# Bart-Weil/Dynamic-Camera-Augmented-VideoPose3D

Measured on AMD Instinct MI355X. Metric: 3D poses/sec, 243-frame RF, 17 joints, 1024ch; MPJPE vs ref, higher is better.
Workload: dtype f16x3; 1 GPU; config4 global batch sharded over ranks, TemporalModelOptimized1f 243-frame RF windows, 17 joints, 1024 ch; window batch assembled on device from resident sequences inside the step; global_batch=65536, windows_per_gpu=65536, parallelism=dp1 (contiguous shards of one global window set, no collective)

## Files before the change

dynamic-camera-augmented-videopose3d_amd/csrc/conv_gemm_a4.hip:

```cpp
#include <cstdlib>
#include <cstring>
#include <utility>

#include "gemm_common.h"

namespace vp3d {
namespace {

using namespace gemm;

typedef __attribute__((address_space(3))) void* lds_ptr_t;
typedef __attribute__((address_space(1))) void* gbl_ptr_t;

constexpr int GM = 256, GN = 256, GK = 64;
constexpr int GBUF = (GM + GN) * GK * 2;
constexpr int GW_OFF = GM * GK * 2;
constexpr int GMAXN = 1024;
constexpr int kLgkm0 = 0xC07F;
constexpr int kVm0Lgkm0 = 0x0070;
constexpr int kVm16Lgkm0 = 0x4070;
constexpr int kVm32Lgkm0 = 0x8070;

template <typename F, int... Is>
__device__ __forceinline__ void static_for_impl(F&& f, std::integer_sequence<int, Is...>) {
    (f(std::integral_constant<int, Is>{}), ...);
}
template <int N, typename F>
__device__ __forceinline__ void static_for(F&& f) {
    static_for_impl(f, std::make_integer_sequence<int, N>{});
}

__device__ __forceinline__ void pinned_barrier() {
    __builtin_amdgcn_sched_barrier(0);
    __builtin_amdgcn_s_barrier();
    __builtin_amdgcn_sched_barrier(0);
}

template <typename CT, int R, bool ZERO>
__device__ __forceinline__ void amma(const u32x4& w, const u32x4& a) {
    if constexpr (std::is_same<CT, __bf16>::value) {
        if constexpr (ZERO)
            asm volatile("v_mfma_f32_16x16x32_bf16 a[%c2:%c3], %0, %1, 0" ::"v"(w), "v"(a), "i"(R), "i"(R + 3));
        else
            asm volatile("v_mfma_f32_16x16x32_bf16 a[%c2:%c3], %0, %1, a[%c2:%c3]" ::"v"(w), "v"(a), "i"(R),
                         "i"(R + 3));
    } else {
        if constexpr (ZERO)
            asm volatile("v_mfma_f32_16x16x32_f16 a[%c2:%c3], %0, %1, 0" ::"v"(w), "v"(a), "i"(R), "i"(R + 3));
        else
            asm volatile("v_mfma_f32_16x16x32_f16 a[%c2:%c3], %0, %1, a[%c2:%c3]" ::"v"(w), "v"(a), "i"(R),
                         "i"(R + 3));
    }
}

#ifdef VP3D_ABLATION
template <typename CT, int R, bool ZERO>
__device__ __forceinline__ void amma32(const u32x4& w, const u32x4& a) {
    if constexpr (std::is_same<CT, __bf16>::value) {
        if constexpr (ZERO)
            asm volatile("v_mfma_f32_32x32x16_bf16 a[%c2:%c3], %0, %1, 0" ::"v"(w), "v"(a), "i"(R), "i"(R + 15));
        else
            asm volatile("v_mfma_f32_32x32x16_bf16 a[%c2:%c3], %0, %1, a[%c2:%c3]" ::"v"(w), "v"(a), "i"(R),
                         "i"(R + 15));
    } else {
        if constexpr (ZERO)
            asm volatile("v_mfma_f32_32x32x16_f16 a[%c2:%c3], %0, %1, 0" ::"v"(w), "v"(a), "i"(R), "i"(R + 15));
        else
            asm volatile("v_mfma_f32_32x32x16_f16 a[%c2:%c3], %0, %1, a[%c2:%c3]" ::"v"(w), "v"(a), "i"(R),
                         "i"(R + 15));
    }
}
#endif

__device__ __forceinline__ void launder_s(int& x) { asm volatile("" : "+s"(x)); }
__device__ __forceinline__ void launder_lane_consts(int& a, int& b, int& c, int& d, int& e, int& f, int& g, int& h,
                                                    int& i) {
    asm volatile("" : "+v"(a), "+v"(b), "+v"(c), "+v"(d), "+v"(e), "+v"(f), "+v"(g), "+v"(h), "+v"(i));
}
__device__ __forceinline__ void launder_params(ConvGemmParams& p) {
    asm volatile("" : "+s"(p.M), "+s"(p.Kp), "+s"(p.T_out), "+s"(p.T_in), "+s"(p.stride), "+s"(p.dil), "+s"(p.Ktap),
                 "+s"(p.lda), "+s"(p.R_T), "+s"(p.R_stride), "+s"(p.R_off), "+s"(p.ldr), "+s"(p.ldy));
    asm volatile("" : "+s"(p.A), "+s"(p.W), "+s"(p.R), "+s"(p.Y));
}

template <int R>
__device__ __forceinline__ float aread() {
    float x;
    asm volatile("v_accvgpr_read_b32 %0, a%c1" : "=v"(x) : "i"(R));
    return x;
}

#define A4_C10(d) "a" #d "0", "a" #d "1", "a" #d "2", "a" #d "3", "a" #d "4", "a" #d "5", "a" #d "6", "a" #d "7", \
                  "a" #d "8", "a" #d "9"
#define A4_ALL_AGPRS                                                                                              \
    "a0", "a1", "a2", "a3", "a4", "a5", "a6", "a7", "a8", "a9", A4_C10(1), A4_C10(2), A4_C10(3), A4_C10(4),      \
        A4_C10(5), A4_C10(6), A4_C10(7), A4_C10(8), A4_C10(9), A4_C10(10), A4_C10(11), A4_C10(12), A4_C10(13),   \
        A4_C10(14), A4_C10(15), A4_C10(16), A4_C10(17), A4_C10(18), A4_C10(19), A4_C10(20), A4_C10(21),          \
        A4_C10(22), A4_C10(23), A4_C10(24), "a250", "a251", "a252", "a253", "a254", "a255"

#ifdef VP3D_ABLATION
__device__ unsigned long long* g_a4_trace;
#endif

template <typename CT, int ABL, int X3 = 0, bool GD = true, bool SPLIT = false, int HNL = 0, bool IX = false>
__global__ __launch_bounds__(256, 1) void conv_gemm_a4(ConvGemmParams p_arg) {
    constexpr bool HN = HNL > 0;
    static_assert(!HN || (GD && !SPLIT), "half-N tiles: grouped pieces, no split");
    static_assert(HNL < 2 || X3 != 0, "quarter-N tiles: the split-fp16 epilogue only");
    static_assert(!IX || (X3 == 1 && GD && !SPLIT), "indirect windows: the split-fp16 whole / half-N / quarter-N tiles");
    constexpr int TN = GN >> HNL;
    constexpr int NJ = TN / 32;
    constexpr int WP = TN / 32;
    constexpr int NB = NJ < 4 ? NJ : 4;
    if (p_arg.gate != nullptr && *p_arg.gate != p_arg.gate_serial) return;
    asm volatile("" ::: A4_ALL_AGPRS);
    ConvGemmParams p = p_arg;

    __shared__ __attribute__((aligned(16))) char smem[2 * GBUF + 2 * GMAXN * 4];
    float* const s_scale = (float*)(smem + 2 * GBUF);
    float* const s_shift = s_scale + GMAXN;

    const int tid = threadIdx.x;
    const int lane = tid & 63;
    const int wid = tid >> 6;
    const int wr = wid >> 1, wc = wid & 1;
    const int widu = __builtin_amdgcn_readfirstlane(wid);

    for (int i = tid; i < p.N; i += 256) {
        s_scale[i] = p.scale[i];
        s_shift[i] = p.shift[i];
    }

    const int ntn = p.N / TN;
    const int ntm = (p.M + GM - 1) / GM;
    const int mt_base = HN ? p.sk_full : 0;
    const int ntiles = (ntm - mt_base) * ntn;
    const int nk_all = p.Kp / GK;
    const int S = SPLIT ? p.sk_split : 1;
    const int sk_full = S > 1 ? p.sk_full : ntiles;
    const int nunits = S > 1 ? sk_full + S * p.sk_left : ntiles;
    constexpr int kWhole = 0, kOwner = 1, kHelper = 2;
    int kb = 0, nk = nk_all, role = kWhole, sidx = 0, sq = 0;
    const bool lres_layer = X3 == 0 && p.R != nullptr && nk_all >= 3;
    bool lres = lres_layer;
#ifdef VP3D_ABLATION
    unsigned long long* const trc = (ABL & 4) && g_a4_trace ? g_a4_trace + (size_t)blockIdx.x * 10 : nullptr;
    unsigned long long mid_cyc = 0;
    auto stamp = [&](int slot) __attribute__((always_inline)) {
        if (trc && tid == 0) {
            trc[slot] = __builtin_amdgcn_s_memrealtime();
            trc[slot + 5] = __builtin_amdgcn_s_memtime();
        }
    };
    stamp(0);
    if (trc && tid == 0)
        trc[4] = ((unsigned long long)__builtin_amdgcn_s_getreg((31 << 11) | 20) << 32) |
                 __builtin_amdgcn_s_getreg((31 << 11) | 4);
#endif

    int prow = lane >> 3;
    int lc = (lane & 7) ^ (((wid & 1) * 4 + (prow >> 1)) & 7);
    constexpr int kReb = GD ? 3072 : 0;
    int m0 = 0, n0 = 0;
    uint32_t va[8], vw[8], vr[8];
    __amdgpu_buffer_rsrc_t a_rsrc, w_rsrc, r_rsrc;
    auto setup = [&](int unit) __attribute__((always_inline)) {
        int tix = unit;
        kb = 0;
        nk = nk_all;
        role = kWhole;
        if (S > 1 && unit >= sk_full) {
            const int v = unit - sk_full;
            sidx = v % p.sk_left;
            sq = S - 1 - v / p.sk_left;
            tix = sk_full + sidx;
            kb = sq * (nk_all / S);
            nk = nk_all / S;
            role = sq == 0 ? kOwner : kHelper;
        }
        lres = lres_layer && role != kHelper && nk >= 3;
        const int wg = xcd_remap(tix, ntiles);
        const int tile_m = wg / ntn;
        const int tile_n = wg - tile_m * ntn;
        m0 = (mt_base + tile_m) * GM;
        n0 = tile_n * TN;
        const int srow0 = IX && p.T_in < 0 ? 0 : src_row(p, m0);
        a_rsrc = make_rsrc((const char*)((const CT*)p.A + (int64_t)srow0 * p.lda) - kReb, 0x7FFFFFFFu);
        w_rsrc = make_rsrc((const char*)((const CT*)p.W + (int64_t)n0 * p.Kp) - kReb, 0x7FFFFFFFu);
        const int rrow0 = lres ? res_row(p, m0) : 0;
        r_rsrc = make_rsrc((const char*)(lres ? (const CT*)p.R + (int64_t)rrow0 * p.ldr : (const CT*)p.A) - kReb,
                           0x7FFFFFFFu);
        int sln = lane, swv = widu;
        asm volatile("" : "+v"(sln));
        launder_s(swv);
        const int spr = sln >> 3;
        if constexpr (IX) {
            int wb[8], wr0[8];
#pragma unroll
            for (int i = 0; i < 8; ++i) {
                const int q = GD ? 8 * swv + i : swv + 4 * i;
                int m = m0 + 8 * q + spr;
                m = m < p.M ? m : p.M - 1;
                wb[i] = m / p.T_out;
                va[i] = (uint32_t)((m - wb[i] * p.T_out) * p.stride);
            }
            window_rows(p.A, p.T_in, wb, wr0);
#pragma unroll
            for (int i = 0; i < 8; ++i) {
                const int lci = GD ? (sln & 7) ^ (((i & 1) * 4 + (spr >> 1)) & 7) : lc;
                const int reb = GD ? kReb - (i & 3) * 1024 : 0;
                va[i] = (uint32_t)(((wr0[i] + (int)va[i] - srow0) * p.lda + lci * 8) * (int)sizeof(CT) + reb);
            }
        }
#pragma unroll
        for (int i = 0; i < 8; ++i) {
            const int q = GD ? 8 * swv + i : swv + 4 * i;
            const int qw = HN ? WP * swv + (i % WP) : q;
            const int lci = GD ? (sln & 7) ^ (((i & 1) * 4 + (spr >> 1)) & 7) : lc;
            const int reb = GD ? kReb - (i & 3) * 1024 : 0;
            int m = m0 + 8 * q + spr;
            m = m < p.M ? m : p.M - 1;
            if constexpr (!IX)
                va[i] = (uint32_t)(((src_row(p, m) - srow0) * p.lda + lci * 8) * (int)sizeof(CT) + reb);
            vw[i] = (uint32_t)(((8 * qw + prow) * p.Kp + lci * 8) * (int)sizeof(CT) + reb);
            vr[i] = lres ? (uint32_t)(((res_row(p, m) - rrow0) * p.ldr + lci * 8) * (int)sizeof(CT) + reb) : 0u;
        }
    };
    auto lds_dst = [&](char* buf, int q) __attribute__((always_inline)) -> char* {
        int w = widu;
        launder_s(w);
        return buf + (w + q) * 1024;
    };
    struct Bases {
        char* g[4];
    };
    auto bases_of = [&](char* buf) __attribute__((always_inline)) -> Bases {
        int w = widu;
        launder_s(w);
        char* b = buf + 8 * w * 1024;
        if constexpr (HN) return Bases{{b, b + 4096, buf + GW_OFF + WP * w * 1024, nullptr}};
        return Bases{{b, b + 4096, b + GW_OFF, b + GW_OFF + 4096}};
    };
    auto piece_lds = [&](char* buf, int i) __attribute__((always_inline)) -> char* {
        if constexpr (GD) {
            int w = widu;
            launder_s(w);
            return buf + (8 * w + (i & 4)) * 1024;
        } else {
            return lds_dst(buf, 4 * i);
        }
    };
    auto res_piece = [&](char* buf, auto k_c, int h) __attribute__((always_inline)) {
        constexpr int k = decltype(k_c)::value;
        constexpr int wcp = k >> 3;
        __builtin_amdgcn_raw_ptr_buffer_load_lds(r_rsrc, (lds_ptr_t)piece_lds(buf + wcp * 32 * 1024, k & 7), 16,
                                                 vr[k & 7], (uint32_t)((n0 + 128 * wcp + 64 * h) * (int)sizeof(CT)),
                                                 GD ? (k & 3) * 1024 : 0, 0);
    };
    auto a_koff = [&](int s) __attribute__((always_inline)) -> int64_t {
        const int k0 = (kb + s) * GK;
        const int tap = k0 / p.Ktap;
        return (int64_t)tap * p.dil * p.lda + (k0 - tap * p.Ktap);
// ... 89 lines not shown
        });
        if constexpr (RD) __builtin_amdgcn_s_waitcnt(kLgkm0);
    };

    auto mid = [&](int vm) __attribute__((always_inline)) {
#ifdef VP3D_ABLATION
        const unsigned long long c0 = (ABL & 4) ? __builtin_amdgcn_s_memtime() : 0;
#endif
        if (vm == 16)
            __builtin_amdgcn_s_waitcnt(kVm16Lgkm0);
        else if (vm == 32)
            __builtin_amdgcn_s_waitcnt(kVm32Lgkm0);
        else
            __builtin_amdgcn_s_waitcnt(kVm0Lgkm0);
        pinned_barrier();
#ifdef VP3D_ABLATION
        if (ABL & 4) mid_cyc += __builtin_amdgcn_s_memtime() - c0;
#endif
    };
    using C0 = std::integral_constant<int, 0>;
    using C1 = std::integral_constant<int, 1>;
    using T_ = std::integral_constant<bool, true>;
    using F_ = std::integral_constant<bool, false>;
    auto ktile = [&](auto zero_c, auto rd_c, auto dma_c, int t, char* b, char* o, int resp, int vm) __attribute__((always_inline)) {
        phase(C0{}, zero_c, T_{}, F_{}, b, fo1, nullptr, 0, -1);
        mid(vm);
        phase(C1{}, F_{}, rd_c, dma_c, o, fo0, b, t + 2, resp);
    };

    typedef float f32x2 __attribute__((ext_vector_type(2)));
    typedef int i32x2 __attribute__((ext_vector_type(2)));
    typedef short s16x2 __attribute__((ext_vector_type(2)));
    typedef CT ct2 __attribute__((ext_vector_type(2)));
    typedef CT ct4 __attribute__((ext_vector_type(4)));
    typedef unsigned int u32x2 __attribute__((ext_vector_type(2)));
    int grp = lane >> 4;
    int c0 = 8 * ((grp & 1) * 2 + (grp >> 1));
    u32x2 resr[8][4];
    int enk = nk;
    auto res_addr = [&](int h, int i, int j) __attribute__((always_inline)) -> const u32x2* {
        return (const u32x2*)(smem + ((enk - 2 + h) & 1) * GBUF + wc * 256 * 128 + wr * 128 * 128 + (lane & 15) * 128 +
                              (grp & 1) * 8 + i * 2048 + (((2 * j + (grp >> 1)) ^ fsw) << 4));
    };
    auto part_ptr = [&](int si, int q) __attribute__((always_inline)) -> float* {
        return p.sk_part + (size_t)(si * (S - 1) + (q - 1)) * 65536 + (size_t)wid * 16384 + lane * 4;
    };
    auto helper_store = [&](int si, int q) __attribute__((always_inline)) {
        float* const base = part_ptr(si, q);
        static_for<64>([&](auto r_c) __attribute__((always_inline)) {
            constexpr int R4 = decltype(r_c)::value;
            *(f32x4*)(base + R4 * 256) = f32x4{aread<4 * R4>(), aread<4 * R4 + 1>(), aread<4 * R4 + 2>(), aread<4 * R4 + 3>()};
        });
        __builtin_amdgcn_fence(__ATOMIC_RELEASE, "agent");
        pinned_barrier();
        if (tid == 0) {
            const SplitCtl* ctl = (const SplitCtl*)((const char*)p.sk_flag + kSplitCtlOffset);
            if (!ctl->drop) __hip_atomic_fetch_add(p.sk_flag + si, 1, __ATOMIC_RELAXED, __HIP_MEMORY_SCOPE_AGENT);
        }
    };
    auto owner_wait = [&](int si) __attribute__((always_inline)) {
        if (tid == 0) {
            const SplitCtl* ctl = (const SplitCtl*)((const char*)p.sk_flag + kSplitCtlOffset);
            const unsigned long long spin = ctl->spin_ticks;
            const unsigned long long t0 = __builtin_amdgcn_s_memrealtime();
            while (__hip_atomic_load(p.sk_flag + si, __ATOMIC_RELAXED, __HIP_MEMORY_SCOPE_AGENT) < S - 1) {
                __builtin_amdgcn_s_sleep(1);
                if (__builtin_amdgcn_s_memrealtime() - t0 > spin) {
                    unsigned* err = ctl->err;
                    if (err) __hip_atomic_fetch_or(err, kFaultSplitTimeout, __ATOMIC_RELAXED, __HIP_MEMORY_SCOPE_SYSTEM);
                    break;
                }
            }
        }
        pinned_barrier();
        __builtin_amdgcn_fence(__ATOMIC_ACQUIRE, "agent");
    };
    auto owner_add = [&](auto r_c, int si, f32x2 (&v)[2]) __attribute__((always_inline)) {
        constexpr int R = decltype(r_c)::value;
        for (int q = 1; q < S; ++q) {
            const f32x4 pr = *(const f32x4*)(part_ptr(si, q) + (R / 4) * 256);
            v[0] = v[0] + f32x2{pr[0], pr[1]};
            v[1] = v[1] + f32x2{pr[2], pr[3]};
        }
    };
    auto owner_done = [&](int si) __attribute__((always_inline)) {
        if (tid == 0) __hip_atomic_fetch_sub(p.sk_flag + si, S - 1, __ATOMIC_RELAXED, __HIP_MEMORY_SCOPE_AGENT);
    };
    auto epi_fast = [&](auto h_c, bool with_res, int em0, int en0, __amdgpu_buffer_rsrc_t y_rsrc, int own_si) __attribute__((always_inline)) {
        constexpr int H = decltype(h_c)::value;
        const int nw = en0 + wc * (TN / 2) + 64 * H;
        f32x2 sc[4][2], sh[4][2];
#pragma unroll
        for (int j = 0; j < 4; ++j) {
            const int n = nw + 16 * j + 4 * grp;
            const f32x4 s4 = *(const f32x4*)&s_scale[n];
            const f32x4 h4 = *(const f32x4*)&s_shift[n];
            sc[j][0] = f32x2{s4[0], s4[1]};
            sc[j][1] = f32x2{s4[2], s4[3]};
            sh[j][0] = f32x2{h4[0], h4[1]};
            sh[j][1] = f32x2{h4[2], h4[3]};
        }
        static_for<8>([&](auto i_c) __attribute__((always_inline)) {
            constexpr int I = decltype(i_c)::value;
            const int m = em0 + wr * 128 + 16 * I + (lane & 15);
            uint32_t pk[4][2];
            static_for<4>([&](auto j_c) __attribute__((always_inline)) {
                constexpr int J = decltype(j_c)::value;
                constexpr int R = 4 * (8 * I + 4 * H + J);
                f32x2 v[2] = {f32x2{aread<R>(), aread<R + 1>()}, f32x2{aread<R + 2>(), aread<R + 3>()}};
                if (own_si >= 0) owner_add(std::integral_constant<int, R>{}, own_si, v);
                ct4 r4;
                if (with_res) r4 = __builtin_bit_cast(ct4, resr[I][J]);
#pragma unroll
                for (int q = 0; q < 2; ++q) {
                    f32x2 x = v[q] * sc[J][q];
                    x = x + sh[J][q];
                    if (with_res) {
                        i32x2 xi = __builtin_bit_cast(i32x2, x);
                        xi = __builtin_elementwise_max(xi, i32x2{0, 0});
                        x = __builtin_bit_cast(f32x2, xi);
                        x = x + f32x2{(float)r4[2 * q], (float)r4[2 * q + 1]};
                    }
                    s16x2 o = __builtin_bit_cast(s16x2, __builtin_convertvector(x, ct2));
                    if (!with_res) o = __builtin_elementwise_max(o, s16x2{0, 0});
                    pk[J][q] = __builtin_bit_cast(uint32_t, o);
                }
            });
            asm volatile("s_nop 1\n\tv_permlane16_swap_b32 %0, %1\n\tv_permlane16_swap_b32 %2, %3\n\t"
                         "v_permlane16_swap_b32 %4, %5\n\tv_permlane16_swap_b32 %6, %7"
                         : "+v"(pk[0][0]), "+v"(pk[1][0]), "+v"(pk[0][1]), "+v"(pk[1][1]), "+v"(pk[2][0]),
                           "+v"(pk[3][0]), "+v"(pk[2][1]), "+v"(pk[3][1]));
            const uint32_t yo = (uint32_t)(((size_t)(m - em0) * p.ldy + nw + c0) * sizeof(CT));
#pragma unroll
            for (int jp = 0; jp < 2; ++jp)
                __builtin_amdgcn_raw_buffer_store_b128(
                    u32x4{pk[2 * jp][0], pk[2 * jp][1], pk[2 * jp + 1][0], pk[2 * jp + 1][1]}, y_rsrc,
                    m < p.M ? yo + 64 * jp : 0xFFFFFFC0u, 0, 0);
        });
    };
    using H0 = std::integral_constant<int, 0>;
    using H1 = std::integral_constant<int, 1>;
    int res0 = -1, res1 = -1;

    int tix = blockIdx.x;
    setup(tix);
    stage_01();
    bool first = true;
    bool prev_lres = false;
    bool x3_prev_res = false;
    bool x3_prev_xres = false;
    for (;;) {
        launder_lane_consts(prow, lc, fsw, fo0, fo1, a_base, w_base, grp, c0);
        launder_params(p);
        const int next = HN ? nunits : tix + (int)gridDim.x;
        const bool has_next = next < nunits;
        res0 = lres ? 0 : -1;
        res1 = lres ? 1 : -1;
        if (first) {
            if (nk > 1)
            {
                if constexpr (HN)
                    asm volatile("s_waitcnt vmcnt(%0)" ::"n"(8 + WP) : "memory");
                else
                    asm volatile("s_waitcnt vmcnt(16)" ::: "memory");
            }
            else
                asm volatile("s_waitcnt vmcnt(0)" ::: "memory");
            asm volatile("s_waitcnt lgkmcnt(0)" ::: "memory");
        } else if constexpr (X3 != 0) {
            if (x3_prev_xres)
                asm volatile("s_waitcnt vmcnt(48)" ::: "memory");
            else if (!x3_prev_res)
                asm volatile("s_waitcnt vmcnt(0)" ::: "memory");
        } else {
            asm volatile("s_waitcnt vmcnt(48)" ::: "memory");
        }
        pinned_barrier();
#pragma unroll
        for (int i = 0; i < 8; ++i) {
            fa[0][i] = *(const u32x4*)(buf0 + a_base + i * 2048 + fo0);
            if (i < NJ) fw[0][i] = *(const u32x4*)(buf0 + w_base + i * 2048 + fo0);
        }
        if constexpr (X3 != 0) {
            const bool xres = X3 == 1 && !SPLIT && !HN && !(ABL & 40) && p.R != nullptr && role != kHelper && nk >= 3;
            __amdgpu_buffer_rsrc_t xr_rsrc;
            auto xres_prep = [&]() __attribute__((always_inline)) {
                int ln = lane, wv = widu;
                asm volatile("" : "+v"(ln));
                launder_s(wv);
                const int pr = ln >> 3;
                const int rrow0x = IX && p.R_T < 0 ? 0 : res_row(p, m0);
                xr_rsrc = make_rsrc((const char*)((const f16*)p.R + (int64_t)rrow0x * p.ldr), 0x7FFFFFFFu);
                if constexpr (IX) {
                    int wb[8], wr0[8];
#pragma unroll
                    for (int i = 0; i < 8; ++i) {
                        int m = m0 + 8 * (8 * wv + i) + pr;
                        m = m < p.M ? m : p.M - 1;
                        wb[i] = m / p.T_out;
                        vr[i] = (uint32_t)((m - wb[i] * p.T_out) * p.R_stride + p.R_off);
                    }
                    window_rows(p.R, p.R_T, wb, wr0);
#pragma unroll
                    for (int i = 0; i < 8; ++i) {
                        const int lci = (ln & 7) ^ (((i & 1) * 4 + (pr >> 1)) & 7);
                        vr[i] = (uint32_t)((wr0[i] + (int)vr[i] - rrow0x) * p.ldr * 2 + lci * 16);
                    }
                } else {
#pragma unroll
                    for (int i = 0; i < 8; ++i) {
                        int m = m0 + 8 * (8 * wv + i) + pr;
                        m = m < p.M ? m : p.M - 1;
                        const int lci = (ln & 7) ^ (((i & 1) * 4 + (pr >> 1)) & 7);
                        vr[i] = (uint32_t)((res_row(p, m) - rrow0x) * p.ldr * 2 + lci * 16);
                    }
                }
            };
            auto xres_piece = [&](char* buf, auto i_c, auto s_c, int wcq, int hh) __attribute__((always_inline)) {
                constexpr int I = decltype(i_c)::value;
                constexpr int S2 = decltype(s_c)::value;
                int w = widu;
                launder_s(w);
                __builtin_amdgcn_raw_ptr_buffer_load_lds(xr_rsrc, (lds_ptr_t)(buf + (2 * (8 * w + I) + S2) * 1024), 16, vr[I],
                                                         (uint32_t)(4 * (n0 + wcq * 128 + 64 * hh) + S2 * 128), 0, 0);
            };
            auto x3_phase = [&](auto h_c, auto kind_c, auto zero_c, auto rd_c, auto dma_c, const char* rbuf, char* dbuf,
                                int s, auto rq_c, char* rqbuf) __attribute__((always_inline)) {
                constexpr int RQ = decltype(rq_c)::value;
                constexpr int H = decltype(h_c)::value;
                constexpr int KIND = decltype(kind_c)::value;
                constexpr bool ZERO = decltype(zero_c)::value;
                constexpr bool DO_RD = decltype(rd_c)::value && !(ABL & 2);
                constexpr bool DO_DMA = decltype(dma_c)::value && !(ABL & 1);
                const int64_t aoff = DO_DMA ? a_koff(s) : 0;
                const Bases bs = DO_DMA ? bases_of(dbuf) : Bases{};
                constexpr int JW = HN ? (NJ > 2 ? 2 : 1) : 4;
                static_for<8>([&](auto i_c) __attribute__((always_inline)) {
                    constexpr int I = decltype(i_c)::value;
                    constexpr bool WI = !HN || I < NJ;
                    static_for<NJ>([&](auto j_c) __attribute__((always_inline)) {
                        constexpr int J = decltype(j_c)::value;
                        if constexpr (KIND == 0) {
                            if constexpr (DO_RD && J == 0)
                                fa[1 - H][I] = *(const u32x4*)(rbuf + a_base + I * 2048 + fo1);
                            if constexpr (DO_RD && J == JW && WI)
                                fw[1][I] = *(const u32x4*)(rbuf + w_base + I * 2048 + fo1);
                            amma<CT, 4 * (8 * I + J), ZERO>(fw[0][J], fa[H][I]);
                        } else if constexpr (KIND == 1) {
                            if constexpr (DO_RD && J == 0 && I > 0)
                                fa[1 - H][I - 1] = *(const u32x4*)(rbuf + a_base + (I - 1) * 2048 + fo0);
                            if constexpr (DO_DMA && J == JW) dma_piece(dbuf, i_c, s, aoff, bs);
                            if constexpr (RQ >= 0 && !HN && (J == 2 || J == 6))
                                xres_piece(rqbuf, i_c, std::integral_constant<int, J / 4>{}, RQ, 0);
                            amma<CT, 4 * (8 * I + J), false>(fw[0][J], fa[1 - H][I]);
                        } else {
                            if constexpr (DO_RD && J == 0 && I == 0)
                                fa[1 - H][7] = *(const u32x4*)(rbuf + a_base + 7 * 2048 + fo0);
                            if constexpr (DO_RD && J == JW && WI)
                                fw[0][I] = *(const u32x4*)(rbuf + w_base + I * 2048 + fo0);
                            if constexpr (DO_DMA && J == (HN ? NJ - 1 : 2) && WI)
                                dma_piece(dbuf, std::integral_constant<int, 8 + I>{}, s, aoff, bs);
                            if constexpr (RQ >= 0 && !HN && (J == 2 || J == 6))
                                xres_piece(rqbuf, i_c, std::integral_constant<int, J / 4>{}, RQ, 0);
                            amma<CT, 4 * (8 * I + J), false>(fw[1][J], fa[H][I]);
                        }
                        __builtin_amdgcn_sched_barrier(0);
                    });
                });
                if constexpr (KIND == 2 && DO_RD) __builtin_amdgcn_s_waitcnt(kLgkm0);
            };
            using K0 = std::integral_constant<int, 0>;
            using K1 = std::integral_constant<int, 1>;
            using K2 = std::integral_constant<int, 2>;
            auto x3_ktile_q = [&](auto h_c, auto zero_c, auto rd_c, auto dma_c, auto rql_c, int t, char* b, char* o,
                                  int vm) __attribute__((always_inline)) {
                constexpr bool rql = decltype(rql_c)::value;
                x3_phase(h_c, K0{}, zero_c, T_{}, F_{}, b, nullptr, 0, std::integral_constant<int, -1>{}, nullptr);
                if (vm == 63)
                    __builtin_amdgcn_s_waitcnt(kLgkm0);
                else if (vm == 32)
                    __builtin_amdgcn_s_waitcnt(kVm32Lgkm0);
                else
                    __builtin_amdgcn_s_waitcnt(kVm0Lgkm0);
                pinned_barrier();
                x3_phase(h_c, K1{}, F_{}, rd_c, dma_c, o, b, t + 2, std::integral_constant<int, rql ? 0 : -1>{}, o);
                x3_phase(h_c, K2{}, F_{}, rd_c, dma_c, o, b, t + 2, std::integral_constant<int, rql ? 1 : -1>{}, b);
            };
            auto x3_ktile = [&](auto h_c, auto zero_c, auto rd_c, auto dma_c, int t, char* b, char* o, int vm = 0)
                                __attribute__((always_inline)) {
                x3_ktile_q(h_c, zero_c, rd_c, dma_c, std::false_type{}, t, b, o, vm);
            };
            const int vm0 = first ? 0 : (x3_prev_xres ? 32 : 63);
            if (nk > 2)
                x3_ktile(C0{}, T_{}, T_{}, T_{}, 0, buf0, buf1, vm0);
            else if (nk == 2)
                x3_ktile(C0{}, T_{}, T_{}, F_{}, 0, buf0, buf1, vm0);
            else
                x3_ktile(C0{}, T_{}, F_{}, F_{}, 0, buf0, buf1, vm0);
            int t = 1;
            for (; t + 3 < nk; t += 2) {
                x3_ktile(C1{}, F_{}, T_{}, T_{}, t, buf1, buf0);
                x3_ktile(C0{}, F_{}, T_{}, T_{}, t + 1, buf0, buf1);
            }
            if (t + 2 < nk) {
                x3_ktile(C1{}, F_{}, T_{}, T_{}, t, buf1, buf0);
                x3_ktile(C0{}, F_{}, T_{}, F_{}, t + 1, buf0, buf1);
                if (xres) {
                    xres_prep();
                    x3_ktile_q(C1{}, F_{}, F_{}, F_{}, std::true_type{}, t + 2, buf1, buf0, 0);
                } else {
                    x3_ktile(C1{}, F_{}, F_{}, F_{}, t + 2, buf1, buf0);
                }
            } else if (t + 1 < nk) {
                x3_ktile(C1{}, F_{}, T_{}, F_{}, t, buf1, buf0);
                if (xres) {
                    xres_prep();
                    x3_ktile_q(C0{}, F_{}, F_{}, F_{}, std::true_type{}, t + 1, buf0, buf1, 0);
                } else {
                    x3_ktile(C0{}, F_{}, F_{}, F_{}, t + 1, buf0, buf1);
                }
            } else if (t < nk) {
                x3_ktile(C1{}, F_{}, F_{}, F_{}, t, buf1, buf0);
            }
            asm volatile("s_nop 7\n\ts_nop 7\n\ts_nop 7" ::: "memory");
            const int em0 = m0, en0 = n0;
            const int erole = role, esidx = sidx, esq = sq;
            char* const qb0 = (nk & 1) ? buf1 : buf0;
            char* const qb1 = (nk & 1) ? buf0 : buf1;
            auto xres_read = [&](u32x4 (&rr)[8][2][2]) __attribute__((always_inline)) {
                int ln = lane, wv = widu;
                asm volatile("" : "+v"(ln));
                launder_s(wv);
                const char* qb = (wv & 1) ? qb1 : qb0;
                const int swz = (((ln >> 3) & 1) * 4 + ((ln & 7) >> 1)) & 7;
                const int g = ln >> 4;
                const int cc = (g & 1) * 2 + (g >> 1);
                const char* rowp = qb + (2 * ((wv >> 1) * 16 + ((ln >> 3) & 1))) * 1024 + (ln & 7) * 128;
#pragma unroll
                for (int i = 0; i < 8; ++i)
#pragma unroll
                    for (int jp = 0; jp < 2; ++jp)
#pragma unroll
                        for (int hl = 0; hl < 2; ++hl)
                            rr[i][jp][hl] = *(const u32x4*)(rowp + (4 * i + jp) * 1024 + (((hl * 4 + cc) ^ swz) << 4));
            };
            constexpr int OB = X3 == 2 ? 4 : 2;
            typedef float f32x2 __attribute__((ext_vector_type(2)));
            typedef int i32x2 __attribute__((ext_vector_type(2)));
            const bool has_r = p.R != nullptr;
            int eln = lane, ewv = widu;
            asm volatile("" : "+v"(eln));
            launder_s(ewv);
            const int egrp = eln >> 4, er16 = eln & 15;
            const int ec0 = 8 * ((egrp & 1) * 2 + (egrp >> 1));
            const int ewr = ewv >> 1, ewc = ewv & 1;
            auto x3_half = [&](auto hh_c, auto wr_c, const u32x4 (&rr)[8][2][2], __amdgpu_buffer_rsrc_t y_rsrc)
                               __attribute__((always_inline)) {
                constexpr int HH = decltype(hh_c)::value;
                constexpr bool WITH_R = decltype(wr_c)::value && !(ABL & 8);
                const int nw = en0 + ewc * (TN / 2) + 64 * HH;
                f32x2 sc[4][2], sh[4][2];
#pragma unroll
                for (int j = 0; j < NB; ++j) {
                    const int n = nw + 16 * j + 4 * egrp;
                    const f32x4 s4 = *(const f32x4*)&s_scale[n];
                    const f32x4 h4 = *(const f32x4*)&s_shift[n];
                    sc[j][0] = f32x2{s4[0], s4[1]};
                    sc[j][1] = f32x2{s4[2], s4[3]};
                    sh[j][0] = f32x2{h4[0], h4[1]};
                    sh[j][1] = f32x2{h4[2], h4[3]};
                }
                static_for<8>([&](auto i_c) __attribute__((always_inline)) {
                    constexpr int I = decltype(i_c)::value;
                    const int m = em0 + ewr * 128 + 16 * I + er16;
                    float v4[4][4];
                    static_for<NB>([&](auto j_c) __attribute__((always_inline)) {
                        constexpr int J = decltype(j_c)::value;
                        constexpr int R = 4 * (8 * I + 4 * HH + J);
                        f32x2 v[2] = {f32x2{aread<R>(), aread<R + 1>()}, f32x2{aread<R + 2>(), aread<R + 3>()}};
                        if (erole == kOwner) owner_add(std::integral_constant<int, R>{}, esidx, v);
#pragma unroll
                        for (int q = 0; q < 2; ++q) {
                            f32x2 x = v[q] * sc[J][q];
                            x = x + sh[J][q];
                            if (p.relu) {
                                i32x2 xi = __builtin_bit_cast(i32x2, x);
                                xi = __builtin_elementwise_max(xi, i32x2{0, 0});
                                x = __builtin_bit_cast(f32x2, xi);
                            }
                            v4[J][2 * q] = x[0];
                            v4[J][2 * q + 1] = x[1];
                        }
                    });
#pragma unroll
                    for (int jp = 0; jp < NB / 2; ++jp) {
                        float* x = v4[2 * jp];
                        float* y = v4[2 * jp + 1];
                        asm volatile("s_nop 1\n\tv_permlane16_swap_b32 %0, %1\n\tv_permlane16_swap_b32 %2, %3\n\t"
                                     "v_permlane16_swap_b32 %4, %5\n\tv_permlane16_swap_b32 %6, %7"
                                     : "+v"(x[0]), "+v"(y[0]), "+v"(x[1]), "+v"(y[1]), "+v"(x[2]), "+v"(y[2]),
                                       "+v"(x[3]), "+v"(y[3]));
                        float v[8] = {x[0], x[1], x[2], x[3], y[0], y[1], y[2], y[3]};
                        if constexpr (WITH_R) {
                            const u32x4 rh = rr[I][jp][0], rl = rr[I][jp][1];
#pragma unroll
                            for (int e = 0; e < 4; ++e) {
                                float t0, t1;
                                gemm::x3_res_sum2(rh[e], rl[e], t0, t1);
                                v[2 * e] += t0;
                                v[2 * e + 1] += t1;
                            }
                        }
                        const bool in = m < p.M;
                        if constexpr (X3 == 2) {
                            const uint32_t yo =
                                in ? (uint32_t)(((size_t)(m - em0) * p.ldy + nw + 32 * jp + ec0) * 4) : 0xFFFFFFE0u;
                            __builtin_amdgcn_raw_buffer_store_b128(
                                __builtin_bit_cast(u32x4, f32x4{v[0], v[1], v[2], v[3]}), y_rsrc, yo, 0, 0);
                            __builtin_amdgcn_raw_buffer_store_b128(
                                __builtin_bit_cast(u32x4, f32x4{v[4], v[5], v[6], v[7]}), y_rsrc, yo + 16, 0, 0);
                        } else {
                            u32x4 oh, ol;
                            float t = 0.f;
#pragma unroll
                            for (int e = 0; e < 4; ++e) {
                                oh[e] = gemm::x3_hi2(v[2 * e], v[2 * e + 1]);
                                ol[e] = gemm::x3_split_lo2(oh[e], v[2 * e], v[2 * e + 1]);
                                t = gemm::x3_absmax2(t, v[2 * e], v[2 * e + 1]);
                            }
                            gemm::x3_range_flag(in ? t : 0.f, p.scale, p.N);
                            const uint32_t yo =
                                in ? (uint32_t)(((size_t)(m - em0) * p.ldy + 2 * nw + 64 * jp + ec0) * 2) : 0xFFFFFF00u;
                            if constexpr ((ABL & 16) != 0) {
                                asm volatile("" ::"v"(oh), "v"(ol));
                            } else {
                                __builtin_amdgcn_raw_buffer_store_b128(oh, y_rsrc, yo, 0, 0);
                                __builtin_amdgcn_raw_buffer_store_b128(ol, y_rsrc, yo + 64, 0, 0);
                            }
                        }
                    }
                });
            };
            auto y_rsrc_of = [&]() __attribute__((always_inline)) {
                const size_t y_rest = (size_t)(p.M - em0) * p.ldy * OB;
                return make_rsrc((const char*)p.Y + (size_t)em0 * p.ldy * OB,
                                 clamp_range31(y_rest));
            };
            if (xres) {
                u32x4 rr[8][2][2];
                asm volatile("s_waitcnt vmcnt(0)" ::: "memory");
                pinned_barrier();
                xres_read(rr);
                __builtin_amdgcn_s_waitcnt(kLgkm0);
                pinned_barrier();
                static_for<8>([&](auto i_c) __attribute__((always_inline)) {
                    xres_piece(qb0, i_c, std::integral_constant<int, 0>{}, 0, 1);
                    xres_piece(qb0, i_c, std::integral_constant<int, 1>{}, 0, 1);
                    xres_piece(qb1, i_c, std::integral_constant<int, 0>{}, 1, 1);
                    xres_piece(qb1, i_c, std::integral_constant<int, 1>{}, 1, 1);
                });
                if (erole == kOwner) owner_wait(esidx);
                const __amdgpu_buffer_rsrc_t y_rsrc = y_rsrc_of();
                x3_half(std::integral_constant<int, 0>{}, T_{}, rr, y_rsrc);
                asm volatile("s_waitcnt vmcnt(32)" ::: "memory");
                pinned_barrier();
                xres_read(rr);
                __builtin_amdgcn_s_waitcnt(kLgkm0);
                pinned_barrier();
                if (has_next) {
                    setup(next);
                    stage_01();
                }
                x3_half(std::integral_constant<int, 1>{}, T_{}, rr, y_rsrc);
                if (erole == kOwner) owner_done(esidx);
            } else {
                if (has_next) {
                    setup(next);
                    stage_01();
                }
                if (erole == kHelper) {
                    helper_store(esidx, esq);
                    x3_prev_res = false;
                    x3_prev_xres = false;
                    if (!has_next) break;
                    tix = next;
                    first = false;
                    continue;
                }
                if (erole == kOwner) owner_wait(esidx);
                const __amdgpu_buffer_rsrc_t y_rsrc = y_rsrc_of();
                const int rrow0 = has_r && !(IX && p.R_T < 0) ? res_row(p, em0) : 0;
                const __amdgpu_buffer_rsrc_t rx_rsrc =
                    make_rsrc(has_r ? (const f16*)p.R + (int64_t)rrow0 * p.ldr : (const f16*)p.A, 0x7FFFFFFFu);
                auto global_half = [&](auto hh_c) __attribute__((always_inline)) {
                    constexpr int HH = decltype(hh_c)::value;
                    const int nw = en0 + ewc * (TN / 2) + 64 * HH;
                    u32x4 rr[8][2][2];
                    if (has_r && !(ABL & 8)) {
                        int wb[8], wo[8], wr0[8];
                        if constexpr (IX) {
#pragma unroll
                            for (int i = 0; i < 8; ++i) {
                                int m = em0 + ewr * 128 + 16 * i + er16;
                                m = m < p.M ? m : p.M - 1;
                                wb[i] = m / p.T_out;
                                wo[i] = (m - wb[i] * p.T_out) * p.R_stride + p.R_off;
                            }
                            window_rows(p.R, p.R_T, wb, wr0);
                        }
#pragma unroll
                        for (int i = 0; i < 8; ++i) {
                            int m = em0 + ewr * 128 + 16 * i + er16;
                            m = m < p.M ? m : p.M - 1;
                            const int off = (((IX ? wr0[i] + wo[i] : res_row(p, m)) - rrow0) * p.ldr + 2 * nw + ec0) * 2;
#pragma unroll
                            for (int jp = 0; jp < NB / 2; ++jp) {
                                rr[i][jp][0] = __builtin_bit_cast(
                                    u32x4, __builtin_amdgcn_raw_buffer_load_b128(rx_rsrc, off + 128 * jp, 0, 0));
                                rr[i][jp][1] = __builtin_bit_cast(
                                    u32x4, __builtin_amdgcn_raw_buffer_load_b128(rx_rsrc, off + 128 * jp + 64, 0, 0));
                            }
                        }
                        x3_half(hh_c, T_{}, rr, y_rsrc);
                    } else {
                        x3_half(hh_c, F_{}, rr, y_rsrc);
                    }
                };
                if constexpr ((ABL & 32) == 0) {
                    global_half(std::integral_constant<int, 0>{});
                    if constexpr (!HN) global_half(std::integral_constant<int, 1>{});
                }
                if (erole == kOwner) owner_done(esidx);
            }
            x3_prev_res = has_r;
            x3_prev_xres = xres;
            if (!has_next) break;
            tix = next;
            first = false;
            continue;
        } else {
        const int vm0 = first ? 0 : prev_lres ? 16 : 32;
        if (nk > 2)
            ktile(T_{}, T_{}, T_{}, 0, buf0, buf1, -1, vm0);
        else if (nk == 2)
            ktile(T_{}, T_{}, F_{}, 0, buf0, buf1, -1, vm0);
        else
            ktile(T_{}, F_{}, F_{}, 0, buf0, buf1, -1, vm0);
#ifdef VP3D_ABLATION
        if (first) stamp(1);
#endif
        const int em0 = m0, en0 = n0;
        enk = nk;
        const int erole = role, esidx = sidx, esq = sq;
        const bool elres = lres;
        auto next_setup = [&]() __attribute__((always_inline)) {
            if (has_next) setup(next);
        };
        auto last_ktile = [&](int t, char* b, char* o) __attribute__((always_inline)) {
            phase(C0{}, F_{}, T_{}, F_{}, b, fo1, nullptr, 0, -1);
            mid(lres ? 16 : 0);
            if (lres || !has_next) {
                phase(C1{}, F_{}, F_{}, F_{}, o, fo0, b, 0, res1);
            } else {
                next_setup();
                phase(C1{}, F_{}, F_{}, F_{}, o, fo0, b, 0, -1);
                stage_01();
            }
        };
        int t = 1;
        for (; t + 3 < nk; t += 2) {
            ktile(F_{}, T_{}, T_{}, t, buf1, buf0, -1, 0);
            ktile(F_{}, T_{}, T_{}, t + 1, buf0, buf1, -1, 0);
        }
        if (t + 2 < nk) {
            ktile(F_{}, T_{}, T_{}, t, buf1, buf0, -1, 0);
            ktile(F_{}, T_{}, F_{}, t + 1, buf0, buf1, res0, 0);
            last_ktile(t + 2, buf1, buf0);
        } else if (t + 1 < nk) {
            ktile(F_{}, T_{}, F_{}, t, buf1, buf0, res0, 0);
            last_ktile(t + 1, buf0, buf1);
        } else if (t < nk) {
            last_ktile(t, buf1, buf0);
        }
        asm volatile("s_nop 7\n\ts_nop 7\n\ts_nop 7" ::: "memory");
#ifdef VP3D_ABLATION
        stamp(2);
        if (trc && tid == 0) trc[9] = mid_cyc;
#endif

        if (erole == kHelper) {
            helper_store(esidx, esq);
            break;
        }
        if (erole == kOwner) owner_wait(esidx);
        const int own_si = erole == kOwner ? esidx : -1;
        const size_t y_rest = (size_t)(p.M - em0) * p.ldy * sizeof(CT);
// ... 19 lines not shown
                    const Bases bh = bases_of(H == 0 ? buf0 : buf1);
                    static_for<16>([&](auto i_c) __attribute__((always_inline)) {
                        dma_piece(H == 0 ? buf0 : buf1, i_c, H, o, bh);
                    });
                }
                epi_fast(h_c, true, em0, en0, y_rsrc, own_si);
            };
            part(H0{});
            part(H1{});
        } else {
            epi_fast(H0{}, false, em0, en0, y_rsrc, own_si);
            if constexpr (!HN) epi_fast(H1{}, false, em0, en0, y_rsrc, own_si);
        }
        if (erole == kOwner) owner_done(esidx);
        prev_lres = elres;
        if (!has_next) break;
        tix = next;
        first = false;
        }
    }
#ifdef VP3D_ABLATION
    if (ABL & 4) {
        asm volatile("s_waitcnt vmcnt(0)" ::: "memory");
        pinned_barrier();
        stamp(3);
    }
#endif
}

#undef A4_C10
#undef A4_ALL_AGPRS

}

#ifdef VP3D_ABLATION
hipError_t conv_gemm_a4_set_trace(unsigned long long* buf) {
    return hipMemcpyToSymbol(HIP_SYMBOL(g_a4_trace), &buf, sizeof(buf));
}
#endif

bool conv_gemm_a4_eligible(const ConvGemmParams& p, Act a_type, Act out_type, Act compute) {
    if (compute == Act::F32 || a_type != compute || out_type != compute) return false;
    if (p.relu != 1) return false;
    if (p.R && p.Kp / GK < 3) return false;
    if (p.Ktap % GK != 0 || p.Kp % GK != 0 || p.lda % 8 != 0) return false;
    if (p.N % GN != 0 || p.N > GMAXN || p.ldy % 8 != 0 || (p.R && p.ldr % 8 != 0)) return false;
    if ((reinterpret_cast<uintptr_t>(p.A) & 15) || (reinterpret_cast<uintptr_t>(p.Y) & 15) ||
        (p.R && (reinterpret_cast<uintptr_t>(p.R) & 15)))
        return false;
    return (size_t)p.N * p.Kp < (1u << 31);
}

static int a4_hn_tail(const ConvGemmParams& p, int ntiles, bool x3, int* level = nullptr);
static bool a4_tail_split(const ConvGemmParams& p, int mt_tail, int level, bool need_ws);
static bool a4_indirect(const ConvGemmParams& p);

static bool a4_x3_shape_ok(const ConvGemmParams& p, bool out_f32) {
    if (p.Ktap % GK != 0 || p.Kp % GK != 0 || p.lda % 8 != 0) return false;
    if (p.N % GN != 0 || p.N > GMAXN || p.ldy % (out_f32 ? 4 : 8) != 0 || (p.R && p.ldr % 8 != 0)) return false;
    if ((reinterpret_cast<uintptr_t>(p.A) & 15) || (reinterpret_cast<uintptr_t>(p.Y) & 15) ||
        (reinterpret_cast<uintptr_t>(p.W) & 15) || (p.R && (reinterpret_cast<uintptr_t>(p.R) & 15)))
        return false;
    return (size_t)p.N * p.Kp < (1u << 31);
}

bool conv_gemm_a4_x3_eligible(const ConvGemmParams& p, bool out_f32) {
    if (!a4_x3_shape_ok(p, out_f32)) return false;
    const int ntiles = ((p.M + GM - 1) / GM) * (p.N / GN);
    if (!conv_gemm_a4_fills(p) && a4_hn_tail(p, ntiles, true) == 0) return false;
    return (size_t)p.N * p.Kp < (1u << 31);
}

static int a4_cus() {
    static const int ncu = [] {
        int dev = 0, n = 0;
        if (hipGetDevice(&dev) != hipSuccess || hipDeviceGetAttribute(&n, hipDeviceAttributeMultiprocessorCount, dev) != hipSuccess)
            return 0;
        return n & ~7;
    }();
    return ncu;
}

int conv_gemm_a4_round_tiles() { return a4_cus(); }
int64_t conv_gemm_a4_tiles(int64_t rows, int N) { return (rows + GM - 1) / GM * (N / GN); }

static void a4_split_plan(ConvGemmParams& q, int ntiles, int nk, bool need_ws = true) {
    q.sk_split = q.sk_full = q.sk_left = 0;
    const char* e = getenv("VP3D_A4_SPLIT");
    const int mode = e ? atoi(e) : 1;
    if (mode == 0 || (need_ws && (!q.sk_part || !q.sk_flag))) return;
    const int ncu = a4_cus();
    if (ncu <= 0 || ncu > 256) return;
    if (mode == 1 && (nk < 64 || ntiles >= 8 * ncu)) return;
    const int L = ntiles % ncu;
    if (L == 0) return;
    int S = ncu / L;
    S = S > 4 ? 4 : S;
    while (S >= 2 && (nk % S != 0 || nk / S < 4 || (nk / S) % 2 != 0)) --S;
    if (S < 2) return;
    q.sk_full = ntiles - L;
    q.sk_split = S;
    q.sk_left = L;
}

static int a4_hn_tail(const ConvGemmParams& p, int ntiles, bool x3, int* level) {
    const char* e = getenv("VP3D_A4_HN");
    if (e && e[0] == '0') return 0;
    const char* sp = getenv("VP3D_A4_SPLIT");
    if (sp && atoi(sp) == 2) return 0;
    const int ncu = a4_cus();
    const int ntn = p.N / GN;
    if ((p.R != nullptr && !x3) || ncu <= 0 || ntn <= 0) return 0;
    const int L = ntiles % ncu;
    if (L == 0 || 2 * L > ncu || L % ntn != 0 || (!x3 && ntiles >= ncu)) return 0;
    if (level) *level = x3 && 4 * L <= ncu && !(e && e[0] == '1') ? 2 : 1;
    return L / ntn;
}

static bool a4_tail_split(const ConvGemmParams& p, int mt_tail, int level, bool need_ws) {
    if (level != 2 || mt_tail <= 0) return false;
    const char* e = getenv("VP3D_A4_TAIL");
    if (e && strcmp(e, "hn") == 0) return false;
    const char* sp = getenv("VP3D_A4_SPLIT");
    if (sp && atoi(sp) == 0) return false;
    const int mt0 = (p.M + GM - 1) / GM - mt_tail;
    if (mt0 <= 0) return false;
    return conv_gemm_tail_fits(p, mt0 * GM, a4_cus(), need_ws);
}

bool conv_gemm_a4_would_split(const ConvGemmParams& p) {
    const int ntiles = ((p.M + GM - 1) / GM) * (p.N / GN);
    int level = 1;
    const int hn = a4_hn_tail(p, ntiles, true, &level);
    if (hn > 0) return a4_tail_split(p, hn, level, false);
    ConvGemmParams q = p;
    a4_split_plan(q, ntiles, p.Kp / GK, false);
    return q.sk_split > 1;
}

static bool a4_indirect(const ConvGemmParams& p) { return p.T_in < 0 || (p.R != nullptr && p.R_T < 0); }

bool conv_gemm_a4_x3_indirect_ok(const ConvGemmParams& p, bool any_fill) {
    if (!(any_fill ? a4_x3_shape_ok(p, false) : conv_gemm_a4_x3_eligible(p, false))) return false;
    const int ntiles = ((p.M + GM - 1) / GM) * (p.N / GN);
    const char* we = getenv("VP3D_A4_WALK");
    int level = 1;
    const int hn = we && atoi(we) == 2 ? 0 : a4_hn_tail(p, ntiles, true, &level);
    if (hn > 0) return !a4_tail_split(p, hn, level, false);
    ConvGemmParams q = p;
    a4_split_plan(q, ntiles, p.Kp / GK, false);
    return q.sk_split <= 1;
}

bool conv_gemm_a4_fills(const ConvGemmParams& p) {
    const int ntiles = ((p.M + GM - 1) / GM) * (p.N / GN);
    if (ntiles >= 384) return true;
    if (a4_hn_tail(p, ntiles, false) > 0) return true;
    ConvGemmParams q = p;
    a4_split_plan(q, ntiles, p.Kp / GK);
    return q.sk_split > 1;
}

template <typename CT, int X3, bool IX = false>
static void a4_launch(const ConvGemmParams& p, dim3 grid, bool split, hipStream_t stream) {
    if constexpr (IX)
        hipLaunchKernelGGL((conv_gemm_a4<CT, 0, X3, true, false, 0, true>), grid, dim3(256), 0, stream, p);
    else if (split)
        hipLaunchKernelGGL((conv_gemm_a4<CT, 0, X3, true, true>), grid, dim3(256), 0, stream, p);
    else
        hipLaunchKernelGGL((conv_gemm_a4<CT, 0, X3, true, false>), grid, dim3(256), 0, stream, p);
}

template <typename CT, int X3, bool IX = false>
static void a4_launch_whole(const ConvGemmParams& p, int mt0, hipStream_t stream, int walk_cus) {
    if (mt0 > 0) {
        ConvGemmParams q = p;
        q.M = mt0 * GM;
        q.sk_split = q.sk_full = q.sk_left = 0;
        const int tiles = mt0 * (p.N / GN);
        const dim3 g(walk_cus > 0 && tiles > walk_cus ? walk_cus : tiles);
        hipLaunchKernelGGL((conv_gemm_a4<CT, 0, X3, true, false, 0, IX>), g, dim3(256), 0, stream, q);
    }
}

template <typename CT, int X3, bool IX = false>
static void a4_launch_hn(const ConvGemmParams& p, int mt_tail, hipStream_t stream, int walk_cus = 0, int level = 1) {
    const int ntm = (p.M + GM - 1) / GM;
    const int mt0 = ntm - mt_tail;
    a4_launch_whole<CT, X3, IX>(p, mt0, stream, walk_cus);
    ConvGemmParams t = p;
    t.sk_split = t.sk_left = 0;
    t.sk_full = mt0;
    if constexpr (X3 != 0) {
        if (level == 2) {
            hipLaunchKernelGGL((conv_gemm_a4<CT, 0, X3, true, false, 2, IX>), dim3(mt_tail * (p.N / (GN / 4))), dim3(256),
                               0, stream, t);
            return;
        }
    }
    hipLaunchKernelGGL((conv_gemm_a4<CT, 0, X3, true, false, 1, IX>), dim3(mt_tail * (p.N / (GN / 2))), dim3(256), 0,
                       stream, t);
}

#ifdef VP3D_ABLATION
template <int ABL>
static void a4_x3_abl(const ConvGemmParams& p, dim3 grid) {
    hipLaunchKernelGGL((conv_gemm_a4<_Float16, ABL, 1, true, false>), grid, dim3(256), 0, 0, p);
}
#endif

hipError_t launch_conv_gemm_a4_x3(const ConvGemmParams& p_in, bool out_f32, hipStream_t stream) {
    const int ntiles = ((p_in.M + GM - 1) / GM) * (p_in.N / GN);
    ConvGemmParams p = p_in;
    const char* we = getenv("VP3D_A4_WALK");
    const int walk_mode = we ? atoi(we) : 1;
    int hn_level = 1;
    const int hn_tail = walk_mode == 2 ? 0 : a4_hn_tail(p, ntiles, true, &hn_level);
    const bool ix = a4_indirect(p);
    if (ix && (out_f32 || !conv_gemm_a4_x3_indirect_ok(p, true))) return hipErrorInvalidValue;
#ifndef VP3D_ABLATION
    if (hn_tail > 0) {
        const int wc = walk_mode > 0 && p.R != nullptr ? a4_cus() : 0;
        if (ix) {
            a4_launch_hn<_Float16, 1, true>(p, hn_tail, stream, wc, hn_level);
            return hipGetLastError();
        }
        if (a4_tail_split(p, hn_tail, hn_level, true)) {
            const int mt0 = (p.M + GM - 1) / GM - hn_tail;
            if (out_f32)
                a4_launch_whole<_Float16, 2>(p, mt0, stream, wc);
            else
                a4_launch_whole<_Float16, 1>(p, mt0, stream, wc);
            return launch_conv_gemm_tail_x3(p, mt0 * GM, out_f32, a4_cus(), stream);
        }
        if (out_f32)
            a4_launch_hn<_Float16, 2>(p, hn_tail, stream, wc, hn_level);
        else
            a4_launch_hn<_Float16, 1>(p, hn_tail, stream, wc, hn_level);
        return hipGetLastError();
    }
#endif
    a4_split_plan(p, ntiles, p.Kp / GK);
    const bool split = p.sk_split > 1;
    const int nunits = split ? p.sk_full + p.sk_split * p.sk_left : ntiles;
    const int ncu = a4_cus();
    const bool walk = walk_mode > 0 && (p.R != nullptr || walk_mode == 2) && ncu > 0 && nunits > ncu;
    const dim3 grid(walk ? ncu : nunits);
#ifdef VP3D_ABLATION
    static const int abl = [] {
        const char* e = getenv("VP3D_ABL");
        return e ? atoi(e) : 0;
    }();
    if (abl && !out_f32 && !split) {
        switch (abl) {
            case 1: a4_x3_abl<1>(p, grid); break;
            case 2: a4_x3_abl<2>(p, grid); break;
            case 3: a4_x3_abl<3>(p, grid); break;
            case 8: a4_x3_abl<8>(p, grid); break;
            case 16: a4_x3_abl<16>(p, grid); break;
            case 24: a4_x3_abl<24>(p, grid); break;
            case 32: a4_x3_abl<32>(p, grid); break;
            default: return hipErrorInvalidValue;
        }
        return hipGetLastError();
    }
#endif
    if (ix)
        a4_launch<_Float16, 1, true>(p, grid, false, stream);
    else if (out_f32)
        a4_launch<_Float16, 2>(p, grid, split, stream);
    else
        a4_launch<_Float16, 1>(p, grid, split, stream);
    return hipGetLastError();
}

hipError_t launch_conv_gemm_a4(const ConvGemmParams& p_in, Act compute, hipStream_t stream) {
    const int ntiles = ((p_in.M + GM - 1) / GM) * (p_in.N / GN);
    const char* we = getenv("VP3D_A4_WALK");
    const int walk_mode = we ? atoi(we) : 1;
    const int ncu = a4_cus();
    const int nk = p_in.Kp / GK;
    ConvGemmParams p = p_in;
#ifndef VP3D_ABLATION
    const int hn_tail = walk_mode == 2 ? 0 : a4_hn_tail(p, ntiles, false);
    if (hn_tail > 0) {
        if (compute == Act::BF16)
            a4_launch_hn<__bf16, 0>(p, hn_tail, stream);
        else
            a4_launch_hn<_Float16, 0>(p, hn_tail, stream);
        return hipGetLastError();
    }
#endif
    {
        int lvl = 1;
        const int mt_tail = walk_mode == 2 ? 0 : a4_hn_tail(p, ntiles, true, &lvl);
        if (mt_tail > 0 && a4_tail_split(p, mt_tail, lvl, true)) {
            const int mt0 = (p.M + GM - 1) / GM - mt_tail;
            const int tiles = mt0 * (p.N / GN);
            const bool wk = walk_mode > 0 && p.R != nullptr && ncu > 0 && nk >= 3 && tiles > ncu && nk % 2 == 0;
            ConvGemmParams q = p;
            q.M = mt0 * GM;
            q.sk_split = q.sk_full = q.sk_left = 0;
            if (compute == Act::BF16)
                a4_launch<__bf16, 0>(q, dim3(wk ? ncu : tiles), false, stream);
            else
                a4_launch<_Float16, 0>(q, dim3(wk ? ncu : tiles), false, stream);
            return launch_conv_gemm_tail16(p, mt0 * GM, compute, ncu, stream);
        }
    }
    a4_split_plan(p, ntiles, nk);
    const bool split = p.sk_split > 1;
    const int nunits = split ? p.sk_full + p.sk_split * p.sk_left : ntiles;
    const bool walk = walk_mode > 0 && (p.R != nullptr || walk_mode == 2) && ncu > 0 && nk >= 3 && nunits > ncu &&
                      (!p.R || nk % 2 == 0);
    const dim3 grid(walk ? ncu : nunits);
#ifdef VP3D_ABLATION
    static const int abl = [] {
        const char* e = getenv("VP3D_ABL");
        return e ? atoi(e) : 0;
    }();
    if (compute == Act::BF16 && abl >= 1) {
        p.sk_split = 0;
        const dim3 g(walk ? ncu : ntiles);
        switch (abl) {
            case 1: hipLaunchKernelGGL((conv_gemm_a4<__bf16, 1>), g, dim3(256), 0, stream, p); break;
            case 2: hipLaunchKernelGGL((conv_gemm_a4<__bf16, 2>), g, dim3(256), 0, stream, p); break;
            case 3: hipLaunchKernelGGL((conv_gemm_a4<__bf16, 3>), g, dim3(256), 0, stream, p); break;
            case 64: hipLaunchKernelGGL((conv_gemm_a4<__bf16, 64>), g, dim3(256), 0, stream, p); break;
            case 65: hipLaunchKernelGGL((conv_gemm_a4<__bf16, 65>), g, dim3(256), 0, stream, p); break;
            case 66: hipLaunchKernelGGL((conv_gemm_a4<__bf16, 66>), g, dim3(256), 0, stream, p); break;
            default: hipLaunchKernelGGL((conv_gemm_a4<__bf16, 4>), g, dim3(256), 0, stream, p); break;
        }
        return hipGetLastError();
    }
#endif
    if (compute == Act::BF16)
        a4_launch<__bf16, 0>(p, grid, split, stream);
    else
        a4_launch<_Float16, 0>(p, grid, split, stream);
    return hipGetLastError();
}

}
```

dynamic-camera-augmented-videopose3d_amd/csrc/expand_table.hip:

```cpp
#include "kernels.h"

namespace vp3d {
namespace {

typedef unsigned int u32x4 __attribute__((ext_vector_type(4)));

__global__ __launch_bounds__(256) void window_bases_kernel(const int32_t* __restrict__ pairs,
                                                           const int32_t* __restrict__ seq_len, int B, int n_seq,
                                                           WindowRegions wr, int lo, int lead,
                                                           int32_t* __restrict__ base, unsigned* fault) {
    const int b = blockIdx.x * 256 + threadIdx.x;
    if (b == 0 && wr.hint) __hip_atomic_store(wr.hint, wr.serial, __ATOMIC_RELAXED, __HIP_MEMORY_SCOPE_SYSTEM);
    if (b >= B) return;
    const int2 pr = *(const int2*)(pairs + 2 * b);
    const bool ok = pr.x >= 0 && pr.x < n_seq;
    const int hi = seq_len[ok ? pr.x : 0] - 1 + lead;
    const int st = pr.y < lo ? lo : (pr.y > hi ? hi : pr.y);
    const bool low = st < 0, high = st >= wr.max_len;
    int row = pr.x * wr.pitch + (st - wr.main_lo);
    if (wr.epitch > 0 && low) row = wr.edge_row0 + 2 * pr.x * wr.epitch + (st - lo);
    if (wr.epitch > 0 && high) row = wr.edge_row0 + (2 * pr.x + 1) * wr.epitch + (st - wr.max_len);
    base[b] = ok ? row : 0;
    if (!ok && fault) __hip_atomic_fetch_or(fault, kFaultWindowStart, __ATOMIC_RELAXED, __HIP_MEMORY_SCOPE_SYSTEM);
    const bool edge = ok && (low || high);
    const unsigned long long em = __ballot(edge);
    if (edge && (threadIdx.x & 63) == __ffsll((long long)em) - 1) {
        if (wr.gate) __hip_atomic_fetch_max(wr.gate, wr.serial, __ATOMIC_RELAXED, __HIP_MEMORY_SCOPE_AGENT);
        if (wr.hint) __hip_atomic_store(wr.hint + 1, wr.serial, __ATOMIC_RELAXED, __HIP_MEMORY_SCOPE_SYSTEM);
    }
}

template <bool NT>
__global__ __launch_bounds__(256) void gather_table_rows_kernel(const u32x4* __restrict__ table,
                                                                const int32_t* __restrict__ base, int64_t rows,
                                                                int T_out, int s0, int row16, u32x4* __restrict__ out) {
    for (int64_t r = blockIdx.x; r < rows; r += gridDim.x) {
        const int b = (int)(r / T_out);
        const int t = (int)(r - (int64_t)b * T_out);
        const u32x4* src = table + (int64_t)(base[b] + t * s0) * row16;
        u32x4* dst = out + r * row16;
        for (int c = threadIdx.x; c < row16; c += 256) {
            const u32x4 v = src[c];
            if (NT)
                __builtin_nontemporal_store(v, dst + c);
            else
                dst[c] = v;
        }
    }
}

}

hipError_t launch_window_bases(const int32_t* pairs, const int32_t* seq_len, int B, int n_seq, const WindowRegions& wr,
                               int lo, int lead, int32_t* base, unsigned* fault, hipStream_t s) {
    if (lo > 0 || lead < 0 || wr.main_lo > 0 || wr.main_lo < lo || wr.epitch < 0) return hipErrorInvalidValue;
    hipLaunchKernelGGL(window_bases_kernel, dim3((B + 255) / 256), dim3(256), 0, s, pairs, seq_len, B, n_seq, wr, lo,
                       lead, base, fault);
    return hipGetLastError();
}

hipError_t launch_gather_table_rows(const void* table, const int32_t* base, int B, int T_out, int s0,
                                    int row_bytes, void* out, hipStream_t s) {
    if (row_bytes % 16 != 0 || B <= 0 || T_out <= 0) return hipErrorInvalidValue;
    const int64_t rows = (int64_t)B * T_out;
    const bool nt = rows * row_bytes > (int64_t)256 << 20;
    const unsigned grid = (unsigned)(rows < (1 << 20) ? rows : (1 << 20));
    if (nt)
        hipLaunchKernelGGL(gather_table_rows_kernel<true>, dim3(grid), dim3(256), 0, s, (const u32x4*)table, base, rows,
                           T_out, s0, row_bytes / 16, (u32x4*)out);
    else
        hipLaunchKernelGGL(gather_table_rows_kernel<false>, dim3(grid), dim3(256), 0, s, (const u32x4*)table, base, rows,
                           T_out, s0, row_bytes / 16, (u32x4*)out);
    return hipGetLastError();
}

}
```

dynamic-camera-augmented-videopose3d_amd/csrc/gemm_common.h:

```cpp
#pragma once
#include "kernels.h"

#pragma clang fp contract(off)

namespace vp3d {
namespace gemm {

typedef __bf16 bf16;
typedef _Float16 f16;
typedef __bf16 bf16x8 __attribute__((ext_vector_type(8)));
typedef _Float16 f16x8 __attribute__((ext_vector_type(8)));
typedef float f32x4 __attribute__((ext_vector_type(4)));
typedef unsigned int u32x4 __attribute__((ext_vector_type(4)));


__device__ __forceinline__ int xcd_remap(int bid, int nwg) {
    const int xcd = bid & 7;
    const int q = nwg >> 3, r = nwg & 7;
    const int base = (xcd < r) ? xcd * (q + 1) : r * (q + 1) + (xcd - r) * q;
    return base + (bid >> 3);
}

template <typename T> __device__ __forceinline__ float to_f32(T v) { return (float)v; }

template <typename T> __device__ __forceinline__ T from_f32(float v) { return (T)v; }

template <typename CT> struct Pack8;
template <> struct Pack8<bf16> { typedef bf16x8 type; };
template <> struct Pack8<f16> { typedef f16x8 type; };

template <typename CT>
__device__ __forceinline__ u32x4 pack8(const float (&v)[8]) {
    typename Pack8<CT>::type r;
#pragma unroll
    for (int e = 0; e < 8; ++e) r[e] = (CT)v[e];
    return __builtin_bit_cast(u32x4, r);
}

template <typename CT>
__device__ __forceinline__ f32x4 mfma16(u32x4 a, u32x4 b, f32x4 c);
template <>
__device__ __forceinline__ f32x4 mfma16<bf16>(u32x4 a, u32x4 b, f32x4 c) {
    return __builtin_amdgcn_mfma_f32_16x16x32_bf16(__builtin_bit_cast(bf16x8, a),
                                                   __builtin_bit_cast(bf16x8, b), c, 0, 0, 0);
}
template <>
__device__ __forceinline__ f32x4 mfma16<f16>(u32x4 a, u32x4 b, f32x4 c) {
    return __builtin_amdgcn_mfma_f32_16x16x32_f16(__builtin_bit_cast(f16x8, a),
                                                  __builtin_bit_cast(f16x8, b), c, 0, 0, 0);
}

__device__ __forceinline__ int src_row(const ConvGemmParams& p, int m) {
    const int b = m / p.T_out;
    const int t = m - b * p.T_out;
    return b * p.T_in + t * p.stride;
}

__device__ __forceinline__ int res_row(const ConvGemmParams& p, int m) {
    const int b = m / p.T_out;
    const int t = m - b * p.T_out;
    return b * p.R_T + t * p.R_stride + p.R_off;
}

template <int N>
__device__ __forceinline__ void window_rows(const void* op, int T, const int (&b)[N], int (&r0)[N]) {
    if (T < 0) {
        typedef const __attribute__((address_space(1))) int* gbl_int_ptr;
        const gbl_int_ptr base = (gbl_int_ptr)op + T;
#pragma unroll
        for (int i = 0; i < N; ++i) r0[i] = base[b[i]];
#pragma unroll
        for (int i = 0; i < N; ++i) asm volatile("" : "+v"(r0[i]));
    } else {
#pragma unroll
        for (int i = 0; i < N; ++i) r0[i] = b[i] * T;
    }
}

enum : int { A_SCALAR = 0, A_PAIRS = 1, A_VEC = 2 };

template <typename AT>
__device__ __forceinline__ float load_a_scalar(const ConvGemmParams& p, int srow, int kk) {
    if (kk >= p.K) return 0.f;
    const int tap = kk / p.Ktap;
    const int c = kk - tap * p.Ktap;
    const AT* A = (const AT*)p.A;
    return to_f32(A[(int64_t)(srow + tap * p.dil) * p.lda + c]);
}

template <typename AT, int AMODE, int NE>
__device__ __forceinline__ void load_a_run(const ConvGemmParams& p, int srow, int kk0, bool valid,
                                           float (&v)[NE]) {
    if (!valid) {
#pragma unroll
        for (int e = 0; e < NE; ++e) v[e] = 0.f;
        return;
    }
    if constexpr (AMODE == A_PAIRS) {
        const float* row = (const float*)p.A + (int64_t)srow * p.lda;
#pragma unroll
        for (int e = 0; e < NE; e += 2) {
            const int kk = kk0 + e;
            if (kk < p.K) {
                const float2 t = *(const float2*)(row + kk);
                v[e] = t.x;
                v[e + 1] = t.y;
            } else {
                v[e] = v[e + 1] = 0.f;
            }
        }
    } else {
#pragma unroll
        for (int e = 0; e < NE; ++e) v[e] = load_a_scalar<AT>(p, srow, kk0 + e);
    }
}

template <typename OT>
__device__ __forceinline__ void epi_store(const ConvGemmParams& p, int m, int n, float v,
                                          float sc, float sh) {
    v = __fadd_rn(__fmul_rn(v, sc), sh);
    if (p.relu == 1) v = v > 0.f ? v : 0.f;
    else if (p.relu == 2) v = v > 0.f ? v : v * 0.01f;
    if (p.R) v += to_f32(((const OT*)p.R)[(int64_t)res_row(p, m) * p.ldr + n]);
    ((OT*)p.Y)[(int64_t)m * p.ldy + n] = from_f32<OT>(v);
}

template <typename OT, int MI>
__device__ __forceinline__ void epilogue_scalar(const ConvGemmParams& p, const f32x4 (&acc)[MI][4],
                                                int mw, int nw, int lane) {
#pragma unroll
    for (int j = 0; j < 4; ++j) {
        const int n = nw + j * 16 + (lane & 15);
        if (n >= p.N) continue;
        const float sc = p.scale[n], sh = p.shift[n];
#pragma unroll
        for (int i = 0; i < MI; ++i)
#pragma unroll
            for (int r = 0; r < 4; ++r) {
                const int m = mw + i * 16 + (lane >> 4) * 4 + r;
                if (m < p.M) epi_store<OT>(p, m, n, acc[i][j][r], sc, sh);
            }
    }
}

constexpr int kEpiLd = 68;

template <typename OT, int MI, int PASS_ROWS>
__device__ __forceinline__ void epilogue_vec(const ConvGemmParams& p, const f32x4 (&acc)[MI][4],
                                             float* stage, int mw, int nw, int lane) {
    constexpr int NP = MI * 16 / PASS_ROWS;
    constexpr int NQ = PASS_ROWS / 8;
    constexpr int RW = sizeof(OT) == 2 ? 1 : 2;
    const int c8 = lane & 7;
    const int n = nw + c8 * 8;
    const bool nval = n < p.N;
    float sc[8], sh[8];
#pragma unroll
    for (int e = 0; e < 8; ++e) {
        sc[e] = nval ? p.scale[n + e] : 0.f;
        sh[e] = nval ? p.shift[n + e] : 0.f;
    }
    u32x4 res[2][NQ][RW];
    auto load_res = [&](int pass, u32x4 (&r)[NQ][RW]) {
#pragma unroll
        for (int q = 0; q < NQ; ++q) {
            const int m = mw + pass * PASS_ROWS + q * 8 + (lane >> 3);
            if (p.R && m < p.M && nval) {
                const OT* rp = (const OT*)p.R + (int64_t)res_row(p, m) * p.ldr + n;
#pragma unroll
                for (int w = 0; w < RW; ++w) r[q][w] = *(const u32x4*)(rp + w * (16 / sizeof(OT)));
            } else {
#pragma unroll
                for (int w = 0; w < RW; ++w) r[q][w] = u32x4{0u, 0u, 0u, 0u};
            }
        }
    };
    load_res(0, res[0]);
#pragma unroll
    for (int pass = 0; pass < NP; ++pass) {
#pragma unroll
        for (int ii = 0; ii < PASS_ROWS / 16; ++ii) {
            const int i = pass * (PASS_ROWS / 16) + ii;
#pragma unroll
            for (int j = 0; j < 4; ++j)
#pragma unroll
                for (int r = 0; r < 4; ++r)
                    stage[(ii * 16 + (lane >> 4) * 4 + r) * kEpiLd + j * 16 + (lane & 15)] = acc[i][j][r];
        }
        asm volatile("" ::: "memory");
        if (pass + 1 < NP) load_res(pass + 1, res[(pass + 1) & 1]);
#pragma unroll
        for (int q = 0; q < NQ; ++q) {
            const int row = q * 8 + (lane >> 3);
            const int m = mw + pass * PASS_ROWS + row;
            const f32x4 lo = *(const f32x4*)&stage[row * kEpiLd + c8 * 8];
            const f32x4 hi = *(const f32x4*)&stage[row * kEpiLd + c8 * 8 + 4];
            if (m < p.M && nval) {
                float v[8] = {lo[0], lo[1], lo[2], lo[3], hi[0], hi[1], hi[2], hi[3]};
#pragma unroll
                for (int e = 0; e < 8; ++e) {
                    v[e] = __fadd_rn(__fmul_rn(v[e], sc[e]), sh[e]);
                    if (p.relu == 1) v[e] = v[e] > 0.f ? v[e] : 0.f;
                    else if (p.relu == 2) v[e] = v[e] > 0.f ? v[e] : v[e] * 0.01f;
                }
                if (p.R) {
                    const u32x4(&rq)[RW] = res[pass & 1][q];
                    if constexpr (sizeof(OT) == 2) {
                        typedef OT ot8 __attribute__((ext_vector_type(8)));
                        const ot8 r8 = __builtin_bit_cast(ot8, rq[0]);
#pragma unroll
                        for (int e = 0; e < 8; ++e) v[e] += (float)r8[e];
                    } else {
                        const f32x4 r0 = __builtin_bit_cast(f32x4, rq[0]);
                        const f32x4 r1 = __builtin_bit_cast(f32x4, rq[1]);
// ... 328 lines not shown
```

dynamic-camera-augmented-videopose3d_amd/csrc/host.h:

```cpp
#pragma once
#include <hip/hip_runtime.h>

#include <cstdint>
#include <cstring>
#include <string>
#include <vector>

#include "../../include/vp3d.h"
#include "kernels.h"

namespace vp3d {
namespace host {

int fail(int code, const std::string& msg);

#define HIP_TRY(expr)                                                                   \
    do {                                                                                \
        hipError_t _e = (expr);                                                         \
        if (_e != hipSuccess)                                                           \
            return ::vp3d::host::fail(_e == hipErrorOutOfMemory ? VP3D_ERR_OOM : VP3D_ERR_HIP, \
                                      std::string(#expr) + ": " + hipGetErrorString(_e)); \
    } while (0)

inline uint16_t f32_to_bf16_rne(float f) {
    uint32_t u;
    std::memcpy(&u, &f, 4);
    if ((u & 0x7f800000u) == 0x7f800000u && (u & 0x7fffffu)) return (uint16_t)((u >> 16) | 0x40);
    u += 0x7fffu + ((u >> 16) & 1u);
    return (uint16_t)(u >> 16);
}

inline uint16_t f32_to_f16_rne(float f) {
    _Float16 h = (_Float16)f;
    uint16_t r;
    std::memcpy(&r, &h, 2);
    return r;
}

inline float bf16_to_f32(uint16_t h) {
    const uint32_t u = (uint32_t)h << 16;
    float f;
    std::memcpy(&f, &u, 4);
    return f;
}

inline float f16_to_f32(uint16_t h) {
    _Float16 v;
    std::memcpy(&v, &h, 2);
    return (float)v;
}

inline size_t x3_pos(size_t k) { return (k >> 5) * 64 + (k & 31); }

struct Layer {
    int cin = 0, cout = 0, taps = 1, dil = 1, stride = 1;
    int K = 0, Kp = 0, Np = 0, Ktap = 0, gemm_taps = 1;
    bool relu = true;
    bool residual = false;
    int res_stride = 1, res_off = 0;
    float* w32 = nullptr;
    uint16_t* wbf = nullptr;
    uint16_t* wh = nullptr;
    float* scale = nullptr;
    float* shift = nullptr;
    uint16_t* wfbf = nullptr;
    uint16_t* wfh = nullptr;
    uint16_t* wx3 = nullptr;
    float* scale_x3 = nullptr;
    float* shift_x3 = nullptr;
    float* scale_x3_f32 = nullptr;
    std::vector<float> sc_host, sh_host;
    int e_x3 = 0;
    bool balance_x3 = true;
};

struct ProfEvent {
    int layer;
    hipEvent_t a, b;
    double flop;
};

int validate_cfg(const vp3d_cfg* c);
void build_geometry(const vp3d_cfg& c, std::vector<int>& pad, std::vector<int>& causal_shift,
                    std::vector<Layer>& layers);
bool layer_lengths(const vp3d_cfg& c, const std::vector<int>& pad, const std::vector<Layer>& layers, int T,
                   std::vector<int>& len);

}
}

struct vp3d_handle {
    vp3d_cfg cfg{};
    int device = 0;
    std::vector<int> pad, causal_shift;
    std::vector<vp3d::host::Layer> layers;
    void* ws = nullptr;
    size_t ws_bytes = 0;
    float* gather_ws = nullptr;
    size_t gather_bytes = 0;
    void* tab_ws = nullptr;
    size_t tab_bytes = 0;
    int32_t* tab_pairs = nullptr;
    std::vector<int32_t> tab_pairs_host;
    int tab_mode = 0;
    int tab_depth = 0;
    unsigned tab_serial = 0;
    unsigned* tab_gate = nullptr;
    unsigned* tab_hint_host = nullptr;
    unsigned* tab_hint_dev = nullptr;
    int tab_layout = 0;
    void* sk_ws = nullptr;
    std::vector<int> x3_prescale;
    vp3d::ActStats* x3_stats = nullptr;
    unsigned* sk_err_host = nullptr;
    unsigned* sk_err_dev = nullptr;
    unsigned long long sk_ctl_spin = 0;
    int sk_ctl_drop = -1;
    vp3d::SplitCtl sk_ctl_stage{};
    bool profiling = false;
    uint64_t prof_mask = ~0ull;
    std::vector<vp3d::host::ProfEvent> pending;
    std::vector<hipEvent_t> free_events;
    std::vector<double> prof_ms;
    std::vector<int64_t> prof_n;
    std::vector<double> prof_flop;
};
```

dynamic-camera-augmented-videopose3d_amd/csrc/kernels.h:

```cpp
#pragma once
#include <hip/hip_runtime.h>
#include <stdint.h>

namespace vp3d {

struct ConvGemmParams {
    const void* A;
    const void* W;
    const float* scale;
    const float* shift;
    const void* R;
    void* Y;
    int M, N, K, Kp;
    int T_out, T_in, stride, dil, Ktap, lda;
    int R_T, R_stride, R_off, ldr;
    int ldy;
    int relu;
    float* sk_part;
    int* sk_flag;
    int sk_full, sk_split, sk_left;
    const unsigned* gate;
    unsigned gate_serial;
};

struct SplitCtl {
    unsigned long long spin_ticks;
    unsigned* err;
    int drop;
    int pad;
};

constexpr size_t kSplitPartBytes = (size_t)256 * 256 * 1024;
constexpr size_t kSplitFlagBytes = 4096;
constexpr size_t kSplitCtlOffset = kSplitFlagBytes - 32;

enum class Act { F32 = 0, BF16 = 1, F16 = 2 };

hipError_t launch_conv_gemm(const ConvGemmParams& p, Act a_type, Act out_type, Act compute,
                            hipStream_t stream);

bool conv_gemm_big_eligible(const ConvGemmParams& p, Act a_type, Act out_type, Act compute);
hipError_t launch_conv_gemm_big(const ConvGemmParams& p, Act out_type, Act compute,
                                hipStream_t stream);
bool conv_gemm_8p_eligible(const ConvGemmParams& p, Act a_type, Act out_type, Act compute);
hipError_t launch_conv_gemm_8p(const ConvGemmParams& p, Act compute, hipStream_t stream);
bool conv_gemm_q64_eligible(const ConvGemmParams& p, Act a_type, Act out_type, Act compute);
hipError_t launch_conv_gemm_q64(const ConvGemmParams& p, Act compute, hipStream_t stream);
bool conv_gemm_a4_eligible(const ConvGemmParams& p, Act a_type, Act out_type, Act compute);
bool conv_gemm_a4_fills(const ConvGemmParams& p);
bool conv_gemm_a4_would_split(const ConvGemmParams& p);
constexpr unsigned long long kSplitSpinTicks = 100000000ull;
hipError_t launch_conv_gemm_a4(const ConvGemmParams& p, Act compute, hipStream_t stream);
bool conv_gemm_a4_x3_eligible(const ConvGemmParams& p, bool out_f32);
int64_t conv_gemm_a4_tiles(int64_t rows, int N);
int conv_gemm_a4_round_tiles();
hipError_t launch_conv_gemm_a4_x3(const ConvGemmParams& p, bool out_f32, hipStream_t stream);
bool conv_gemm_a4_x3_indirect_ok(const ConvGemmParams& p, bool any_fill = false);
bool conv_gemm_tail_fits(const ConvGemmParams& p, int m_begin, int ncu, bool need_ws);
hipError_t launch_conv_gemm_tail_x3(const ConvGemmParams& p, int m_begin, bool out_f32, int ncu,
                                    hipStream_t stream);
hipError_t launch_conv_gemm_tail16(const ConvGemmParams& p, int m_begin, Act compute, int ncu,
                                   hipStream_t stream);
hipError_t launch_conv_gemm_x3_shrink(const ConvGemmParams& p, hipStream_t stream);
bool conv_gemm_q64_x3_eligible(const ConvGemmParams& p, bool out_f32);
hipError_t launch_conv_gemm_q64_x3(const ConvGemmParams& p, bool out_f32, hipStream_t stream);
hipError_t conv_gemm_8p_set_trace(unsigned long long* buf);
hipError_t conv_gemm_a4_set_trace(unsigned long long* buf);

struct GatherSrc {
    const float* kps = nullptr;
    int f2 = 0;
    const float* cams = nullptr;
    const int64_t* seq_off = nullptr;
    const int32_t* seq_len = nullptr;
    const int32_t* pairs = nullptr;
    int lead = 0;
};

bool expand_gemm_eligible(const ConvGemmParams& p, Act out_type, Act compute);
hipError_t launch_expand_gemm(const ConvGemmParams& p, Act compute, hipStream_t stream);
bool expand_gather_eligible(const ConvGemmParams& p, const GatherSrc& g, Act out_type, Act compute);
hipError_t launch_expand_gemm_gather(const ConvGemmParams& p, const GatherSrc& g, Act compute,
                                     hipStream_t stream);

bool expand_gemm_x3_eligible(const ConvGemmParams& p, const GatherSrc* g);
hipError_t launch_expand_gemm_x3(const ConvGemmParams& p, const GatherSrc* g, hipStream_t stream);

constexpr int kPadN = 256;
constexpr int kPadK = 64;

struct StreamLayerParams {
    const void* W;
    const float* scale;
    const float* shift;
    int N, K, Kp, cin, taps, dil, relu;
    const float* in;
    int in_R;
    const float* in_frame;
    int in_frame_R;
    float* in_ring_w;
    const float* res;
    int res_R;
    float* out;
    int out_R;
    int* frames_seen;
    int advance;
    unsigned* done_counter;
};
hipError_t launch_stream_gemv(const StreamLayerParams& q, Act wtype, hipStream_t s);

constexpr int kStreamBatchMax = 64;
struct StreamBatchParams {
    const void* W;
    const float* scale;
    const float* shift;
    int N, K, Kp, cin, taps, dil, relu;
    int S;
    const float* in;
    int in_R;
    int64_t in_stride;
    const float* in_frame;
    float* in_ring_w;
    const float* res;
    int res_R;
    int64_t res_stride;
    float* out;
    int out_R;
    int64_t out_stride;
    const int* t;
    const int* active;
    const int* n;
    int lookahead;
    int res_back;
    int in_clamp;
    int out_gate;
};
constexpr int kStreamCodeIdle = 0, kStreamCodeConsume = 1, kStreamCodeDrain = 2;
hipError_t launch_stream_batch(const StreamBatchParams& q, Act wtype, hipStream_t s);
hipError_t launch_stream_batch_advance(int* t, const int* active, int S, hipStream_t s);
hipError_t launch_stream_batch_advance_look(int* t, int* n, const int* codes, int* pose_frame, int lookahead, int S,
                                            hipStream_t s);

struct StreamFault {
    unsigned* err;
    unsigned* err_host;
    unsigned long long spin_ticks;
};
constexpr unsigned long long kStreamSpinTicks = 25000000ull;

constexpr int kStreamMaxLayers = 16;
constexpr int kStreamMaxTaps = 8;
constexpr int kStreamMaxBlocks = 7;
struct StreamPersistParams {
    const void* W[kStreamMaxLayers];
    const float* scale[kStreamMaxLayers];
    const float* shift[kStreamMaxLayers];
    int Kp[kStreamMaxLayers], N[kStreamMaxLayers];
    int w_off[kStreamMaxLayers];
    int nl, nb, C, CPW, G, cin0;
    int taps[kStreamMaxBlocks + 1], dil[kStreamMaxBlocks + 1], ring[kStreamMaxBlocks + 1];
    int x_off, xin_off, hist_off, part_off, ss_off;
    int part_floats, state_floats;
    const float* frames;
    int queue;
    float* poses;
    int* frames_seen;
    unsigned long long* gran;
    StreamFault fault;
    float* state;
    int steps;
};
int stream_persist_lds_bytes();
hipError_t launch_stream_persist(const StreamPersistParams& p, Act wtype, hipStream_t s);

constexpr int kPipeCwK = 3;
constexpr int kPipeCwP = 8;
constexpr int kPipeMaxCh = 512;
constexpr int kPipeExpandK = 128;
constexpr int kStreamTraceSlots = 11;
struct StreamPipeParams {
    const void* W[kStreamMaxLayers];
    const float* scale[kStreamMaxLayers];
    const float* shift[kStreamMaxLayers];
    int Kp[kStreamMaxLayers], N[kStreamMaxLayers];
    int cu0[kStreamMaxLayers + 1];
    int nl, nb, C, cin0;
    int dil[kStreamMaxBlocks + 1], ring[kStreamMaxBlocks + 1];
    const float* frames;
    int queue;
    float* poses;
    int* frames_seen;
    unsigned* arrivals;
    unsigned long long* gran;
    int chunk_stride;
    int poll_pause;
    int row_contig;
    StreamFault fault;
    float* state;
    int state_stride;
    int steps;
    int serve;
    const unsigned long long* frame_gran;
    unsigned long long* pose_gran;
    const unsigned* stop;
    unsigned* end_frame;
    unsigned* end_claim;
    unsigned* ended_host;
    unsigned long long idle_ticks;
    int fold;
    unsigned long long* trace;
    int trace_frames;
};
constexpr unsigned kServeEndBit = 0x80000000u;
int stream_pipe_lds_bytes(int C, int cin0, int max_ring);
bool stream_pipe_channels_ok(int C);
hipError_t stream_pipe_prepare(Act wtype, int C, int lds_bytes);
hipError_t launch_stream_pipe(const StreamPipeParams& p, Act wtype, int lds_bytes, hipStream_t s);

hipError_t launch_normalize_screen(const float* x, int64_t n, int w, int h, float* out,
                                   bool inverse, hipStream_t s);
hipError_t launch_normalize_screen_f64(const double* x, int64_t n, double w, double hw, float* out, hipStream_t s);
hipError_t launch_camera_matrices(const float* intr, const int32_t* frame_seq, const double* extr,
                                  int64_t n_frames, float* out, hipStream_t s);
hipError_t launch_world_to_camera(const float* X, int64_t n, const float q[4], const float t[3],
                                  float* out, hipStream_t s);
hipError_t launch_gather_windows(const float* kps, int f2, const float* cams,
                                 const int64_t* seq_off, const int32_t* seq_len,
                                 const int32_t* pairs, int B, int window, int pad, int shift,
                                 float* out, hipStream_t s);
hipError_t launch_pack_rows(const float* x, int M, int T_out, int T_in, int stride, int lda,
                            int K, int Kp, void* out, bool bf16, hipStream_t s);
hipError_t launch_pack_rows_x3(const float* x, const struct GatherSrc* g, int M, int T_out, int T_in, int stride,
                               int cin, int K, int Kp, void* out, unsigned* fault, hipStream_t s);
hipError_t launch_mpjpe_accumulate(const float* pred, const float* target, int64_t n,
                                   double* acc, hipStream_t s);
hipError_t launch_mpjpe_backward(const float* pred, const float* target, int64_t n, const float* grad_loss,
                                 float* grad_pred, hipStream_t s);
hipError_t launch_project_to_2d(const float* X, int64_t n_cams, int64_t pts_per_cam, const float* params,
                                bool linear, float* out, hipStream_t s);
hipError_t launch_nonfinite_check(const float* y, int64_t n, unsigned* flag, unsigned bit, hipStream_t s);
constexpr unsigned kFaultSplitTimeout = 1u;
constexpr unsigned kFaultNonFinite = 2u;
constexpr unsigned kFaultWindowStart = 4u;
struct WindowRegions {
    int pitch, main_lo, max_len;
    int edge_row0, epitch;
    unsigned serial;
    unsigned* gate;
    unsigned* hint;
};
hipError_t launch_window_bases(const int32_t* pairs, const int32_t* seq_len, int B, int n_seq, const WindowRegions& wr,
                               int lo, int lead, int32_t* base, unsigned* fault, hipStream_t s);
hipError_t launch_gather_table_rows(const void* table, const int32_t* base, int B, int T_out, int s0,
                                    int row_bytes, void* out, hipStream_t s);
hipError_t launch_pose_metrics(const float* pred, const float* target, int64_t n_frames, int J, double* acc,
                               hipStream_t s);

struct alignas(128) ActStats {
    unsigned absmax_bits;
    unsigned pad_;
    double sumsq;
    unsigned long long small;
};
constexpr int kActStatSlots = 64;
hipError_t launch_act_stats(const float* a, int64_t n, ActStats* out, hipStream_t s);

struct WgradParams {
    const void* dZ;
    int ldz, dz_T, dz_off;
    const void* X;
    int cin, T_in, stride, dil, T_out;
    int64_t M;
    int N, K;
    int64_t rows_per_split;
    float* part;
};
constexpr int kMaxAdamTensors = 64;
struct AdamList {
    float* param[kMaxAdamTensors];
    const float* grad[kMaxAdamTensors];
    float* exp_avg[kMaxAdamTensors];
    float* exp_avg_sq[kMaxAdamTensors];
    float* max_exp_avg_sq[kMaxAdamTensors];
    int64_t numel[kMaxAdamTensors];
    int block_start[kMaxAdamTensors + 1];
    int n;
};
struct AdamHyper {
    float lerp_w, beta2, one_minus_beta2, bc2_sqrt, eps, neg_step_size, weight_decay;
    int amsgrad;
};
int64_t train_reduce_part_doubles(int64_t M, int C);
int64_t train_reduce_chunks(int64_t M, int C);
hipError_t launch_pack_weights(const float* w, int cout, int cin, int taps, int mode, int Kp, float* out,
                               hipStream_t s);
hipError_t launch_pack_weights_bf16(const float* w, int cout, int cin, int taps, int mode, int Kp, void* out,
                                    hipStream_t s);
hipError_t launch_bn_train_stats(const float* Z, int64_t M, int C, double* part, const float* gamma,
                                 const float* beta, float eps, double momentum, float* running_mean,
                                 float* running_var, float* mean, float* invstd, float* alpha, float* shift,
                                 hipStream_t s);
hipError_t launch_bn_act_fwd(const float* Z, int64_t M, int C, const float* alpha, const float* shift, float p,
                             uint64_t seed, int layer, const float* R, int T_out, int R_T, int R_stride, int R_off,
                             float* Y, void* Y16, hipStream_t s);
hipError_t launch_bn_train_backward(const float* dO, const float* Z, int64_t M, int C, const float* gamma,
                                    const float* alpha, const float* shift, const float* mean, const float* invstd,
                                    float p, uint64_t seed, int layer, double* part, float* coef, float* dgamma,
                                    float* dbeta, int T_out, int dz_T, int dz_off, float* dZ, void* dZ16,
                                    hipStream_t s);
hipError_t launch_colsum(const float* D, int64_t M, int C, int ld, double* part, float* out, hipStream_t s);
hipError_t launch_res_grad_add(float* dIn, const float* dOut, int64_t M, int C, int T_out, int T_in, int rs, int ro,
                               hipStream_t s);
int wgrad_splits(int64_t M, int N, int K, int64_t max_part_floats);
hipError_t launch_wgrad(const WgradParams& p, int S, int taps, float* dW, hipStream_t s, bool bf16_rows = false);
hipError_t launch_wgrad_bf16_tiles(const WgradParams& p, int S, hipStream_t s);
hipError_t launch_rows_to_f32(const void* src, bool src_bf16, int64_t M, int C, int T_out, int src_T, int src_off,
                              float* out, hipStream_t s);
hipError_t launch_adam(const AdamList& L, const AdamHyper& hp, hipStream_t s);
hipError_t launch_dropout_mask(uint64_t seed, float p, int layer, int64_t n, uint8_t* out, hipStream_t s);
hipError_t launch_relu_mask(const float* Z, int64_t n, int C, const float* alpha, const float* shift, uint8_t* out,
                            hipStream_t s);

struct LstmParams {
    const float* gin;
    int win_stride;
    int n_win, W, H, L;
    const float* wih_t[4];
    const float* whh_t[4];
    const float* bias[4];
    const float* out_scale;
    const float* out_shift;
    float* out;
};
hipError_t launch_concat_frames(const float* a, int fa, const float* b, int fb, int64_t rows, float* out,
                                hipStream_t s);
hipError_t launch_layernorm_rows(const float* X, int d, int64_t n_rows, int W, int win_stride, const float* pe,
                                 const float* gamma, const float* beta, float eps, float* out, hipStream_t s);
hipError_t launch_attention(const float* QKV, int n_win, int W, int d, int heads, int last_only, float* O,
                            hipStream_t s);
hipError_t launch_lstm(const LstmParams& p, hipStream_t s);

struct LstmTrainParams {
    const float* gin;
    int B, T, H, L;
    const float* wih_t[4];
    const float* whh_t[4];
    const float* bias[4];
    float* gates;
    float* cs;
    float* hs;
    float* hlast;
    float dscale;
    uint64_t seed, thresh;
};
hipError_t launch_lstm_train_fwd(const LstmTrainParams& p, hipStream_t s);
struct LstmBpttParams {
    int B, T, H, L;
    const float* wih[4];
    const float* whh[4];
    float* gates;
    const float* cs;
    const float* dhlast;
    float dscale;
    uint64_t seed, thresh;
};
hipError_t launch_lstm_bptt(const LstmBpttParams& p, hipStream_t s);
hipError_t launch_lstm_drop_rows(const float* hs, int B, int T, int H, float p, uint64_t seed, int site, float* out,
                                 hipStream_t s);
hipError_t launch_vec_add(const float* a, const float* b, int n, float* out, hipStream_t s);
hipError_t launch_head_linear(const float* X, const float* W, const float* bias, int M, int N, int K, float* Y,
                              hipStream_t s);
hipError_t launch_head_linear_dgrad(const float* dY, const float* W, int M, int N, int K, float* dX, hipStream_t s);
hipError_t launch_bn_leaky_fwd(const float* Z, int M, int C, const float* alpha, const float* shift, float slope,
                               float p, uint64_t seed, int site, float* Y, hipStream_t s);
hipError_t launch_bn_leaky_bwd(const float* dO, const float* Z, int M, int C, const float* gamma, const float* alpha,
                               const float* shift, const float* mean, const float* invstd, float slope, float p,
                               uint64_t seed, int site, float* coef, float* dgamma, float* dbeta, float* dZ,
                               hipStream_t s);

constexpr int kStackedMaxLinear = 10;
struct StackedParams {
    const float* ya;
    const float* yb;
    float* y;
    const float* w;
    int64_t n_rows;
    int D;
    int ld;
    int n_lin;
    int Kp[kStackedMaxLinear], Np[kStackedMaxLinear];
    int w_off[kStackedMaxLinear], b_off[kStackedMaxLinear];
};
int stacked_mlp_lds_bytes(int mi, int ld);
constexpr int kStackedMaxLds = 160 * 1024;
hipError_t stacked_mlp_prepare();
hipError_t launch_stacked_mlp(const StackedParams& p, int mi, hipStream_t s);

}
```

dynamic-camera-augmented-videopose3d_amd/csrc/vp3d_capi.cpp:

```cpp
#include <hip/hip_runtime.h>

#include <algorithm>
#include <chrono>
#include <cmath>
#include <cstdlib>
#include <cstdio>
#include <cstring>
#include <string>
#include <vector>

#include "../../include/vp3d.h"
#include "kernels.h"
#include "host.h"

using namespace vp3d;

namespace vp3d {
namespace host {

thread_local std::string g_last_error;

int fail(int code, const std::string& msg) {
    g_last_error = msg;
    return code;
// ... 277 lines not shown
}

namespace vp3d {
namespace host {

bool layer_lengths(const vp3d_cfg& cfg, const std::vector<int>& pad, const std::vector<Layer>& layers, int T,
                   std::vector<int>& len) {
    struct {
        const vp3d_cfg& cfg;
        const std::vector<int>& pad;
        const std::vector<Layer>& layers;
    } hh{cfg, pad, layers}, *h = &hh;
    len.clear();
    int L = T;
    for (const Layer& ly : h->layers) {
        const int span = (ly.taps - 1) * ly.dil + 1;
        if (L < span) return false;
        const int out = (L - span) / ly.stride + 1;
        if (ly.residual) {
        }
        len.push_back(out);
        L = out;
    }
    const int nb = h->cfg.n_widths - 1;
    for (int b = 1; b <= nb; ++b) {
        const Layer& pw = h->layers[2 * b];
        const int lin = len[2 * b - 2];
        const int lout = len[2 * b];
        int rlen;
        if (pw.res_stride == 1)
            rlen = lin - 2 * h->pad[b];
        else
            rlen = (lin - pw.res_off + pw.res_stride - 1) / pw.res_stride;
        if (rlen != lout) return false;
    }
    return true;
}

}
}

namespace {

bool layer_lengths(const vp3d_handle* h, int T, std::vector<int>& len) {
    return layer_lengths(h->cfg, h->pad, h->layers, T, len);
}

size_t esize(int dtype) { return dtype == VP3D_DTYPE_F32 || dtype == VP3D_DTYPE_F16X3 ? 4 : 2; }

int ensure_ws(vp3d_handle* h, int B, int T, int dtype, int first = 0) {
    std::vector<int> len;
    if (!layer_lengths(h, T, len)) return fail(VP3D_ERR_ARG, "input too short for the receptive field");
    const size_t rows = (size_t)B * len[first];
    const size_t need = 3 * rows * h->cfg.channels * esize(dtype) +
                        (dtype == VP3D_DTYPE_F32 ? 0 : rows * h->layers[0].Kp * (dtype == VP3D_DTYPE_F16X3 ? 4 : 2));
    if (need <= h->ws_bytes) return VP3D_OK;
    if (h->ws) HIP_TRY(hipFree(h->ws));
    h->ws = nullptr;
    h->ws_bytes = 0;
    HIP_TRY(hipMalloc(&h->ws, need));
    h->ws_bytes = need;
    return VP3D_OK;
}

bool x3_supported(const vp3d_handle* h) { return h->cfg.channels % 64 == 0 && h->cfg.channels <= 1024; }
const char* x3_requirement() { return "dtype f16x3 needs channels % 64 == 0 and channels <= 1024"; }

int ensure_fault_word(vp3d_handle* h) {
    if (h->sk_err_host) return VP3D_OK;
    HIP_TRY(hipHostMalloc((void**)&h->sk_err_host, 4, hipHostMallocMapped));
    HIP_TRY(hipHostGetDevicePointer((void**)&h->sk_err_dev, h->sk_err_host, 0));
    *(volatile unsigned*)h->sk_err_host = 0u;
    return VP3D_OK;
}

int write_split_ctl(vp3d_handle* h, unsigned long long spin, int drop, hipStream_t s) {
    h->sk_ctl_stage = vp3d::SplitCtl{spin, h->sk_err_dev, drop, 0};
    HIP_TRY(hipMemcpyAsync((char*)h->sk_ws + kSplitPartBytes + vp3d::kSplitCtlOffset, &h->sk_ctl_stage,
                           sizeof(vp3d::SplitCtl), hipMemcpyHostToDevice, s));
    h->sk_ctl_spin = spin;
    h->sk_ctl_drop = drop;
    return VP3D_OK;
}

int ensure_split_ws(vp3d_handle* h, hipStream_t s) {
    if (h->sk_ws) return VP3D_OK;
    if (const int rc = ensure_fault_word(h)) return rc;
    void* ws = nullptr;
    HIP_TRY(hipMalloc(&ws, vp3d::kSplitPartBytes + vp3d::kSplitFlagBytes));
    const hipError_t e = hipMemsetAsync((char*)ws + vp3d::kSplitPartBytes, 0, vp3d::kSplitFlagBytes, s);
    if (e != hipSuccess) {
        hipFree(ws);
        return fail(VP3D_ERR_HIP, std::string("split-K flags: ") + hipGetErrorString(e));
    }
    h->sk_ws = ws;
    return write_split_ctl(h, vp3d::kSplitSpinTicks, 0, s);
}

int attach_split_ws(vp3d_handle* h, ConvGemmParams& p, hipStream_t s) {
    if (!conv_gemm_a4_would_split(p)) return VP3D_OK;
    const int rc = ensure_split_ws(h, s);
    if (rc) return rc;
    const char* sp = getenv("VP3D_A4_SPLIT_SPIN_TICKS");
    const char* dr = getenv("VP3D_A4_SPLIT_DROP");
    const unsigned long long spin = sp ? strtoull(sp, nullptr, 10) : vp3d::kSplitSpinTicks;
    const int drop = dr && atoi(dr) != 0 ? 1 : 0;
    if (spin != h->sk_ctl_spin || drop != h->sk_ctl_drop) {
        HIP_TRY(hipStreamSynchronize(s));
        if (const int rc2 = write_split_ctl(h, spin, drop, s)) return rc2;
    }
    p.sk_part = (float*)h->sk_ws;
    p.sk_flag = (int*)((char*)h->sk_ws + kSplitPartBytes);
    return VP3D_OK;
}

bool x3_split_shrink(const vp3d_handle* h) {
    const char* e = getenv("VP3D_X3_SHRINK");
    return !(e && strcmp(e, "f32") == 0) && h->layers.back().cout <= 64;
}

constexpr const char* kSplitFaultMsg =
    "split-K: an owner tile timed out waiting for its helper units (an earlier forward on this "
    "handle produced wrong poses); vp3d_sync_status clears the fault";
constexpr const char* kNonFiniteMsg =
    "f16x3: an earlier forward on this handle split an activation past the f16 range (|x| <= "
    "65504) or produced non-finite poses; its outputs are not valid -- run those inputs in fp32 "
    "(with an activation pre-scale set: re-calibrate with more headroom or clear the pre-scale). "
    "vp3d_sync_status clears the fault";
constexpr const char* kWindowStartMsg =
    "f16x3 expand table: an earlier forward on this handle had a window that names a sequence outside "
    "the pool, [0, n_seq); its outputs are not valid. vp3d_sync_status clears the fault";
const char* fault_msg(unsigned w) {
    if (w & vp3d::kFaultSplitTimeout) return kSplitFaultMsg;
    return (w & vp3d::kFaultWindowStart) && !(w & vp3d::kFaultNonFinite) ? kWindowStartMsg : kNonFiniteMsg;
}

struct TablePlan {
    int mode = 0;
    int T_tab = 0;
    int lo = 0;
    int s0 = 1;
    int b_pad = 0;
    size_t table_bytes = 0;
    bool forced = false;
    int depth = 0;
    std::vector<int> pitch, step;
    int max_base = 0;
    bool ix_allowed = false;
    bool trimmed = false;
    int main_lo = 0;
    int max_len = 0;
    int edge_row0 = 0;
    std::vector<int> epitch;
};
constexpr int kTableFactor = 2;
constexpr int kTableRatioNum = 1, kTableRatioDen = 1;
bool table_pays(int64_t rows, int64_t wrows, int C) {
    const int round = vp3d::conv_gemm_a4_round_tiles();
    if (round <= 0 || vp3d::conv_gemm_a4_tiles(rows, C) < round) return rows <= wrows / kTableFactor;
    return rows * kTableRatioDen <= wrows * kTableRatioNum;
}

void table_layer_geometry(ConvGemmParams& p, const Layer& L, int n_seq, int pitch_in, int step) {
    const int pitch_out = pitch_in - (L.taps - 1) * L.dil * step;
    p.M = n_seq * pitch_out;
    p.T_out = pitch_out;
    p.T_in = pitch_in;
    p.stride = 1;
    p.dil = L.dil * step;
    p.Ktap = 2 * L.cin;
}
void table_residual_geometry(ConvGemmParams& p, const Layer& L, int pitch_res, int step) {
    p.R_T = pitch_res;
    p.R_stride = 1;
    p.R_off = L.res_off * step;
}
void indirect_layer_geometry(ConvGemmParams& p, const Layer& L, int b_pad, int step) {
    if (L.residual) {
        p.R_T = -b_pad;
        p.R_stride = L.res_stride * step;
        p.R_off = L.res_off * step;
    } else {
        p.T_in = -b_pad;
        p.stride = L.stride * step;
        p.dil = L.dil * step;
        p.Ktap = 2 * L.cin;
    }
}
ConvGemmParams x3_probe(const Layer& L, int M, int T_out, int T_in) {
    void* const al = (void*)(uintptr_t)256;
    ConvGemmParams q{};
    q.A = q.W = al;
    q.Y = al;
    q.M = M;
    q.N = L.cout;
    q.K = L.K;
    q.Kp = 2 * L.Kp;
    q.T_out = T_out;
    q.T_in = T_in;
    q.stride = L.stride;
    q.dil = L.dil;
    q.Ktap = 2 * L.Ktap;
    q.lda = 2 * L.cin;
    q.ldy = 2 * L.cout;
    q.relu = 1;
    if (L.residual) {
        q.R = al;
        q.ldr = 2 * L.cout;
        q.R_stride = L.res_stride;
        q.R_off = L.res_off;
    }
    return q;
}

void plan_frame_tables(const vp3d_handle* h, int B, const std::vector<int>& len, int n_seq, TablePlan& tp) {
    tp.depth = 0;
    tp.pitch.assign(1, tp.T_tab);
    tp.step.assign(1, tp.s0);
    if (tp.mode == 0 || !tp.ix_allowed) return;
    const int nl = (int)h->layers.size();
    int want = (nl - 2) / 2 - 1;
    bool force = false;
    if (const char* e = getenv("VP3D_FRAME_TABLES")) {
        want = std::min(want, std::max(0, atoi(e)));
        force = true;
    }
    const int C = h->layers[0].cout;
    int ok_depth = 0;
    for (int l = 1; l <= want; ++l) {
        const Layer &Lk = h->layers[2 * l - 1], &Lp = h->layers[2 * l];
        const int pin = tp.pitch[l - 1], st = tp.step[l - 1];
        const int pout = pin - (Lk.taps - 1) * Lk.dil * st;
        if (!Lk.relu || Lk.residual || !Lp.relu || !Lp.residual || Lp.taps != 1 || Lp.stride != 1 ||
            Lp.res_stride != Lk.stride || Lk.cin != C || Lk.cout != C || Lp.cout != C || pout <= 0)
            break;
        if ((int64_t)tp.max_base + (int64_t)(len[2 * l] - 1) * st * Lk.stride >= pout) break;
        if (!force && !table_pays((int64_t)n_seq * pin, (int64_t)B * len[2 * l - 1], C)) break;
        ConvGemmParams q = x3_probe(Lk, 0, 0, 0);
        table_layer_geometry(q, Lk, n_seq, pin, st);
        ConvGemmParams r = x3_probe(Lp, 0, 0, 0);
        table_layer_geometry(r, Lp, n_seq, pout, st);
        table_residual_geometry(r, Lp, pin, st);
        if (!vp3d::conv_gemm_a4_x3_eligible(q, false) || !vp3d::conv_gemm_a4_x3_eligible(r, false)) break;
        tp.pitch.push_back(pout);
        tp.step.push_back(st * Lk.stride);
        const Layer &Nk = h->layers[2 * l + 1], &Np = h->layers[2 * l + 2];
        if (nl - 2 == 2 * l + 2 && !x3_split_shrink(h)) continue;
        ConvGemmParams ck = x3_probe(Nk, B * len[2 * l + 1], len[2 * l + 1], 0);
        indirect_layer_geometry(ck, Nk, tp.b_pad, tp.step[l]);
        ConvGemmParams cp = x3_probe(Np, B * len[2 * l + 2], len[2 * l + 2], len[2 * l + 1]);
        indirect_layer_geometry(cp, Np, tp.b_pad, tp.step[l]);
        if (Nk.relu && !Nk.residual && Np.relu && Np.residual && vp3d::conv_gemm_a4_x3_indirect_ok(ck, true) &&
            vp3d::conv_gemm_a4_x3_indirect_ok(cp, true))
            ok_depth = l;
    }
    tp.depth = ok_depth;
    tp.pitch.resize(ok_depth + 1);
    tp.step.resize(ok_depth + 1);
    if (ok_depth >= 1) tp.mode = 1;
}

TablePlan plan_expand_table(const vp3d_handle* h, int B, const std::vector<int>& len, int dtype, const GatherSrc* gs,
                            int n_seq, int max_len) {
    TablePlan tp;
    const int nl = (int)h->layers.size();
    if (dtype != VP3D_DTYPE_F16X3 || !gs || gs->cams || n_seq <= 0 || max_len <= 0 || nl < 4) return tp;
    const char* e = getenv("VP3D_EXPAND_TABLE");
    if (e && e[0] == '0') return tp;
    const bool force = e && (strcmp(e, "1") == 0 || strcmp(e, "copy") == 0);
    const char* fe = getenv("VP3D_FRAME_TABLES");
    const bool force_size = force || (fe && atoi(fe) >= 1);
    const Layer& L0 = h->layers[0];
    const int C = L0.cout;
    tp.s0 = L0.stride;
    if (gs->lead < 0) return tp;
    const int64_t span = (int64_t)(len[0] - 1) * tp.s0;
    tp.lo = -(int)(span + std::max(0, L0.taps - 1 - gs->lead));
    const int64_t t_tab = ((int64_t)max_len - 1 + gs->lead - tp.lo + span + 1 + 15) / 16 * 16;
    const int64_t rows = (int64_t)n_seq * t_tab;
    const int64_t bytes = rows * 2 * C * 2;
    if (bytes >= ((int64_t)1 << 31) - 65536) return tp;
    if (!force_size && !table_pays(rows, (int64_t)B * len[0], C)) return tp;
    tp.T_tab = (int)t_tab;
    tp.main_lo = tp.lo;
    tp.max_len = max_len;
    tp.max_base = max_len - 1 + gs->lead - tp.lo;
    tp.table_bytes = (size_t)bytes;
    tp.b_pad = (B + 63) / 64 * 64;
    tp.mode = 2;
    tp.forced = force;
    if (e && strcmp(e, "copy") == 0) return tp;
    const char* ge = getenv("VP3D_GEMM");
    if (ge && strcmp(ge, "q64") == 0) return tp;
    if (nl - 2 == 2 && !x3_split_shrink(h)) return tp;
    tp.ix_allowed = true;
    const Layer &L1 = h->layers[1], &L2 = h->layers[2];
    ConvGemmParams q = x3_probe(L1, B * len[1], len[1], 0);
    indirect_layer_geometry(q, L1, tp.b_pad, tp.s0);
    if (!L1.relu || L1.residual || !vp3d::conv_gemm_a4_x3_indirect_ok(q)) return tp;
    ConvGemmParams r = x3_probe(L2, B * len[2], len[2], len[1]);
    indirect_layer_geometry(r, L2, tp.b_pad, tp.s0);
    if (!L2.relu || !L2.residual || !vp3d::conv_gemm_a4_x3_indirect_ok(r)) return tp;
    tp.mode = 1;
    return tp;
}

bool want_trimmed(const vp3d_handle* h) {
    if (const char* e = getenv("VP3D_TABLE_TRIM")) return atoi(e) != 0;
    if (!h->tab_hint_host) return true;
    const unsigned edges = ((volatile unsigned*)h->tab_hint_host)[1];
    const unsigned seen = ((volatile unsigned*)h->tab_hint_host)[0];
    return !(seen != 0 && edges == seen);
}

void plan_table_layout(const vp3d_handle* h, const std::vector<int>& len, const GatherSrc* gs, int n_seq,
                       TablePlan& tp) {
    tp.epitch.assign((size_t)tp.depth + 1, 0);
    if (tp.mode != 1 || !want_trimmed(h)) return;
    const int C = h->layers[0].cout;
    const int64_t span = (int64_t)(len[0] - 1) * tp.s0;
    const int emax = std::max(-tp.lo, gs->lead) - 1;
    if (emax < 0) return;
    const int64_t main0 = ((int64_t)tp.max_len + span + 15) / 16 * 16;
    const int64_t edge0 = ((int64_t)emax + 1 + span + 15) / 16 * 16;
    const int64_t rows = (int64_t)n_seq * (main0 + 2 * edge0);
    if (rows * 2 * C * 2 >= ((int64_t)1 << 31) - 65536) return;
    std::vector<int> pitch{(int)main0}, epitch{(int)edge0};
    for (int l = 1; l <= tp.depth; ++l) {
        const Layer &Lk = h->layers[2 * l - 1], &Lp = h->layers[2 * l];
        const int st = tp.step[l - 1], reach = (Lk.taps - 1) * Lk.dil * st;
        const int pout = pitch[l - 1] - reach, eout = epitch[l - 1] - reach;
        const int64_t rd = (int64_t)(len[2 * l] - 1) * st * Lk.stride;
        if (pout <= 0 || eout <= 0 || tp.max_len - 1 + rd >= pout || emax + rd >= eout) return;
        for (int edge = 0; edge < 2; ++edge) {
            const int ns = edge ? 2 * n_seq : n_seq, pin = edge ? epitch[l - 1] : pitch[l - 1];
            ConvGemmParams q = x3_probe(Lk, 0, 0, 0);
            table_layer_geometry(q, Lk, ns, pin, st);
            ConvGemmParams r = x3_probe(Lp, 0, 0, 0);
            table_layer_geometry(r, Lp, ns, pin - reach, st);
            table_residual_geometry(r, Lp, pin, st);
            if (!vp3d::conv_gemm_a4_x3_eligible(q, false) || !vp3d::conv_gemm_a4_x3_eligible(r, false)) return;
        }
        pitch.push_back(pout);
        epitch.push_back(eout);
    }
    tp.trimmed = true;
    tp.main_lo = 0;
    tp.T_tab = (int)main0;
    tp.max_base = tp.max_len - 1;
    tp.pitch = pitch;
    tp.epitch = epitch;
    tp.edge_row0 = (int)(n_seq * main0);
    tp.table_bytes = (size_t)rows * 2 * C * 2;
}

size_t table_slot_bytes(const TablePlan& tp) { return (size_t)tp.b_pad * 4 + tp.table_bytes; }

int ensure_table(vp3d_handle* h, const TablePlan& tp, int n_seq, hipStream_t s) {
    const bool same_pairs = (int)h->tab_pairs_host.size() == 8 * n_seq &&
                            (n_seq == 0 || (h->tab_pairs_host[1] == tp.lo && h->tab_pairs_host[4 * n_seq + 3] == tp.max_len));
    if (!h->tab_gate) {
        HIP_TRY(hipMalloc((void**)&h->tab_gate, 256));
        HIP_TRY(hipMemsetAsync(h->tab_gate, 0, 256, s));
        HIP_TRY(hipHostMalloc((void**)&h->tab_hint_host, 8, hipHostMallocMapped));
        HIP_TRY(hipHostGetDevicePointer((void**)&h->tab_hint_dev, h->tab_hint_host, 0));
        ((volatile unsigned*)h->tab_hint_host)[0] = 0u;
        ((volatile unsigned*)h->tab_hint_host)[1] = 0u;
    }
    const size_t need = table_slot_bytes(tp) * (tp.depth > 0 ? 3 : 1);
    if (need > h->tab_bytes) {
        if (h->tab_ws) HIP_TRY(hipFree(h->tab_ws));
        h->tab_ws = nullptr;
        h->tab_bytes = 0;
        HIP_TRY(hipMalloc(&h->tab_ws, need));
        h->tab_bytes = need;
    }
    if (!same_pairs) {
        if (h->tab_pairs) HIP_TRY(hipFree(h->tab_pairs));
        h->tab_pairs = nullptr;
        h->tab_pairs_host.assign((size_t)8 * n_seq, 0);
        int32_t* const wide = h->tab_pairs_host.data();
        int32_t *const main = wide + 2 * n_seq, *const edge = wide + 4 * n_seq;
        for (int i = 0; i < n_seq; ++i) {
            wide[2 * i] = main[2 * i] = edge[4 * i] = edge[4 * i + 2] = i;
            wide[2 * i + 1] = edge[4 * i + 1] = tp.lo;
            main[2 * i + 1] = 0;
            edge[4 * i + 3] = tp.max_len;
        }
        HIP_TRY(hipMalloc((void**)&h->tab_pairs, (size_t)8 * n_seq * 4));
        HIP_TRY(hipMemcpyAsync(h->tab_pairs, h->tab_pairs_host.data(), (size_t)8 * n_seq * 4, hipMemcpyHostToDevice, s));
    }
    return VP3D_OK;
}

hipEvent_t get_event(vp3d_handle* h) {
    if (!h->free_events.empty()) {
        hipEvent_t e = h->free_events.back();
        h->free_events.pop_back();
        return e;
    }
    hipEvent_t e = nullptr;
    hipEventCreate(&e);
    return e;
}

}

extern "C" {

int vp3d_abi_version(void) { return VP3D_ABI_VERSION; }

const char* vp3d_last_error(void) { return g_last_error.c_str(); }

int vp3d_weight_count(const vp3d_cfg* cfg) {
    if (validate_cfg(cfg) != VP3D_OK) return -1;
    return 5 + 10 * (cfg->n_widths - 1) + 2;
}

int vp3d_create(const vp3d_cfg* cfg, const float* const* weights, int n_weights, vp3d_handle** out) {
    if (!out) return fail(VP3D_ERR_ARG, "out is NULL");
    *out = nullptr;
    int rc = validate_cfg(cfg);
    if (rc) return rc;
    vp3d_handle* h = new vp3d_handle();
    h->cfg = *cfg;
    if (h->cfg.bn_eps <= 0.f) h->cfg.bn_eps = 1e-5f;
    hipGetDevice(&h->device);
    build_geometry(h);
    h->x3_prescale.assign(h->layers.size() - 1, 0);
    rc = ensure_fault_word(h);
    if (!rc) rc = upload_weights(h, weights, n_weights);
    if (rc) {
        vp3d_destroy(h);
        return rc;
    }
    h->prof_ms.assign(h->layers.size(), 0.0);
    h->prof_n.assign(h->layers.size(), 0);
    h->prof_flop.assign(h->layers.size(), 0.0);
    *out = h;
    return VP3D_OK;
}

int vp3d_load_weights(vp3d_handle* h, const float* const* weights, int n_weights) {
    if (!h) return fail(VP3D_ERR_ARG, "handle is NULL");
    int dev = 0;
    hipGetDevice(&dev);
    if (dev != h->device) return fail(VP3D_ERR_STATE, "handle belongs to another device");
    return upload_weights(h, weights, n_weights);
}

int vp3d_destroy(vp3d_handle* h) {
    if (!h) return VP3D_OK;
    int prev = 0;
    hipGetDevice(&prev);
    hipSetDevice(h->device);
    free_layers(h);
    if (h->ws) hipFree(h->ws);
    if (h->gather_ws) hipFree(h->gather_ws);
    if (h->tab_ws) hipFree(h->tab_ws);
    if (h->tab_pairs) hipFree(h->tab_pairs);
    if (h->tab_gate) hipFree(h->tab_gate);
    if (h->tab_hint_host) hipHostFree(h->tab_hint_host);
    if (h->sk_ws) hipFree(h->sk_ws);
    if (h->x3_stats) hipFree(h->x3_stats);
    if (h->sk_err_host) hipHostFree(h->sk_err_host);
    for (auto& e : h->pending) {
        hipEventDestroy(e.a);
        hipEventDestroy(e.b);
    }
    for (auto e : h->free_events) hipEventDestroy(e);
    hipSetDevice(prev);
    delete h;
    return VP3D_OK;
}

int vp3d_receptive_field(const vp3d_handle* h) {
    if (!h) return -1;
    int frames = 0;
    for (int p : h->pad) frames += p;
    return 1 + 2 * frames;
}

int vp3d_total_causal_shift(const vp3d_handle* h) {
    if (!h) return -1;
    int frames = h->causal_shift[0];
    int next_dilation = h->cfg.filter_widths[0];
    for (int i = 1; i < h->cfg.n_widths; ++i) {
        frames += h->causal_shift[i] * next_dilation;
        next_dilation *= h->cfg.filter_widths[i];
    }
    return frames;
}

int vp3d_out_frames(const vp3d_handle* h, int T) {
    if (!h) return -1;
    std::vector<int> len;
    if (!layer_lengths(h, T, len)) return -1;
    return len.back();
}

int vp3d_layer_count(const vp3d_handle* h) { return h ? (int)h->layers.size() : -1; }

int vp3d_reserve(vp3d_handle* h, int B, int T, int dtype) {
    if (!h) return fail(VP3D_ERR_ARG, "handle is NULL");
    if (B <= 0) return fail(VP3D_ERR_ASSERT, "batch must be positive");
    if (dtype < 0 || dtype > VP3D_DTYPE_F16X3) return fail(VP3D_ERR_ARG, "unknown dtype");
    if (dtype == VP3D_DTYPE_F16X3 && !x3_supported(h)) return fail(VP3D_ERR_ARG, x3_requirement());
    return ensure_ws(h, B, T, dtype);
}

static int forward_impl(vp3d_handle* h, const float* x, int B, int T, float* y, int dtype, void* stream,
                        const GatherSrc* gs, vp3d::ActStats* calib = nullptr, int n_seq = 0, int max_len = 0) {
    int dev = 0;
    hipGetDevice(&dev);
    if (dev != h->device) return fail(VP3D_ERR_STATE, "handle belongs to another device");
    std::vector<int> len;
    if (!layer_lengths(h, T, len))
        return fail(VP3D_ERR_ARG, "input of " + std::to_string(T) +
                                      " frames does not fit the receptive field of " +
                                      std::to_string(vp3d_receptive_field(h)));
    if (h->sk_err_host) {
        const unsigned fw = *(volatile unsigned*)h->sk_err_host;
        if ((fw & vp3d::kFaultSplitTimeout) || (fw && dtype == VP3D_DTYPE_F16X3))
            return fail(VP3D_ERR_STATE, fault_msg(fw));
    }
    const bool x3 = dtype == VP3D_DTYPE_F16X3;
    if (x3 && !x3_supported(h)) return fail(VP3D_ERR_ARG, x3_requirement());
    TablePlan tp = plan_expand_table(h, B, len, dtype, gs, n_seq, max_len);
    plan_frame_tables(h, B, len, n_seq, tp);
    if (tp.mode == 2 && !tp.forced) tp = TablePlan{};
    if (tp.mode) plan_table_layout(h, len, gs, n_seq, tp);
    GatherSrc tab_gs, etab_gs;
    ConvGemmParams tab_p{}, etab_p{};
    if (tp.mode) {
        const Layer& L0 = h->layers[0];
        tab_gs = *gs;
        tab_p.M = n_seq * tp.T_tab;
        tab_p.N = L0.cout;
        tab_p.K = L0.K;
        tab_p.Kp = 2 * L0.Kp;
        tab_p.T_out = tp.T_tab;
        tab_p.T_in = T;
        tab_p.stride = 1;
        tab_p.dil = L0.dil;
        tab_p.Ktap = L0.Ktap;
        tab_p.lda = L0.cin;
        tab_p.relu = L0.relu ? 1 : 0;
        tab_p.ldy = 2 * L0.cout;
        tab_p.W = L0.wx3;
        tab_p.scale = L0.scale_x3;
        tab_p.shift = L0.shift_x3;
        tab_p.Y = (void*)(uintptr_t)256;
        const char* xe = getenv("VP3D_X3_EXPAND");
        if ((xe && strcmp(xe, "pack") == 0) || !expand_gemm_x3_eligible(tab_p, &tab_gs)) tp = TablePlan{};
    }
    if (gs) {
        h->tab_mode = tp.mode;
        h->tab_depth = tp.depth;
        h->tab_layout = tp.mode ? (tp.trimmed ? 2 : 1) : 0;
    }
    const int buf_first = tp.mode == 1 ? 2 * tp.depth + 1 : 0;
    int rc = ensure_ws(h, B, T, dtype, buf_first);
    if (rc) return rc;

    hipStream_t s = (hipStream_t)stream;
    char* table = nullptr;
    if (tp.mode) {
        if ((rc = ensure_table(h, tp, n_seq, s))) return rc;
        table = (char*)h->tab_ws + (size_t)tp.b_pad * 4;
        tab_gs.pairs = h->tab_pairs + (tp.trimmed ? 2 * n_seq : 0);
        tab_p.Y = table;
    }
    void* tbuf[3] = {table, nullptr, nullptr};
    if (tp.depth > 0)
        for (int i = 1; i < 3; ++i) tbuf[i] = table + i * table_slot_bytes(tp);
    const size_t edge_off = tp.trimmed ? (size_t)tp.edge_row0 * 2 * h->layers[0].cout * 2 : 0;
    unsigned serial = 0;
    int dslot = 0;
    if (tp.mode) {
        if (h->tab_serial == 0xffffffffu) {
            HIP_TRY(hipStreamSynchronize(s));
            HIP_TRY(hipMemsetAsync(h->tab_gate, 0, 256, s));
            ((volatile unsigned*)h->tab_hint_host)[0] = 0u;
            ((volatile unsigned*)h->tab_hint_host)[1] = 0u;
            h->tab_serial = 0;
        }
        serial = ++h->tab_serial;
        if (tp.trimmed) {
            etab_gs = tab_gs;
            etab_gs.pairs = h->tab_pairs + 4 * n_seq;
            etab_p = tab_p;
            etab_p.M = 2 * n_seq * tp.epitch[0];
            etab_p.T_out = tp.epitch[0];
            etab_p.Y = table + edge_off;
            etab_p.gate = h->tab_gate;
            etab_p.gate_serial = serial;
            if (!expand_gemm_x3_eligible(etab_p, &etab_gs))
                return fail(VP3D_ERR_ASSERT, "the edge fill of a trimmed expand table left the f16x3 expand kernels");
        }
        for (int li = 1, cur = 0, blk = -1; li <= 2 * tp.depth; ++li) {
            int out = 0;
            while (out == cur || out == blk) ++out;
            if (li & 1) blk = cur;
            cur = dslot = out;
        }
        vp3d::WindowRegions wr{};
        wr.pitch = tp.pitch[tp.depth];
        wr.main_lo = tp.main_lo;
        wr.max_len = tp.max_len;
        wr.edge_row0 = tp.edge_row0;
        wr.epitch = tp.trimmed ? tp.epitch[tp.depth] : 0;
        wr.serial = serial;
        wr.gate = h->tab_gate;
        wr.hint = h->tab_hint_dev;
        const hipError_t be = launch_window_bases(gs->pairs, gs->seq_len, B, n_seq, wr, tp.lo, gs->lead,
                                                  (int32_t*)tbuf[dslot] - tp.b_pad, h->sk_err_dev, s);
        if (be != hipSuccess) return fail(VP3D_ERR_HIP, std::string("window bases: ") + hipGetErrorString(be));
    }
    const Act act = dtype == VP3D_DTYPE_F32 ? Act::F32 : (dtype == VP3D_DTYPE_BF16 ? Act::BF16 : Act::F16);
    const size_t es = esize(dtype);
    const size_t buf_elems = (size_t)B * len[buf_first] * h->cfg.channels;
    char* base = (char*)h->ws;
    void* buf[3] = {base, base + buf_elems * es, base + 2 * buf_elems * es};

    const int nl = (int)h->layers.size();
    const void* cur_in = x;
    int cur_len = T;
    int xin_buf = -1;
    const void* block_in = nullptr;
    int block_len = 0;
    for (int li = 0; li < nl; ++li) {
        const Layer& L = h->layers[li];
        const bool first = li == 0, last = li == nl - 1;
        ConvGemmParams p{};
        p.A = cur_in;
        p.scale = L.scale;
        p.shift = dtype == VP3D_DTYPE_F16X3 ? L.shift_x3 : L.shift;
        p.M = B * len[li];
        p.N = L.cout;
        p.K = L.K;
        p.Kp = L.Kp;
        p.T_out = len[li];
        p.T_in = cur_len;
        p.stride = L.stride;
        p.dil = L.dil;
        p.Ktap = L.Ktap;
        p.lda = L.cin;
        p.relu = L.relu ? 1 : 0;
        p.ldy = L.cout;
        p.W = dtype == VP3D_DTYPE_F32 ? (const void*)L.w32
                                      : (dtype == VP3D_DTYPE_BF16 ? (const void*)L.wbf : (const void*)L.wh);
        const int tlevel = tp.mode == 1 && li >= 1 && li <= 2 * tp.depth ? (li + 1) / 2 : 0;
        const int ilevel = tp.mode == 1 && (li == 2 * tp.depth + 1 || li == 2 * tp.depth + 2) ? tp.depth : -1;
        int out_buf = -1;
        if (last) {
            p.Y = y;
        } else {
            void* const* const bufs = tlevel ? tbuf : buf;
            for (int bi = 0; bi < 3; ++bi) {
                if (bufs[bi] == cur_in || bufs[bi] == block_in) continue;
                out_buf = bi;
                break;
            }
            p.Y = bufs[out_buf];
        }
        if (L.residual) {
            p.R = block_in;
            p.R_T = block_len;
            p.R_stride = L.res_stride;
            p.R_off = L.res_off;
            p.ldr = L.cout;
        }
        if (tlevel) {
            table_layer_geometry(p, L, n_seq, cur_len, tp.step[tlevel - 1]);
            if (L.residual) table_residual_geometry(p, L, block_len, tp.step[tlevel - 1]);
        } else if (first && tp.mode) {
            p.M = tab_p.M;
        }
        ProfEvent pe{};
        const bool timed = h->profiling && li < 64 && ((h->prof_mask >> li) & 1);
        if (timed) {
            pe.layer = li;
            pe.a = get_event(h);
            pe.b = get_event(h);
            pe.flop = 2.0 * (double)p.M * (double)p.N * (double)p.K;
            hipEventRecord(pe.a, s);
        }
        Act a_type = first ? Act::F32 : act;
        const Act o_type = last ? Act::F32 : act;
        hipError_t e = hipSuccess;
        bool launched = false;
        if (x3 && last && x3_split_shrink(h)) {
            if ((rc = ensure_split_ws(h, s))) return rc;
            p.W = L.wx3;
            p.Kp = 2 * L.Kp;
            p.lda = 2 * L.cin;
            p.Ktap = 2 * L.Ktap;
            p.scale = L.scale_x3;
            p.sk_part = (float*)h->sk_ws;
            e = launch_conv_gemm_x3_shrink(p, s);
            launched = true;
        } else if (x3 && last) {
            p.W = L.w32;
            p.scale = L.scale_x3_f32;
            e = launch_conv_gemm(p, Act::F32, Act::F32, Act::F32, s);
            launched = true;
        } else if (x3 && first && tp.mode) {
            e = launch_expand_gemm_x3(tab_p, &tab_gs, s);
            if (e == hipSuccess && tp.trimmed) e = launch_expand_gemm_x3(etab_p, &etab_gs, s);
            if (e == hipSuccess && tp.mode == 2)
                e = launch_gather_table_rows(table, (const int32_t*)h->tab_ws, B, len[0], tp.s0, 2 * L.cout * 2, p.Y, s);
            if (tp.mode == 1) p.Y = table;
            launched = true;
        } else if (x3 && first && nl > 2 && [&] {
                       const char* xe = getenv("VP3D_X3_EXPAND");
                       if (xe && strcmp(xe, "pack") == 0) return false;
                       ConvGemmParams q = p;
                       q.W = L.wx3;
                       q.Kp = 2 * L.Kp;
                       q.ldy = 2 * L.cout;
                       return expand_gemm_x3_eligible(q, gs);
                   }()) {
            p.W = L.wx3;
            p.Kp = 2 * L.Kp;
            p.scale = L.scale_x3;
            p.ldy = 2 * L.cout;
            e = launch_expand_gemm_x3(p, gs, s);
            launched = true;
        } else if (x3) {
            if (first) {
                void* packed = base + 3 * buf_elems * es;
                e = launch_pack_rows_x3(gs ? nullptr : x, gs, p.M, p.T_out, p.T_in, p.stride, L.cin, L.K, L.Kp,
                                        packed, h->sk_err_dev, s);
                if (e != hipSuccess) return fail(VP3D_ERR_HIP, std::string("pack: ") + hipGetErrorString(e));
                p.A = packed;
                p.T_in = p.T_out;
                p.stride = 1;
                p.dil = 1;
                p.lda = 2 * L.Kp;
                p.Ktap = 2 * L.Kp;
            } else {
                p.lda = 2 * L.cin;
                p.Ktap = 2 * L.Ktap;
            }
            if (ilevel >= 0 && !L.residual) indirect_layer_geometry(p, L, tp.b_pad, tp.step[ilevel]);
            if (tlevel) p.Ktap = 2 * L.cin;
            const bool out_f32 = li == nl - 2 && !x3_split_shrink(h);
            p.Kp = 2 * L.Kp;
            p.W = L.wx3;
            p.scale = L.scale_x3;
            p.ldy = out_f32 ? L.cout : 2 * L.cout;
            if (L.residual) p.ldr = 2 * L.cout;
            if (ilevel >= 0 && L.residual) indirect_layer_geometry(p, L, tp.b_pad, tp.step[ilevel]);
            const char* ge = getenv("VP3D_GEMM");
            if (tlevel) {
                if (out_f32 || !conv_gemm_a4_x3_eligible(p, false))
                    return fail(VP3D_ERR_ASSERT, "frame table layer " + std::to_string(li) + " left the a4 tile forms");
                if (li == 2 * tp.depth && p.Y != tbuf[dslot])
                    return fail(VP3D_ERR_ASSERT, "the deepest frame table left the slot its window bases are in front of");
                e = launch_conv_gemm_a4_x3(p, false, s);
                if (e == hipSuccess && tp.trimmed) {
                    ConvGemmParams q = p;
                    table_layer_geometry(q, L, 2 * n_seq, tp.epitch[L.residual ? tlevel : tlevel - 1], tp.step[tlevel - 1]);
                    if (L.residual) table_residual_geometry(q, L, tp.epitch[tlevel - 1], tp.step[tlevel - 1]);
                    q.A = (const char*)p.A + edge_off;
                    q.Y = (char*)p.Y + edge_off;
                    if (p.R) q.R = (const char*)p.R + edge_off;
                    q.gate = h->tab_gate;
                    q.gate_serial = serial;
                    if (!conv_gemm_a4_x3_eligible(q, false))
                        return fail(VP3D_ERR_ASSERT, "frame table layer " + std::to_string(li) + " (edge segments) left the a4 tile forms");
                    e = launch_conv_gemm_a4_x3(q, false, s);
                }
            } else if ((rc = attach_split_ws(h, p, s))) {
                return rc;
            } else if (!(ge && strcmp(ge, "q64") == 0) &&
                       (conv_gemm_a4_x3_eligible(p, out_f32) || (ilevel >= 1 && !out_f32))) {
                e = launch_conv_gemm_a4_x3(p, out_f32, s);
            } else {
                if (!conv_gemm_q64_x3_eligible(p, out_f32)) return fail(VP3D_ERR_ARG, x3_requirement());
                e = launch_conv_gemm_q64_x3(p, out_f32, s);
            }
            launched = true;
        }
        const void* wfold = act == Act::BF16 ? (const void*)L.wfbf : (const void*)L.wfh;
        ConvGemmParams pf = p;
        pf.W = wfold;
        if (launched) {
        } else if (first && gs && act != Act::F32 && wfold && expand_gather_eligible(pf, *gs, o_type, act)) {
            e = launch_expand_gemm_gather(pf, *gs, act, s);
            launched = true;
        } else if (first && gs) {
            const size_t need = (size_t)B * T * L.cin * sizeof(float);
            if (need > h->gather_bytes) {
                if (h->gather_ws) HIP_TRY(hipFree(h->gather_ws));
                h->gather_ws = nullptr;
                h->gather_bytes = 0;
                HIP_TRY(hipMalloc(&h->gather_ws, need));
                h->gather_bytes = need;
            }
            hipError_t ge = launch_gather_windows(gs->kps, gs->f2, gs->cams, gs->seq_off, gs->seq_len,
                                                  gs->pairs, B, T, gs->lead, 0, h->gather_ws, s);
            if (ge != hipSuccess) return fail(VP3D_ERR_HIP, std::string("gather: ") + hipGetErrorString(ge));
            x = h->gather_ws;
            p.A = x;
        }
        if (launched) {
        } else if (first && act != Act::F32 && wfold && expand_gemm_eligible(pf, o_type, act)) {
            pf.A = p.A;
            e = launch_expand_gemm(pf, act, s);
            launched = true;
        } else if (first && act != Act::F32) {
            void* packed = base + 3 * buf_elems * es;
            hipError_t pe = launch_pack_rows((const float*)x, p.M, p.T_out, p.T_in, p.stride, p.lda,
                                             p.K, p.Kp, packed, act == Act::BF16, s);
            if (pe != hipSuccess) return fail(VP3D_ERR_HIP, std::string("pack: ") + hipGetErrorString(pe));
            p.A = packed;
            p.K = p.Kp;
            p.Ktap = p.Kp;
            p.lda = p.Kp;
            p.T_in = p.T_out;
            p.stride = 1;
            p.dil = 1;
            a_type = act;
        }
        if (!launched) {
            if (act != Act::F32 && !first && !last && (rc = attach_split_ws(h, p, s))) return rc;
            e = launch_conv_gemm(p, a_type, o_type, act, s);
        }
        if (e != hipSuccess)
            return fail(VP3D_ERR_HIP, std::string("conv layer ") + std::to_string(li) + ": " +
                                          hipGetErrorString(e));
        if (timed) {
            hipEventRecord(pe.b, s);
            h->pending.push_back(pe);
        }
        if (calib && !last) {
            const hipError_t ce = launch_act_stats((const float*)p.Y, (int64_t)p.M * L.cout, calib + (size_t)li * vp3d::kActStatSlots, s);
            if (ce != hipSuccess) return fail(VP3D_ERR_HIP, std::string("activation statistics: ") + hipGetErrorString(ce));
        }
        if (!last && !L.residual && !first) {
            block_in = cur_in;
            block_len = cur_len;
        }
        cur_in = p.Y;
        cur_len = tlevel ? p.T_out : (first && tp.mode == 1 ? tp.T_tab : len[li]);
        (void)xin_buf;
    }
    if (x3) {
        if ((rc = ensure_fault_word(h))) return rc;
        const hipError_t e = launch_nonfinite_check(y, (int64_t)B * len.back() * h->layers.back().cout,
                                                    h->sk_err_dev, vp3d::kFaultNonFinite, s);
        if (e != hipSuccess) return fail(VP3D_ERR_HIP, std::string("finite check: ") + hipGetErrorString(e));
    }
    return VP3D_OK;
}

int vp3d_forward(vp3d_handle* h, const float* x, int B, int T, float* y, int dtype, void* stream) {
    if (!h) return fail(VP3D_ERR_ARG, "handle is NULL");
    if (!x || !y) return fail(VP3D_ERR_ARG, "x / y is NULL");
    if (B <= 0) return fail(VP3D_ERR_ASSERT, "batch must be positive");
    if (dtype < 0 || dtype > VP3D_DTYPE_F16X3) return fail(VP3D_ERR_ARG, "unknown dtype");
    return forward_impl(h, x, B, T, y, dtype, stream, nullptr);
}

int vp3d_forward_windows(vp3d_handle* h, const float* kps, int32_t f2, const float* cams, const int64_t* seq_off,
                         const int32_t* seq_len, const int32_t* pairs, int B, int window, int lead, float* y,
                         int dtype, void* stream) {
    if (!h) return fail(VP3D_ERR_ARG, "handle is NULL");
    if (!kps || !seq_off || !seq_len || !pairs || !y) return fail(VP3D_ERR_ARG, "a device pointer is NULL");
    if (B <= 0) return fail(VP3D_ERR_ASSERT, "batch must be positive");
    if (dtype < 0 || dtype > VP3D_DTYPE_F16X3) return fail(VP3D_ERR_ARG, "unknown dtype");
    if (cams && dtype == VP3D_DTYPE_BF16)
        return fail(VP3D_ERR_ARG, "bf16 is refused with the camera concat (use fp16, f16x3 or fp32)");
    const int cin = h->cfg.num_joints_in * h->cfg.in_features;
    if (f2 + (cams ? 12 : 0) != cin)
        return fail(VP3D_ERR_ASSERT, "frame features (" + std::to_string(f2) + (cams ? " + 12" : "") +
                                         ") != num_joints_in * in_features (" + std::to_string(cin) + ")");
    GatherSrc g;
    g.kps = kps;
    g.f2 = f2;
    g.cams = cams;
    g.seq_off = seq_off;
    g.seq_len = seq_len;
    g.pairs = pairs;
    g.lead = lead;
    return forward_impl(h, nullptr, B, window, y, dtype, stream, &g);
}

int vp3d_forward_windows_pool(vp3d_handle* h, const float* kps, int32_t f2, const float* cams, const int64_t* seq_off,
                              const int32_t* seq_len, int32_t n_seq, int32_t max_len, const int32_t* pairs, int B,
                              int window, int lead, float* y, int dtype, void* stream) {
    if (!h) return fail(VP3D_ERR_ARG, "handle is NULL");
    if (!kps || !seq_off || !seq_len || !pairs || !y) return fail(VP3D_ERR_ARG, "a device pointer is NULL");
    if (B <= 0) return fail(VP3D_ERR_ASSERT, "batch must be positive");
    if (n_seq <= 0 || max_len <= 0) return fail(VP3D_ERR_ARG, "n_seq and max_len must be positive");
    if (dtype < 0 || dtype > VP3D_DTYPE_F16X3) return fail(VP3D_ERR_ARG, "unknown dtype");
    if (cams && dtype == VP3D_DTYPE_BF16)
        return fail(VP3D_ERR_ARG, "bf16 is refused with the camera concat (use fp16, f16x3 or fp32)");
    const int cin = h->cfg.num_joints_in * h->cfg.in_features;
    if (f2 + (cams ? 12 : 0) != cin)
        return fail(VP3D_ERR_ASSERT, "frame features (" + std::to_string(f2) + (cams ? " + 12" : "") +
                                         ") != num_joints_in * in_features (" + std::to_string(cin) + ")");
    GatherSrc g;
    g.kps = kps;
    g.f2 = f2;
    g.cams = cams;
    g.seq_off = seq_off;
    g.seq_len = seq_len;
    g.pairs = pairs;
    g.lead = lead;
    return forward_impl(h, nullptr, B, window, y, dtype, stream, &g, nullptr, n_seq, max_len);
}

int vp3d_expand_table_mode(const vp3d_handle* h) { return h ? h->tab_mode : -1; }

int vp3d_frame_table_depth(const vp3d_handle* h) { return h ? h->tab_depth : -1; }

int vp3d_table_layout(const vp3d_handle* h, int* edges) {
    if (!h) return -1;
    if (edges)
        *edges = h->tab_layout != 0 && h->tab_hint_host && ((volatile unsigned*)h->tab_hint_host)[1] == h->tab_serial;
    return h->tab_layout;
}

void vp3d_table_depth_rule(int* factor, int* ratio_num, int* ratio_den) {
    if (factor) *factor = kTableFactor;
    if (ratio_num) *ratio_num = kTableRatioNum;
    if (ratio_den) *ratio_den = kTableRatioDen;
}

int vp3d_sync_status(vp3d_handle* h, void* stream) {
    if (!h) return fail(VP3D_ERR_ARG, "handle is NULL");
    HIP_TRY(hipStreamSynchronize((hipStream_t)stream));
    if (!h->sk_err_host || !*(volatile unsigned*)h->sk_err_host) return VP3D_OK;
    const unsigned w = *(volatile unsigned*)h->sk_err_host;
    if (h->sk_ws && (w & vp3d::kFaultSplitTimeout)) {
        HIP_TRY(hipMemsetAsync((char*)h->sk_ws + vp3d::kSplitPartBytes, 0, vp3d::kSplitCtlOffset, (hipStream_t)stream));
        HIP_TRY(hipStreamSynchronize((hipStream_t)stream));
    }
    *(volatile unsigned*)h->sk_err_host = 0u;
    return fail(VP3D_ERR_STATE, fault_msg(w));
}

int vp3d_set_x3_prescale(vp3d_handle* h, const int32_t* p, int n) {
    if (!h) return fail(VP3D_ERR_ARG, "handle is NULL");
    if (!p) return fail(VP3D_ERR_ARG, "exponents is NULL");
    const int want = (int)h->layers.size() - 1;
    if (n != want)
        return fail(VP3D_ERR_ARG, "f16x3 pre-scale: expected " + std::to_string(want) +
                                      " exponents (one per conv layer output, none for the shrink), got " +
                                      std::to_string(n));
    for (int l = 0; l < n; ++l)
        if (p[l] < -VP3D_X3_PRESCALE_MAX || p[l] > VP3D_X3_PRESCALE_MAX)
            return fail(VP3D_ERR_ARG, "f16x3 pre-scale: layer " + std::to_string(l) + " has exponent " +
                                          std::to_string(p[l]) + ", past +-" + std::to_string(VP3D_X3_PRESCALE_MAX));
    for (int l = 2; l < n; l += 2)
        if (p[l] != p[0])
            return fail(VP3D_ERR_ARG, "f16x3 pre-scale: layer " + std::to_string(l) + " (a block's 1x1 output) has exponent " +
                                          std::to_string(p[l]) + " but the residual chain (layer 0, the expand output) has " +
                                          std::to_string(p[0]) + "; the layers a residual add joins share one exponent");
    int dev = 0;
    hipGetDevice(&dev);
    if (dev != h->device) return fail(VP3D_ERR_STATE, "handle belongs to another device");
    if (std::equal(p, p + n, h->x3_prescale.begin())) return VP3D_OK;
    HIP_TRY(hipDeviceSynchronize());
    const std::vector<int> prev = h->x3_prescale;
    h->x3_prescale.assign(p, p + n);
    const int rc = fold_x3(h);
    if (rc) h->x3_prescale = prev;
    return rc;
}

int vp3d_get_x3_prescale(const vp3d_handle* h, int32_t* p, int n) {
    if (!h) return fail(VP3D_ERR_ARG, "handle is NULL");
    if (!p) return fail(VP3D_ERR_ARG, "exponents is NULL");
    if (n != (int)h->x3_prescale.size())
        return fail(VP3D_ERR_ARG, "f16x3 pre-scale: expected room for " + std::to_string(h->x3_prescale.size()) +
                                      " exponents, got " + std::to_string(n));
    std::copy(h->x3_prescale.begin(), h->x3_prescale.end(), p);
    return VP3D_OK;
}

static int calibrate_impl(vp3d_handle* h, const float* x, int B, int T, vp3d_act_stats* out, void* stream,
                          const GatherSrc* gs) {
    if (!out) return fail(VP3D_ERR_ARG, "stats_out is NULL");
    int dev = 0;
    hipGetDevice(&dev);
    if (dev != h->device) return fail(VP3D_ERR_STATE, "handle belongs to another device");
    std::vector<int> len;
    if (!layer_lengths(h, T, len))
        return fail(VP3D_ERR_ARG, "input of " + std::to_string(T) + " frames does not fit the receptive field of " +
                                      std::to_string(vp3d_receptive_field(h)));
    const int n = (int)h->layers.size() - 1;
    hipStream_t s = (hipStream_t)stream;
    const size_t stat_bytes = (size_t)n * vp3d::kActStatSlots * sizeof(vp3d::ActStats);
    if (!h->x3_stats) HIP_TRY(hipMalloc((void**)&h->x3_stats, stat_bytes));
    HIP_TRY(hipMemsetAsync(h->x3_stats, 0, stat_bytes, s));
    float* y = nullptr;
    HIP_TRY(hipMalloc((void**)&y, (size_t)B * len.back() * h->layers.back().cout * sizeof(float)));
    int rc = forward_impl(h, x, B, T, y, VP3D_DTYPE_F32, stream, gs, h->x3_stats);
    std::vector<vp3d::ActStats> host((size_t)n * vp3d::kActStatSlots);
    hipError_t e = hipStreamSynchronize(s);
    if (e == hipSuccess) e = hipMemcpy(host.data(), h->x3_stats, stat_bytes, hipMemcpyDeviceToHost);
    hipFree(y);
    if (rc) return rc;
    if (e != hipSuccess) return fail(VP3D_ERR_HIP, std::string("calibration read-back: ") + hipGetErrorString(e));
    for (int l = 0; l < n; ++l) {
        const double count = (double)B * len[l] * h->layers[l].cout;
        unsigned bits = 0;
        double sumsq = 0.0;
        unsigned long long small = 0;
        for (int k = 0; k < vp3d::kActStatSlots; ++k) {
            const vp3d::ActStats& t = host[(size_t)l * vp3d::kActStatSlots + k];
            bits = std::max(bits, t.absmax_bits);
            sumsq += t.sumsq;
            small += t.small;
        }
        float amax;
        std::memcpy(&amax, &bits, 4);
        out[l].absmax = (double)amax;
        out[l].rms = std::sqrt(sumsq / count);
        out[l].small_share = (double)small / count;
    }
    return VP3D_OK;
}

int vp3d_x3_calibrate(vp3d_handle* h, const float* x, int B, int T, vp3d_act_stats* stats_out, void* stream) {
    if (!h) return fail(VP3D_ERR_ARG, "handle is NULL");
    if (!x) return fail(VP3D_ERR_ARG, "x is NULL");
    if (B <= 0) return fail(VP3D_ERR_ASSERT, "batch must be positive");
    return calibrate_impl(h, x, B, T, stats_out, stream, nullptr);
}

int vp3d_x3_calibrate_windows(vp3d_handle* h, const float* kps, int32_t f2, const float* cams, const int64_t* seq_off,
                              const int32_t* seq_len, const int32_t* pairs, int B, int window, int lead,
                              vp3d_act_stats* stats_out, void* stream) {
    if (!h) return fail(VP3D_ERR_ARG, "handle is NULL");
    if (!kps || !seq_off || !seq_len || !pairs) return fail(VP3D_ERR_ARG, "a device pointer is NULL");
    if (B <= 0) return fail(VP3D_ERR_ASSERT, "batch must be positive");
    const int cin = h->cfg.num_joints_in * h->cfg.in_features;
    if (f2 + (cams ? 12 : 0) != cin)
        return fail(VP3D_ERR_ASSERT, "frame features (" + std::to_string(f2) + (cams ? " + 12" : "") +
                                         ") != num_joints_in * in_features (" + std::to_string(cin) + ")");
    GatherSrc g;
    g.kps = kps;
    g.f2 = f2;
    g.cams = cams;
    g.seq_off = seq_off;
    g.seq_len = seq_len;
    g.pairs = pairs;
    g.lead = lead;
    return calibrate_impl(h, nullptr, B, window, stats_out, stream, &g);
}

int vp3d_profile_enable(vp3d_handle* h, int enable) {
    if (!h) return fail(VP3D_ERR_ARG, "handle is NULL");
    h->profiling = enable != 0;
    return VP3D_OK;
}

int vp3d_profile_layers(vp3d_handle* h, uint64_t mask) {
    if (!h) return fail(VP3D_ERR_ARG, "handle is NULL");
    h->prof_mask = mask;
    return VP3D_OK;
}

int vp3d_profile_reset(vp3d_handle* h) {
    if (!h) return fail(VP3D_ERR_ARG, "handle is NULL");
    for (auto& e : h->pending) {
        hipEventSynchronize(e.b);
        h->free_events.push_back(e.a);
        h->free_events.push_back(e.b);
    }
    h->pending.clear();
    std::fill(h->prof_ms.begin(), h->prof_ms.end(), 0.0);
// ... 1181 lines not shown
```

dynamic-camera-augmented-videopose3d_amd/vp3d_amd/_native.py:

```python
from __future__ import annotations

import ctypes
import os
import threading

import torch

_LIB_PATH = os.path.join(os.path.dirname(os.path.abspath(__file__)), "libvp3d.so")

VP3D_OK = 0
VP3D_ERR_ASSERT = 1
VP3D_ERR_ARG = 2
VP3D_ERR_HIP = 3
VP3D_ERR_OOM = 4
VP3D_ERR_STATE = 5

VARIANT_DILATED = 0
VARIANT_STRIDED_1F = 1

DTYPE_F32 = 0
DTYPE_BF16 = 1
DTYPE_F16 = 2
DTYPE_F16X3 = 3
DTYPES = {"fp32": DTYPE_F32, "float32": DTYPE_F32, "f32": DTYPE_F32,
          "bf16": DTYPE_BF16, "bfloat16": DTYPE_BF16,
          "fp16": DTYPE_F16, "float16": DTYPE_F16, "f16": DTYPE_F16,
          "f16x3": DTYPE_F16X3}

MAX_BLOCKS = 8

EXPORTS = [
    "vp3d_weight_count", "vp3d_create", "vp3d_load_weights", "vp3d_destroy",
    "vp3d_receptive_field", "vp3d_total_causal_shift", "vp3d_out_frames",
    "vp3d_reserve", "vp3d_forward", "vp3d_forward_windows", "vp3d_forward_windows_pool",
    "vp3d_expand_table_mode", "vp3d_frame_table_depth", "vp3d_table_layout", "vp3d_table_depth_rule",
    "vp3d_sync_status", "vp3d_profile_enable",
    "vp3d_layer_count",
    "vp3d_set_x3_prescale", "vp3d_get_x3_prescale", "vp3d_x3_calibrate", "vp3d_x3_calibrate_windows",
    "vp3d_profile_read", "vp3d_profile_reset", "vp3d_profile_layers", "vp3d_normalize_screen",
    "vp3d_normalize_screen_f64", "vp3d_image_coordinates", "vp3d_camera_matrices", "vp3d_world_to_camera",
    "vp3d_gather_windows", "vp3d_mpjpe_accumulate", "vp3d_pose_metrics", "vp3d_project_to_2d", "vp3d_last_error", "vp3d_abi_version",
    "vp3d_build_hash",
    "vp3d_stream_create", "vp3d_stream_reset", "vp3d_stream_io", "vp3d_stream_step",
    "vp3d_stream_frames_seen", "vp3d_stream_graph_capture", "vp3d_stream_graph_launch",
    "vp3d_stream_destroy", "vp3d_stream_persistent", "vp3d_stream_mode", "vp3d_stream_status",
    "vp3d_stream_serve_begin", "vp3d_stream_serve_post", "vp3d_stream_serve_wait", "vp3d_stream_serve_end",
    "vp3d_stream_trace", "vp3d_stream_serve_step",
    "vp3d_mstream_create", "vp3d_mstream_io", "vp3d_mstream_step", "vp3d_mstream_reset",
    "vp3d_mstream_frames_seen", "vp3d_mstream_graph_capture", "vp3d_mstream_graph_launch",
    "vp3d_mstream_destroy",
    "vp3d_lstream_create", "vp3d_lstream_lookahead", "vp3d_lstream_io", "vp3d_lstream_step",
    "vp3d_lstream_reset", "vp3d_lstream_counts", "vp3d_lstream_graph_capture", "vp3d_lstream_graph_launch",
    "vp3d_lstream_destroy",
    "vp3d_trainer_create", "vp3d_trainer_destroy", "vp3d_train_forward", "vp3d_train_backward",
    "vp3d_trainer_set_compute", "vp3d_trainer_compute", "vp3d_train_capture", "vp3d_train_read",
    "vp3d_train_profile",
    "vp3d_train_dropout_mask", "vp3d_train_relu_mask", "vp3d_train_layer_rows", "vp3d_train_reduce_doubles", "vp3d_adam_step", "vp3d_mpjpe_backward",
    "vp3d_seq_weight_count", "vp3d_seq_create", "vp3d_seq_destroy", "vp3d_seq_forward",
    "vp3d_seq_sliding_window",
    "vp3d_seq_trainer_create", "vp3d_seq_trainer_destroy", "vp3d_seq_train_forward", "vp3d_seq_train_backward",
    "vp3d_seq_train_mask", "vp3d_seq_train_bytes", "vp3d_seq_train_profile",
    "vp3d_stacked_weight_count", "vp3d_stacked_create", "vp3d_stacked_forward", "vp3d_stacked_destroy",
]


class vp3d_cfg(ctypes.Structure):
    _fields_ = [
        ("num_joints_in", ctypes.c_int32),
        ("in_features", ctypes.c_int32),
        ("num_joints_out", ctypes.c_int32),
        ("n_widths", ctypes.c_int32),
        ("filter_widths", ctypes.c_int32 * MAX_BLOCKS),
        ("causal", ctypes.c_int32),
        ("channels", ctypes.c_int32),
        ("dense", ctypes.c_int32),
        ("variant", ctypes.c_int32),
        ("bn_eps", ctypes.c_float),
    ]


X3_PRESCALE_MAX = 24


class vp3d_act_stats(ctypes.Structure):
    _fields_ = [
        ("absmax", ctypes.c_double),
        ("rms", ctypes.c_double),
        ("small_share", ctypes.c_double),
    ]


SEQ_TRANSFORMER = 0
SEQ_LSTM = 1
SEQ_MAX_HEAD = 8


class vp3d_seq_cfg(ctypes.Structure):
    _fields_ = [
        ("kind", ctypes.c_int32),
        ("num_joints_in", ctypes.c_int32),
        ("in_features", ctypes.c_int32),
        ("num_joints_out", ctypes.c_int32),
        ("out_features", ctypes.c_int32),
        ("d_model", ctypes.c_int32),
        ("num_layers", ctypes.c_int32),
        ("n_heads", ctypes.c_int32),
        ("dim_feedforward", ctypes.c_int32),
        ("n_head_layers", ctypes.c_int32),
        ("head_layers", ctypes.c_int32 * SEQ_MAX_HEAD),
        ("max_len", ctypes.c_int32),
        ("eps", ctypes.c_float),
    ]


STACKED_MAX_LAYERS = 8
STACKED_MAX_LAYER_SIZE = 512


class vp3d_stacked_cfg(ctypes.Structure):
    _fields_ = [
        ("num_joints", ctypes.c_int32),
        ("features", ctypes.c_int32),
        ("num_layers", ctypes.c_int32),
        ("layer_size", ctypes.c_int32),
    ]


_lib = None
_lock = threading.Lock()

_vp = ctypes.c_void_p
_i32 = ctypes.c_int32
_i64 = ctypes.c_int64
_int = ctypes.c_int

_SIGNATURES = {
    "vp3d_weight_count": (_int, [ctypes.POINTER(vp3d_cfg)]),
    "vp3d_create": (_int, [ctypes.POINTER(vp3d_cfg), ctypes.POINTER(_vp), _int, ctypes.POINTER(_vp)]),
    "vp3d_load_weights": (_int, [_vp, ctypes.POINTER(_vp), _int]),
    "vp3d_destroy": (_int, [_vp]),
    "vp3d_receptive_field": (_int, [_vp]),
    "vp3d_total_causal_shift": (_int, [_vp]),
    "vp3d_out_frames": (_int, [_vp, _int]),
    "vp3d_reserve": (_int, [_vp, _int, _int, _int]),
    "vp3d_forward": (_int, [_vp, _vp, _int, _int, _vp, _int, _vp]),
    "vp3d_forward_windows": (_int, [_vp, _vp, _i32, _vp, _vp, _vp, _vp, _int, _int, _int, _vp, _int, _vp]),
    "vp3d_forward_windows_pool": (_int, [_vp, _vp, _i32, _vp, _vp, _vp, _i32, _i32, _vp, _int, _int, _int, _vp,
                                         _int, _vp]),
    "vp3d_expand_table_mode": (_int, [_vp]),
    "vp3d_frame_table_depth": (_int, [_vp]),
    "vp3d_table_layout": (_int, [_vp, ctypes.POINTER(_int)]),
    "vp3d_table_depth_rule": (None, [ctypes.POINTER(_int), ctypes.POINTER(_int), ctypes.POINTER(_int)]),
    "vp3d_profile_enable": (_int, [_vp, _int]),
    "vp3d_sync_status": (_int, [_vp, _vp]),
    "vp3d_layer_count": (_int, [_vp]),
    "vp3d_set_x3_prescale": (_int, [_vp, ctypes.POINTER(_i32), _int]),
    "vp3d_get_x3_prescale": (_int, [_vp, ctypes.POINTER(_i32), _int]),
    "vp3d_x3_calibrate": (_int, [_vp, _vp, _int, _int, ctypes.POINTER(vp3d_act_stats), _vp]),
    "vp3d_x3_calibrate_windows": (_int, [_vp, _vp, _i32, _vp, _vp, _vp, _vp, _int, _int, _int,
                                         ctypes.POINTER(vp3d_act_stats), _vp]),
    "vp3d_profile_read": (_int, [_vp, _vp, _vp, _vp]),
    "vp3d_profile_reset": (_int, [_vp]),
    "vp3d_profile_layers": (_int, [_vp, ctypes.c_uint64]),
    "vp3d_normalize_screen": (_int, [_vp, _i64, _i32, _i32, _vp, _vp]),
    "vp3d_normalize_screen_f64": (_int, [_vp, _i64, ctypes.c_double, ctypes.c_double, _vp, _vp]),
    "vp3d_image_coordinates": (_int, [_vp, _i64, _i32, _i32, _vp, _vp]),
    "vp3d_camera_matrices": (_int, [_vp, _vp, _vp, _i64, _vp, _vp]),
    "vp3d_world_to_camera": (_int, [_vp, _i64, _vp, _vp, _vp, _vp]),
    "vp3d_gather_windows": (_int, [_vp, _i32, _vp, _vp, _vp, _vp, _i32, _i32, _i32, _i32, _vp, _vp]),
    "vp3d_mpjpe_accumulate": (_int, [_vp, _vp, _i64, _vp, _vp]),
    "vp3d_mpjpe_backward": (_int, [_vp, _vp, _i64, _vp, _vp, _vp]),
    "vp3d_pose_metrics": (_int, [_vp, _vp, _i64, _i32, _vp, _vp]),
    "vp3d_project_to_2d": (_int, [_vp, _i64, _i64, _vp, _i32, _vp, _vp]),
    "vp3d_stream_create": (_int, [_vp, _int, ctypes.POINTER(_vp)]),
    "vp3d_stream_reset": (_int, [_vp, _vp]),
    "vp3d_stream_io": (_int, [_vp, ctypes.POINTER(_vp), ctypes.POINTER(_vp), ctypes.POINTER(_int)]),
    "vp3d_stream_step": (_int, [_vp, _vp, _vp, _vp]),
    "vp3d_stream_frames_seen": (ctypes.c_int64, [_vp]),
    "vp3d_stream_graph_capture": (_int, [_vp, _vp, _int]),
    "vp3d_stream_graph_launch": (_int, [_vp, _vp]),
    "vp3d_stream_destroy": (_int, [_vp]),
    "vp3d_stream_persistent": (_int, [_vp]),
    "vp3d_stream_mode": (_int, [_vp]),
    "vp3d_stream_status": (_int, [_vp]),
    "vp3d_stream_serve_begin": (_int, [_vp, _vp, ctypes.c_double]),
    "vp3d_stream_serve_post": (_int, [_vp, _vp, ctypes.POINTER(_i64)]),
    "vp3d_stream_serve_wait": (_int, [_vp, _i64, _vp, ctypes.c_double]),
    "vp3d_stream_serve_end": (_int, [_vp, _vp]),
    "vp3d_stream_trace": (_int, [_vp, _vp, ctypes.c_int64, _vp, _vp, _vp]),
    "vp3d_stream_serve_step": (_int, [_vp, _vp, _vp, ctypes.c_double, _vp]),
    "vp3d_mstream_create": (_int, [_vp, _int, _int, ctypes.POINTER(_vp)]),
    "vp3d_mstream_io": (_int, [_vp, ctypes.POINTER(_vp), ctypes.POINTER(_vp), ctypes.POINTER(_vp)]),
    "vp3d_mstream_step": (_int, [_vp, _vp, _vp, _vp, _vp]),
    "vp3d_mstream_reset": (_int, [_vp, _int, _vp]),
    "vp3d_mstream_frames_seen": (_int, [_vp, _vp]),
    "vp3d_mstream_graph_capture": (_int, [_vp, _vp]),
    "vp3d_mstream_graph_launch": (_int, [_vp, _vp]),
    "vp3d_mstream_destroy": (_int, [_vp]),
    "vp3d_lstream_create": (_int, [_vp, _int, _int, ctypes.POINTER(_vp)]),
    "vp3d_lstream_lookahead": (_int, [_vp, ctypes.POINTER(ctypes.c_int32)]),
    "vp3d_lstream_io": (_int, [_vp, ctypes.POINTER(_vp), ctypes.POINTER(_vp), ctypes.POINTER(_vp),
                               ctypes.POINTER(_vp)]),
    "vp3d_lstream_step": (_int, [_vp, _vp, _vp, _vp, _vp, _vp]),
    "vp3d_lstream_reset": (_int, [_vp, _int, _vp]),
    "vp3d_lstream_counts": (_int, [_vp, _vp, _vp]),
    "vp3d_lstream_graph_capture": (_int, [_vp, _vp]),
    "vp3d_lstream_graph_launch": (_int, [_vp, _vp]),
    "vp3d_lstream_destroy": (_int, [_vp]),
    "vp3d_trainer_create": (_int, [ctypes.POINTER(vp3d_cfg), ctypes.POINTER(_vp)]),
    "vp3d_trainer_destroy": (_int, [_vp]),
    "vp3d_train_forward": (_int, [_vp, ctypes.POINTER(_vp), _int, _vp, _int, _int, ctypes.c_float,
                                  ctypes.c_double, ctypes.c_uint64, _vp, _vp]),
    "vp3d_train_backward": (_int, [_vp, ctypes.POINTER(_vp), _int, _vp, ctypes.POINTER(_vp), _vp]),
    "vp3d_train_dropout_mask": (_int, [_vp, _int, _i64, _vp, _vp]),
    "vp3d_train_relu_mask": (_int, [_vp, _int, _i64, _vp, _vp]),
    "vp3d_train_layer_rows": (_i64, [_vp, _int]),
    "vp3d_trainer_set_compute": (_int, [_vp, _int]),
    "vp3d_trainer_compute": (_int, [_vp]),
    "vp3d_train_capture": (_int, [_vp, _int]),
    "vp3d_train_profile": (_int, [_vp, _int, ctypes.POINTER(ctypes.c_double)]),
    "vp3d_train_read": (_int, [_vp, _int, _int, _vp, _i64, _vp]),
    "vp3d_train_reduce_doubles": (_i64, [_i64, _int, _int]),
    "vp3d_adam_step": (_int, [_int, ctypes.POINTER(_vp), ctypes.POINTER(_vp), ctypes.POINTER(_vp),
                              ctypes.POINTER(_vp), ctypes.POINTER(_vp), ctypes.POINTER(_i64),
                              ctypes.c_double, ctypes.c_double, ctypes.c_double, ctypes.c_double,
                              ctypes.c_double, _i64, _int, _vp]),
    "vp3d_seq_weight_count": (_int, [ctypes.POINTER(vp3d_seq_cfg)]),
    "vp3d_seq_create": (_int, [ctypes.POINTER(vp3d_seq_cfg), ctypes.POINTER(_vp), _int, ctypes.POINTER(_vp)]),
    "vp3d_seq_destroy": (_int, [_vp]),
    "vp3d_seq_forward": (_int, [_vp, _vp, _vp, _int, _int, _vp, _vp]),
    "vp3d_seq_sliding_window": (_int, [_vp, _vp, _vp, _int, _int, _vp, _vp]),
    "vp3d_seq_trainer_create": (_int, [ctypes.POINTER(vp3d_seq_cfg), ctypes.POINTER(_vp)]),
    "vp3d_seq_trainer_destroy": (_int, [_vp]),
    "vp3d_seq_train_forward": (_int, [_vp, ctypes.POINTER(_vp), _int, _vp, _vp, _int, _int, ctypes.c_float,
                                      ctypes.POINTER(ctypes.c_double), ctypes.c_uint64, _vp, _vp]),
    "vp3d_seq_train_backward": (_int, [_vp, ctypes.POINTER(_vp), _int, _vp, ctypes.POINTER(_vp), _vp]),
    "vp3d_seq_train_mask": (_int, [_vp, _int, _int, _i64, _vp, _vp]),
    "vp3d_seq_train_bytes": (_i64, [ctypes.POINTER(vp3d_seq_cfg), _int, _int]),
    "vp3d_seq_train_profile": (_int, [_vp, _int, ctypes.POINTER(ctypes.c_double)]),
    "vp3d_stacked_weight_count": (_int, [ctypes.POINTER(vp3d_stacked_cfg)]),
    "vp3d_stacked_create": (_int, [ctypes.POINTER(vp3d_stacked_cfg), ctypes.POINTER(_vp), _int,
                                   ctypes.POINTER(_vp)]),
    "vp3d_stacked_forward": (_int, [_vp, _vp, _vp, _i64, _vp, _vp]),
    "vp3d_stacked_destroy": (_int, [_vp]),
    "vp3d_last_error": (ctypes.c_char_p, []),
    "vp3d_abi_version": (_int, []),
    "vp3d_build_hash": (ctypes.c_char_p, []),
}


def lib_path() -> str:
    return _LIB_PATH


def load():
    global _lib
    if _lib is not None:
        return _lib
    with _lock:
        if _lib is not None:
            return _lib
        if not os.path.exists(_LIB_PATH):
            raise ImportError(
                f"vp3d: native library not built ({_LIB_PATH}); run "
                "`python __graft_entry__.py build` (hipcc --offload-arch=gfx950)")
        lib = ctypes.CDLL(_LIB_PATH, mode=ctypes.RTLD_LOCAL)
        for name, (res, args) in _SIGNATURES.items():
            fn = getattr(lib, name)
            fn.restype = res
            fn.argtypes = args
        _check_provenance(lib)
        _lib = lib
        return lib


def _check_provenance(lib) -> None:
    from . import build as _build
    if not os.path.isdir(_build.CSRC):
        return
    want = _build.source_hash()
    got = lib.vp3d_build_hash().decode()
    if got != want:
        raise ImportError(
            f"vp3d: {_LIB_PATH} was built from other sources or for another target (library {got[:16]}, "
            f"tree {want[:16]} for arch {_build.ARCH}, VP3D_OFFLOAD_ARCH); "
            "rebuild with `python __graft_entry__.py build`")


class NativeError(RuntimeError):
    pass


def check(rc: int, what: str = "") -> None:
    if rc == VP3D_OK:
        return
    msg = load().vp3d_last_error().decode("utf-8", "replace")
    if what:
        msg = f"{what}: {msg}"
    if rc == VP3D_ERR_ASSERT:
        raise AssertionError(msg)
    raise NativeError(f"vp3d error {rc}: {msg}")


def make_cfg(num_joints_in, in_features, num_joints_out, filter_widths, causal, channels,
# ... 22 lines not shown
```

dynamic-camera-augmented-videopose3d_amd/vp3d_amd/lifter.py:

```python
from __future__ import annotations

import ctypes
from typing import Iterable, List, Sequence

import numpy as np
import torch

from . import _native as N


def weight_order(n_widths: int) -> List[str]:
    keys = ["expand_conv.weight", "expand_bn.weight", "expand_bn.bias",
            "expand_bn.running_mean", "expand_bn.running_var"]
    for i in range(2 * (n_widths - 1)):
        keys += [f"layers_conv.{i}.weight", f"layers_bn.{i}.weight", f"layers_bn.{i}.bias",
                 f"layers_bn.{i}.running_mean", f"layers_bn.{i}.running_var"]
    keys += ["shrink.weight", "shrink.bias"]
    return keys


def _host_f32(v) -> np.ndarray:
    if isinstance(v, torch.Tensor):
        v = v.detach().to("cpu", torch.float32).contiguous().numpy()
    return np.ascontiguousarray(np.asarray(v, dtype=np.float32))


class NativeLifter:

    def __init__(self, num_joints_in: int, in_features: int, num_joints_out: int,
                 filter_widths: Sequence[int], causal: bool, channels: int, dense: bool,
                 variant: int, state: dict, device=None, bn_eps: float = 1e-5):
        self._lib = N.load()
        self.n_widths = len(filter_widths)
        self.num_joints_out = num_joints_out
        self.cfg = N.make_cfg(num_joints_in, in_features, num_joints_out, filter_widths, causal,
                              channels, dense, variant, bn_eps)
        self.device = torch.device("cuda", torch.cuda.current_device() if device is None
                                   else torch.device(device).index or 0)
        self._h = ctypes.c_void_p()
        arrays, ptrs = self._pack(state)
        with torch.cuda.device(self.device):
            N.check(self._lib.vp3d_create(ctypes.byref(self.cfg), ptrs, len(arrays),
                                          ctypes.byref(self._h)), "vp3d_create")
        self.n_layers = self._lib.vp3d_layer_count(self._h)

    def _pack(self, state: dict):
        keys = weight_order(self.n_widths)
        missing = [k for k in keys if k not in state]
        if missing:
            raise KeyError(f"missing state_dict keys: {missing}")
        arrays = [_host_f32(state[k]) for k in keys]
        ptrs = (ctypes.c_void_p * len(arrays))(*[a.ctypes.data for a in arrays])
        return arrays, ptrs

    def load_weights(self, state: dict) -> None:
        arrays, ptrs = self._pack(state)
        with torch.cuda.device(self.device):
            N.check(self._lib.vp3d_load_weights(self._h, ptrs, len(arrays)), "vp3d_load_weights")

    def receptive_field(self) -> int:
        return self._lib.vp3d_receptive_field(self._h)

    def total_causal_shift(self) -> int:
        return self._lib.vp3d_total_causal_shift(self._h)

    def out_frames(self, T: int) -> int:
        return self._lib.vp3d_out_frames(self._h, int(T))

    def reserve(self, B: int, T: int, dtype: str = "fp32") -> None:
        with torch.cuda.device(self.device):
            N.check(self._lib.vp3d_reserve(self._h, int(B), int(T), N.DTYPES[dtype]), "vp3d_reserve")

    def forward(self, x: torch.Tensor, dtype: str = "fp32", out: torch.Tensor | None = None
                ) -> torch.Tensor:
        if x.device != self.device:
            raise RuntimeError(f"input on {x.device}, model on {self.device}")
        if x.dtype != torch.float32:
            x = x.float()
        x = x.contiguous()
        B, T = int(x.shape[0]), int(x.shape[1])
        T_out = self.out_frames(T)
        if T_out < 1:
            raise RuntimeError(f"input of {T} frames is invalid for receptive field "
                               f"{self.receptive_field()}")
        if out is None:
            out = torch.empty((B, T_out, self.num_joints_out, 3), dtype=torch.float32,
                              device=self.device)
        with torch.cuda.device(self.device):
            N.check(self._lib.vp3d_forward(self._h, x.data_ptr(), B, T, out.data_ptr(),
                                           N.DTYPES[dtype], N.stream_ptr(self.device)),
                    "vp3d_forward")
        return out

    def forward_windows(self, seqs, pairs: torch.Tensor, window: int, lead: int,
                        concat_cams: bool = False, dtype: str = "fp32",
                        out: torch.Tensor | None = None) -> torch.Tensor:
        def _idx(d):
            d = torch.device(d)
            return (d.type, d.index if d.index is not None else torch.cuda.current_device())
        if _idx(pairs.device) != _idx(self.device) or _idx(seqs.kps.device) != _idx(self.device):
            raise RuntimeError("pairs / sequences must live on the model's device")
        pairs = pairs.contiguous().to(torch.int32)
        B = int(pairs.shape[0])
        T_out = self.out_frames(window)
        if T_out < 1:
            raise RuntimeError(f"window of {window} frames is invalid for receptive field "
                               f"{self.receptive_field()}")
        cams = None
        if concat_cams:
            if seqs.cam is None:
                raise ValueError("no cameras loaded")
            cams = seqs.cam.data_ptr()
        if out is None:
            out = torch.empty((B, T_out, self.num_joints_out, 3), dtype=torch.float32,
                              device=self.device)
        with torch.cuda.device(self.device):
            N.check(self._lib.vp3d_forward_windows_pool(
                self._h, seqs.kps.data_ptr(), seqs.f2, cams, seqs.seq_off.data_ptr(),
                seqs.seq_len.data_ptr(), int(seqs.n_seq), int(max(seqs.lengths)), pairs.data_ptr(), B,
                int(window), int(lead), out.data_ptr(), N.DTYPES[dtype], N.stream_ptr(self.device)),
                "vp3d_forward_windows")
        return out

    def expand_table_mode(self) -> int:
        return self._lib.vp3d_expand_table_mode(self._h)

    def frame_table_depth(self) -> int:
        return self._lib.vp3d_frame_table_depth(self._h)

    def table_layout(self):
        e = ctypes.c_int(0)
        layout = self._lib.vp3d_table_layout(self._h, ctypes.byref(e))
        return layout, bool(e.value)

    def table_depth_rule(self):
        f, n, d = ctypes.c_int(0), ctypes.c_int(0), ctypes.c_int(0)
        self._lib.vp3d_table_depth_rule(ctypes.byref(f), ctypes.byref(n), ctypes.byref(d))
        return f.value, n.value, d.value

    def set_x3_prescale(self, p) -> None:
        n = self.n_layers - 1
        vals = [0] * n if p is None else [int(v) for v in p]
        arr = (ctypes.c_int32 * len(vals))(*vals)
        with torch.cuda.device(self.device):
            N.check(self._lib.vp3d_set_x3_prescale(self._h, arr, len(vals)), "vp3d_set_x3_prescale")

    def x3_prescale(self) -> List[int]:
        n = self.n_layers - 1
        arr = (ctypes.c_int32 * n)()
        N.check(self._lib.vp3d_get_x3_prescale(self._h, arr, n), "vp3d_get_x3_prescale")
        return list(arr)

    def calibrate_x3(self, x: torch.Tensor | None = None, *, seqs=None, pairs: torch.Tensor | None = None,
                     window: int | None = None, lead: int = 0, concat_cams: bool = False) -> List[dict]:
        n = self.n_layers - 1
        stats = (N.vp3d_act_stats * n)()
        if x is not None:
            if x.device != self.device:
                raise RuntimeError(f"input on {x.device}, model on {self.device}")
            x = x.float().contiguous()
            with torch.cuda.device(self.device):
                N.check(self._lib.vp3d_x3_calibrate(self._h, x.data_ptr(), int(x.shape[0]), int(x.shape[1]),
                                                    stats, N.stream_ptr(self.device)), "vp3d_x3_calibrate")
        else:
            if seqs is None or pairs is None or window is None:
                raise ValueError("calibrate_x3 takes x, or seqs + pairs + window")
            if pairs.device != self.device or seqs.kps.device != self.device:
                raise RuntimeError("pairs / sequences must live on the model's device")
            pairs = pairs.contiguous().to(torch.int32)
            cams = None
            if concat_cams:
                if seqs.cam is None:
                    raise ValueError("no cameras loaded")
                cams = seqs.cam.data_ptr()
            with torch.cuda.device(self.device):
                N.check(self._lib.vp3d_x3_calibrate_windows(
                    self._h, seqs.kps.data_ptr(), seqs.f2, cams, seqs.seq_off.data_ptr(),
                    seqs.seq_len.data_ptr(), pairs.data_ptr(), int(pairs.shape[0]), int(window), int(lead),
                    stats, N.stream_ptr(self.device)), "vp3d_x3_calibrate_windows")
        return [dict(layer=i, absmax=s.absmax, rms=s.rms, small_share=s.small_share) for i, s in enumerate(stats)]

    def sync_status(self) -> None:
        with torch.cuda.device(self.device):
            N.check(self._lib.vp3d_sync_status(self._h, N.stream_ptr(self.device)), "vp3d_sync_status")

    def profile(self, enable: bool) -> None:
        N.check(self._lib.vp3d_profile_enable(self._h, 1 if enable else 0))

    def profile_layers(self, layers=None) -> None:
        mask = (1 << 64) - 1 if layers is None else sum(1 << int(i) for i in layers)
        N.check(self._lib.vp3d_profile_layers(self._h, mask))

    def profile_reset(self) -> None:
        with torch.cuda.device(self.device):
            N.check(self._lib.vp3d_profile_reset(self._h))

    def profile_read(self):
        n = self.n_layers
        ms = (ctypes.c_double * n)()
        cnt = (ctypes.c_int64 * n)()
        fl = (ctypes.c_double * n)()
        with torch.cuda.device(self.device):
            N.check(self._lib.vp3d_profile_read(self._h, ctypes.addressof(ms),
                                                ctypes.addressof(cnt), ctypes.addressof(fl)))
        return [dict(layer=i, ms_total=ms[i], launches=cnt[i], flop=fl[i]) for i in range(n)]

    def close(self) -> None:
        if self._h:
            self._lib.vp3d_destroy(self._h)
            self._h = ctypes.c_void_p()

    def __del__(self):
        try:
            self.close()
        except Exception:
            pass
```

include/vp3d.h:

```cpp
#ifndef VP3D_H
#define VP3D_H

#include <stdint.h>

#ifdef __cplusplus
extern "C" {
#endif

#define VP3D_ABI_VERSION 1
#define VP3D_MAX_BLOCKS 8

#define VP3D_OK 0
#define VP3D_ERR_ASSERT 1
#define VP3D_ERR_ARG 2
#define VP3D_ERR_HIP 3
#define VP3D_ERR_OOM 4
#define VP3D_ERR_STATE 5

#define VP3D_VARIANT_DILATED 0
#define VP3D_VARIANT_STRIDED_1F 1

#define VP3D_DTYPE_F32 0
#define VP3D_DTYPE_BF16 1
#define VP3D_DTYPE_F16 2
#define VP3D_DTYPE_F16X3 3

typedef struct vp3d_cfg {
    int32_t num_joints_in;
    int32_t in_features;
    int32_t num_joints_out;
    int32_t n_widths;
    int32_t filter_widths[VP3D_MAX_BLOCKS];
    int32_t causal;
    int32_t channels;
    int32_t dense;
    int32_t variant;
    float bn_eps;
} vp3d_cfg;

typedef struct vp3d_handle vp3d_handle;


int vp3d_weight_count(const vp3d_cfg* cfg);

int vp3d_create(const vp3d_cfg* cfg, const float* const* weights, int n_weights, vp3d_handle** out);

int vp3d_load_weights(vp3d_handle* h, const float* const* weights, int n_weights);

int vp3d_destroy(vp3d_handle* h);

int vp3d_receptive_field(const vp3d_handle* h);
int vp3d_total_causal_shift(const vp3d_handle* h);
int vp3d_out_frames(const vp3d_handle* h, int T);


int vp3d_reserve(vp3d_handle* h, int B, int T, int dtype);

int vp3d_forward(vp3d_handle* h, const float* x, int B, int T, float* y, int dtype, void* stream);

int vp3d_sync_status(vp3d_handle* h, void* stream);

int vp3d_forward_windows(vp3d_handle* h, const float* kps, int32_t f2, const float* cams,
                         const int64_t* seq_off, const int32_t* seq_len, const int32_t* pairs, int B,
                         int window, int lead, float* y, int dtype, void* stream);

int vp3d_forward_windows_pool(vp3d_handle* h, const float* kps, int32_t f2, const float* cams,
                              const int64_t* seq_off, const int32_t* seq_len, int32_t n_seq, int32_t max_len,
                              const int32_t* pairs, int B, int window, int lead, float* y, int dtype,
                              void* stream);
int vp3d_expand_table_mode(const vp3d_handle* h);
int vp3d_frame_table_depth(const vp3d_handle* h);
int vp3d_table_layout(const vp3d_handle* h, int* edges);
void vp3d_table_depth_rule(int* factor, int* ratio_num, int* ratio_den);

#define VP3D_X3_PRESCALE_MAX 24

int vp3d_set_x3_prescale(vp3d_handle* h, const int32_t* p, int n);
int vp3d_get_x3_prescale(const vp3d_handle* h, int32_t* p, int n);

typedef struct vp3d_act_stats {
    double absmax;
    double rms;
    double small_share;
} vp3d_act_stats;

int vp3d_x3_calibrate(vp3d_handle* h, const float* x, int B, int T, vp3d_act_stats* stats_out, void* stream);
int vp3d_x3_calibrate_windows(vp3d_handle* h, const float* kps, int32_t f2, const float* cams,
                              const int64_t* seq_off, const int32_t* seq_len, const int32_t* pairs, int B,
                              int window, int lead, vp3d_act_stats* stats_out, void* stream);

int vp3d_profile_enable(vp3d_handle* h, int enable);
int vp3d_profile_layers(vp3d_handle* h, uint64_t mask);
int vp3d_layer_count(const vp3d_handle* h);
int vp3d_profile_read(vp3d_handle* h, double* ms_total, int64_t* launches, double* flop_last);
int vp3d_profile_reset(vp3d_handle* h);

typedef struct vp3d_stream vp3d_stream;

int vp3d_stream_create(vp3d_handle* h, int dtype, vp3d_stream** out);
int vp3d_stream_reset(vp3d_stream* s, void* stream);
int vp3d_stream_io(vp3d_stream* s, float** in_frames, float** out_poses, int* queue_len);
int vp3d_stream_step(vp3d_stream* s, const float* frame, float* pose, void* stream);
int64_t vp3d_stream_frames_seen(vp3d_stream* s);
int vp3d_stream_graph_capture(vp3d_stream* s, void* stream, int steps);
int vp3d_stream_graph_launch(vp3d_stream* s, void* stream);
int vp3d_stream_destroy(vp3d_stream* s);
int vp3d_stream_persistent(const vp3d_stream* s);
int vp3d_stream_mode(const vp3d_stream* s);
int vp3d_stream_status(vp3d_stream* s);

int vp3d_stream_serve_begin(vp3d_stream* s, void* stream, double idle_ms);
int vp3d_stream_serve_post(vp3d_stream* s, const float* frame, int64_t* frame_index);
int vp3d_stream_serve_wait(vp3d_stream* s, int64_t frame_index, float* pose, double timeout_ms);
int vp3d_stream_serve_step(vp3d_stream* s, const float* frame, float* pose, double timeout_ms, double* latency_us);
int vp3d_stream_serve_end(vp3d_stream* s, void* stream);
int vp3d_stream_trace(vp3d_stream* s, uint64_t* out, int64_t capacity, int32_t* role_first_wg, int32_t* n_roles,
                      int32_t* frames);

#define VP3D_MSTREAM_MAX 64
typedef struct vp3d_mstream vp3d_mstream;

int vp3d_mstream_create(vp3d_handle* h, int dtype, int n_streams, vp3d_mstream** out);
int vp3d_mstream_io(vp3d_mstream* m, float** frames, int32_t** active, float** poses);
int vp3d_mstream_step(vp3d_mstream* m, const float* frames, const int32_t* active, float* poses, void* stream);
int vp3d_mstream_reset(vp3d_mstream* m, int slot, void* stream);
int vp3d_mstream_frames_seen(vp3d_mstream* m, int64_t* out);
int vp3d_mstream_graph_capture(vp3d_mstream* m, void* stream);
int vp3d_mstream_graph_launch(vp3d_mstream* m, void* stream);
int vp3d_mstream_destroy(vp3d_mstream* m);

typedef struct vp3d_lstream vp3d_lstream;

int vp3d_lstream_create(vp3d_handle* h, int dtype, int n_streams, vp3d_lstream** out);
int vp3d_lstream_lookahead(vp3d_lstream* l, int32_t* out);
int vp3d_lstream_io(vp3d_lstream* l, float** frames, int32_t** codes, float** poses, int32_t** pose_frame);
int vp3d_lstream_step(vp3d_lstream* l, const float* frames, const int32_t* codes, float* poses, int32_t* pose_frame,
                      void* stream);
int vp3d_lstream_reset(vp3d_lstream* l, int slot, void* stream);
int vp3d_lstream_counts(vp3d_lstream* l, int64_t* consumed, int64_t* emitted);
int vp3d_lstream_graph_capture(vp3d_lstream* l, void* stream);
int vp3d_lstream_graph_launch(vp3d_lstream* l, void* stream);
int vp3d_lstream_destroy(vp3d_lstream* l);

typedef struct vp3d_trainer vp3d_trainer;

int vp3d_trainer_create(const vp3d_cfg* cfg, vp3d_trainer** out);
int vp3d_trainer_destroy(vp3d_trainer* t);

int vp3d_train_forward(vp3d_trainer* t, float* const* params, int n_params, const float* x, int B, int T,
                       float dropout_p, double momentum, uint64_t seed, float* y, void* stream);

int vp3d_train_backward(vp3d_trainer* t, float* const* params, int n_params, const float* dy,
                        float* const* grads, void* stream);

int vp3d_train_dropout_mask(vp3d_trainer* t, int layer, int64_t n_elems, uint8_t* out, void* stream);

int vp3d_train_relu_mask(vp3d_trainer* t, int layer, int64_t n_elems, uint8_t* out, void* stream);

int vp3d_trainer_set_compute(vp3d_trainer* t, int dtype);
int vp3d_trainer_compute(const vp3d_trainer* t);

int vp3d_train_capture(vp3d_trainer* t, int on);
int vp3d_train_read(vp3d_trainer* t, int layer, int which, float* out, int64_t n, void* stream);

int vp3d_train_profile(vp3d_trainer* t, int on, double* ms);

int64_t vp3d_train_layer_rows(const vp3d_trainer* t, int layer);

int64_t vp3d_train_reduce_doubles(int64_t rows, int channels, int reserved);

int vp3d_adam_step(int n, float* const* params, const float* const* grads, float* const* exp_avg,
                   float* const* exp_avg_sq, float* const* max_exp_avg_sq, const int64_t* numel, double lr,
                   double beta1, double beta2, double eps, double weight_decay, int64_t step, int amsgrad,
                   void* stream);

#define VP3D_SEQ_TRANSFORMER 0
#define VP3D_SEQ_LSTM 1
#define VP3D_SEQ_MAX_HEAD 8

typedef struct vp3d_seq_cfg {
    int32_t kind;
    int32_t num_joints_in, in_features, num_joints_out, out_features;
    int32_t d_model;
    int32_t num_layers;
    int32_t n_heads;
    int32_t dim_feedforward;
    int32_t n_head_layers;
    int32_t head_layers[VP3D_SEQ_MAX_HEAD];
    int32_t max_len;
    float eps;
} vp3d_seq_cfg;

typedef struct vp3d_seq_lifter vp3d_seq_lifter;

int vp3d_seq_weight_count(const vp3d_seq_cfg* cfg);
int vp3d_seq_create(const vp3d_seq_cfg* cfg, const float* const* weights, int n_weights, vp3d_seq_lifter** out);
int vp3d_seq_destroy(vp3d_seq_lifter* h);

int vp3d_seq_forward(vp3d_seq_lifter* h, const float* x2d, const float* xcam, int B, int T, float* y, void* stream);

int vp3d_seq_sliding_window(vp3d_seq_lifter* h, const float* x2d, const float* xcam, int L, int window, float* y,
                            void* stream);

typedef struct vp3d_seq_trainer vp3d_seq_trainer;

int vp3d_seq_trainer_create(const vp3d_seq_cfg* cfg, vp3d_seq_trainer** out);
int vp3d_seq_trainer_destroy(vp3d_seq_trainer* t);

int vp3d_seq_train_forward(vp3d_seq_trainer* t, float* const* params, int n_params, const float* x2d,
                           const float* xcam, int B, int T, float dropout_p, const double* momenta, uint64_t seed,
                           float* y, void* stream);

int vp3d_seq_train_backward(vp3d_seq_trainer* t, float* const* params, int n_params, const float* dy,
                            float* const* grads, void* stream);

int vp3d_seq_train_mask(vp3d_seq_trainer* t, int site, int which, int64_t n, uint8_t* out, void* stream);

int64_t vp3d_seq_train_bytes(const vp3d_seq_cfg* cfg, int B, int T);

int vp3d_seq_train_profile(vp3d_seq_trainer* t, int on, double* ms);

#define VP3D_STACKED_MAX_LAYERS 8
#define VP3D_STACKED_MAX_LAYER_SIZE 512
#define VP3D_STACKED_MAX_POSE 512

// ... 56 lines not shown
```

Baseline: 7.477 million poses/s.

## Compute frame-table layers only between edge rows and replicate edge rows

For frame-table levels, the planner works out which rows lie outside the region where padded frames differ. The GEMMs for those layers run only over the interior rows, and the residual layer writes into the full-pitch table through a new pitched-output kernel variant. The edge rows are then filled by copying the nearest computed row. This cuts redundant GEMM work on padding-constant rows, at the cost of an extra copy kernel and more template instantiations.

```diff
diff --git a/dynamic-camera-augmented-videopose3d_amd/csrc/conv_gemm_a4.hip b/dynamic-camera-augmented-videopose3d_amd/csrc/conv_gemm_a4.hip
--- a/dynamic-camera-augmented-videopose3d_amd/csrc/conv_gemm_a4.hip
+++ b/dynamic-camera-augmented-videopose3d_amd/csrc/conv_gemm_a4.hip
@@ -102,12 +102,14 @@
 __device__ unsigned long long* g_a4_trace;
 #endif
 
-template <typename CT, int ABL, int X3 = 0, bool GD = true, bool SPLIT = false, int HNL = 0, bool IX = false>
+template <typename CT, int ABL, int X3 = 0, bool GD = true, bool SPLIT = false, int HNL = 0, bool IX = false,
+          bool YP = false>
 __global__ __launch_bounds__(256, 1) void conv_gemm_a4(ConvGemmParams p_arg) {
     constexpr bool HN = HNL > 0;
     static_assert(!HN || (GD && !SPLIT), "half-N tiles: grouped pieces, no split");
     static_assert(HNL < 2 || X3 != 0, "quarter-N tiles: the split-fp16 epilogue only");
     static_assert(!IX || (X3 == 1 && GD && !SPLIT), "indirect windows: the split-fp16 whole / half-N / quarter-N tiles");
+    static_assert(!YP || (X3 == 1 && GD && !SPLIT && !IX), "pitched output: the split-fp16 whole / half-N / quarter-N tiles");
     constexpr int TN = GN >> HNL;
     constexpr int NJ = TN / 32;
     constexpr int WP = TN / 32;
@@ -503,6 +505,7 @@
     for (;;) {
         launder_lane_consts(prow, lc, fsw, fo0, fo1, a_base, w_base, grp, c0);
         launder_params(p);
+        if constexpr (YP) launder_s(p.Y_T);
         const int next = HN ? nunits : tix + (int)gridDim.x;
         const bool has_next = next < nunits;
         res0 = lres ? 0 : -1;
@@ -721,9 +724,21 @@
                     sh[j][0] = f32x2{h4[0], h4[1]};
                     sh[j][1] = f32x2{h4[2], h4[3]};
                 }
+                int ypr = 0, yr = 0;
+                if constexpr (YP) {
+                    const int mf = em0 + ewr * 128 + er16;
+                    const int yb = mf / p.T_out, yb0 = em0 / p.T_out;
+                    ypr = mf - yb * p.T_out;
+                    yr = (yb - yb0) * p.Y_T + ypr - (em0 - yb0 * p.T_out);
+                }
                 static_for<8>([&](auto i_c) __attribute__((always_inline)) {
                     constexpr int I = decltype(i_c)::value;
                     const int m = em0 + ewr * 128 + 16 * I + er16;
+                    if constexpr (YP && I > 0) {
+                        const bool wrap = ypr + 16 >= p.T_out;
+                        ypr += wrap ? 16 - p.T_out : 16;
+                        yr += wrap ? 16 + p.Y_T - p.T_out : 16;
+                    }
                     float v4[4][4];
                     static_for<NB>([&](auto j_c) __attribute__((always_inline)) {
                         constexpr int J = decltype(j_c)::value;
@@ -780,8 +795,11 @@
                                 t = gemm::x3_absmax2(t, v[2 * e], v[2 * e + 1]);
                             }
                             gemm::x3_range_flag(in ? t : 0.f, p.scale, p.N);
-                            const uint32_t yo =
-                                in ? (uint32_t)(((size_t)(m - em0) * p.ldy + 2 * nw + 64 * jp + ec0) * 2) : 0xFFFFFF00u;
+                            uint32_t yo;
+                            if constexpr (YP)
+                                yo = in ? (uint32_t)(((size_t)yr * p.ldy + 2 * nw + 64 * jp + ec0) * 2) : 0xFFFFFF00u;
+                            else
+                                yo = in ? (uint32_t)(((size_t)(m - em0) * p.ldy + 2 * nw + 64 * jp + ec0) * 2) : 0xFFFFFF00u;
                             if constexpr ((ABL & 16) != 0) {
                                 asm volatile("" ::"v"(oh), "v"(ol));
                             } else {
@@ -793,6 +811,11 @@
                 });
             };
             auto y_rsrc_of = [&]() __attribute__((always_inline)) {
+                if constexpr (YP) {
+                    const int yrow0 = out_row(p, em0);
+                    const size_t y_rest = (size_t)(out_row(p, p.M - 1) + 1 - yrow0) * p.ldy * OB;
+                    return make_rsrc((const char*)p.Y + (size_t)yrow0 * p.ldy * OB, clamp_range31(y_rest));
+                }
                 const size_t y_rest = (size_t)(p.M - em0) * p.ldy * OB;
                 return make_rsrc((const char*)p.Y + (size_t)em0 * p.ldy * OB,
                                  clamp_range31(y_rest));
@@ -1118,6 +1141,14 @@
     return q.sk_split <= 1;
 }
 
+bool conv_gemm_a4_x3_pitched_ok(const ConvGemmParams& p) {
+    if (p.Y_T < p.T_out || p.T_out < 16 || p.M <= 0 || p.R == nullptr || a4_indirect(p)) return false;
+    if (p.sk_part != nullptr || p.sk_flag != nullptr) return false;
+    const int64_t yrows = ((int64_t)(p.M - 1) / p.T_out) * p.Y_T + p.T_out;
+    if (yrows * p.ldy * 2 >= ((int64_t)1 << 31) - 65536) return false;
+    return a4_x3_shape_ok(p, false);
+}
+
 bool conv_gemm_a4_fills(const ConvGemmParams& p) {
     const int ntiles = ((p.M + GM - 1) / GM) * (p.N / GN);
     if (ntiles >= 384) return true;
@@ -1137,7 +1168,7 @@
         hipLaunchKernelGGL((conv_gemm_a4<CT, 0, X3, true, false>), grid, dim3(256), 0, stream, p);
 }
 
-template <typename CT, int X3, bool IX = false>
+template <typename CT, int X3, bool IX = false, bool YP = false>
 static void a4_launch_whole(const ConvGemmParams& p, int mt0, hipStream_t stream, int walk_cus) {
     if (mt0 > 0) {
         ConvGemmParams q = p;
@@ -1145,26 +1176,26 @@
         q.sk_split = q.sk_full = q.sk_left = 0;
         const int tiles = mt0 * (p.N / GN);
         const dim3 g(walk_cus > 0 && tiles > walk_cus ? walk_cus : tiles);
-        hipLaunchKernelGGL((conv_gemm_a4<CT, 0, X3, true, false, 0, IX>), g, dim3(256), 0, stream, q);
+        hipLaunchKernelGGL((conv_gemm_a4<CT, 0, X3, true, false, 0, IX, YP>), g, dim3(256), 0, stream, q);
     }
 }
 
-template <typename CT, int X3, bool IX = false>
+template <typename CT, int X3, bool IX = false, bool YP = false>
 static void a4_launch_hn(const ConvGemmParams& p, int mt_tail, hipStream_t stream, int walk_cus = 0, int level = 1) {
     const int ntm = (p.M + GM - 1) / GM;
     const int mt0 = ntm - mt_tail;
-    a4_launch_whole<CT, X3, IX>(p, mt0, stream, walk_cus);
+    a4_launch_whole<CT, X3, IX, YP>(p, mt0, stream, walk_cus);
     ConvGemmParams t = p;
     t.sk_split = t.sk_left = 0;
     t.sk_full = mt0;
     if constexpr (X3 != 0) {
         if (level == 2) {
-            hipLaunchKernelGGL((conv_gemm_a4<CT, 0, X3, true, false, 2, IX>), dim3(mt_tail * (p.N / (GN / 4))), dim3(256),
+            hipLaunchKernelGGL((conv_gemm_a4<CT, 0, X3, true, false, 2, IX, YP>), dim3(mt_tail * (p.N / (GN / 4))), dim3(256),
                                0, stream, t);
             return;
         }
     }
-    hipLaunchKernelGGL((conv_gemm_a4<CT, 0, X3, true, false, 1, IX>), dim3(mt_tail * (p.N / (GN / 2))), dim3(256), 0,
+    hipLaunchKernelGGL((conv_gemm_a4<CT, 0, X3, true, false, 1, IX, YP>), dim3(mt_tail * (p.N / (GN / 2))), dim3(256), 0,
                        stream, t);
 }
 
@@ -1184,11 +1215,17 @@
     const int hn_tail = walk_mode == 2 ? 0 : a4_hn_tail(p, ntiles, true, &hn_level);
     const bool ix = a4_indirect(p);
     if (ix && (out_f32 || !conv_gemm_a4_x3_indirect_ok(p, true))) return hipErrorInvalidValue;
+    const bool yp = p.Y_T != 0;
+    if (yp && !conv_gemm_a4_x3_pitched_ok(p)) return hipErrorInvalidValue;
 #ifndef VP3D_ABLATION
     if (hn_tail > 0) {
         const int wc = walk_mode > 0 && p.R != nullptr ? a4_cus() : 0;
         if (ix) {
             a4_launch_hn<_Float16, 1, true>(p, hn_tail, stream, wc, hn_level);
+            return hipGetLastError();
+        }
+        if (yp) {
+            a4_launch_hn<_Float16, 1, false, true>(p, hn_tail, stream, wc, hn_level);
             return hipGetLastError();
         }
         if (a4_tail_split(p, hn_tail, hn_level, true)) {
@@ -1217,7 +1254,7 @@
         const char* e = getenv("VP3D_ABL");
         return e ? atoi(e) : 0;
     }();
-    if (abl && !out_f32 && !split) {
+    if (abl && !out_f32 && !split && !yp) {
         switch (abl) {
             case 1: a4_x3_abl<1>(p, grid); break;
             case 2: a4_x3_abl<2>(p, grid); break;
@@ -1233,6 +1270,8 @@
 #endif
     if (ix)
         a4_launch<_Float16, 1, true>(p, grid, false, stream);
+    else if (yp)
+        hipLaunchKernelGGL((conv_gemm_a4<_Float16, 0, 1, true, false, 0, false, true>), grid, dim3(256), 0, stream, p);
     else if (out_f32)
         a4_launch<_Float16, 2>(p, grid, split, stream);
     else
diff --git a/dynamic-camera-augmented-videopose3d_amd/csrc/expand_table.hip b/dynamic-camera-augmented-videopose3d_amd/csrc/expand_table.hip
--- a/dynamic-camera-augmented-videopose3d_amd/csrc/expand_table.hip
+++ b/dynamic-camera-augmented-videopose3d_amd/csrc/expand_table.hip
@@ -49,6 +49,31 @@
     }
 }
 
+__global__ __launch_bounds__(256) void replicate_edge_rows_kernel(u32x4* __restrict__ table, int64_t reps, int per_seq,
+                                                                  int pitch, int a, int b, int row16) {
+    for (int64_t r = blockIdx.x; r < reps; r += gridDim.x) {
+        const int i = (int)(r / per_seq);
+        const int j = (int)(r - (int64_t)i * per_seq);
+        const int dst_row = j < a ? j : b + 1 + (j - a);
+        const int src_row = j < a ? a : b;
+        u32x4* const seq = table + (int64_t)i * pitch * row16;
+        const u32x4* src = seq + (int64_t)src_row * row16;
+        u32x4* dst = seq + (int64_t)dst_row * row16;
+        for (int c = threadIdx.x; c < row16; c += 256) dst[c] = src[c];
+    }
+}
+
+}
+
+hipError_t launch_replicate_edge_rows(void* table, int n_seq, int pitch, int a, int b, int row_bytes, hipStream_t s) {
+    if (row_bytes % 16 != 0 || row_bytes <= 0 || n_seq <= 0 || a < 0 || b < a || b >= pitch) return hipErrorInvalidValue;
+    const int per_seq = a + (pitch - 1 - b);
+    if (per_seq == 0) return hipSuccess;
+    const int64_t reps = (int64_t)n_seq * per_seq;
+    const unsigned grid = (unsigned)(reps < (1 << 20) ? reps : (1 << 20));
+    hipLaunchKernelGGL(replicate_edge_rows_kernel, dim3(grid), dim3(256), 0, s, (u32x4*)table, reps, per_seq, pitch, a, b,
+                       row_bytes / 16);
+    return hipGetLastError();
 }
 
 hipError_t launch_window_bases(const int32_t* pairs, const int32_t* seq_len, int B, int n_seq, const WindowRegions& wr,
diff --git a/dynamic-camera-augmented-videopose3d_amd/csrc/gemm_common.h b/dynamic-camera-augmented-videopose3d_amd/csrc/gemm_common.h
--- a/dynamic-camera-augmented-videopose3d_amd/csrc/gemm_common.h
+++ b/dynamic-camera-augmented-videopose3d_amd/csrc/gemm_common.h
@@ -60,6 +60,11 @@
     const int b = m / p.T_out;
     const int t = m - b * p.T_out;
     return b * p.R_T + t * p.R_stride + p.R_off;
+}
+
+__device__ __forceinline__ int out_row(const ConvGemmParams& p, int m) {
+    const int b = m / p.T_out;
+    return b * p.Y_T + (m - b * p.T_out);
 }
 
 template <int N>
diff --git a/dynamic-camera-augmented-videopose3d_amd/csrc/host.h b/dynamic-camera-augmented-videopose3d_amd/csrc/host.h
--- a/dynamic-camera-augmented-videopose3d_amd/csrc/host.h
+++ b/dynamic-camera-augmented-videopose3d_amd/csrc/host.h
@@ -109,6 +109,7 @@
     unsigned* tab_hint_host = nullptr;
     unsigned* tab_hint_dev = nullptr;
     int tab_layout = 0;
+    std::vector<int> tab_rows;
     void* sk_ws = nullptr;
     std::vector<int> x3_prescale;
     vp3d::ActStats* x3_stats = nullptr;
diff --git a/dynamic-camera-augmented-videopose3d_amd/csrc/kernels.h b/dynamic-camera-augmented-videopose3d_amd/csrc/kernels.h
--- a/dynamic-camera-augmented-videopose3d_amd/csrc/kernels.h
+++ b/dynamic-camera-augmented-videopose3d_amd/csrc/kernels.h
@@ -21,6 +21,7 @@
     int sk_full, sk_split, sk_left;
     const unsigned* gate;
     unsigned gate_serial;
+    int Y_T;
 };
 
 struct SplitCtl {
@@ -56,6 +57,7 @@
 int conv_gemm_a4_round_tiles();
 hipError_t launch_conv_gemm_a4_x3(const ConvGemmParams& p, bool out_f32, hipStream_t stream);
 bool conv_gemm_a4_x3_indirect_ok(const ConvGemmParams& p, bool any_fill = false);
+bool conv_gemm_a4_x3_pitched_ok(const ConvGemmParams& p);
 bool conv_gemm_tail_fits(const ConvGemmParams& p, int m_begin, int ncu, bool need_ws);
 hipError_t launch_conv_gemm_tail_x3(const ConvGemmParams& p, int m_begin, bool out_f32, int ncu,
                                     hipStream_t stream);
@@ -253,6 +255,7 @@
                                int lo, int lead, int32_t* base, unsigned* fault, hipStream_t s);
 hipError_t launch_gather_table_rows(const void* table, const int32_t* base, int B, int T_out, int s0,
                                     int row_bytes, void* out, hipStream_t s);
+hipError_t launch_replicate_edge_rows(void* table, int n_seq, int pitch, int a, int b, int row_bytes, hipStream_t s);
 hipError_t launch_pose_metrics(const float* pred, const float* target, int64_t n_frames, int J, double* acc,
                                hipStream_t s);
 
diff --git a/dynamic-camera-augmented-videopose3d_amd/csrc/vp3d_capi.cpp b/dynamic-camera-augmented-videopose3d_amd/csrc/vp3d_capi.cpp
--- a/dynamic-camera-augmented-videopose3d_amd/csrc/vp3d_capi.cpp
+++ b/dynamic-camera-augmented-videopose3d_amd/csrc/vp3d_capi.cpp
@@ -453,6 +453,7 @@
     int max_len = 0;
     int edge_row0 = 0;
     std::vector<int> epitch;
+    std::vector<int> row_a, row_b;
 };
 constexpr int kTableFactor = 2;
 constexpr int kTableRatioNum = 1, kTableRatioDen = 1;
@@ -655,6 +656,41 @@
     tp.table_bytes = (size_t)rows * 2 * C * 2;
 }
 
+void plan_table_edges(const vp3d_handle* h, const GatherSrc* gs, int n_seq, TablePlan& tp) {
+    tp.row_a.assign((size_t)tp.depth + 1, 0);
+    tp.row_b.resize((size_t)tp.depth + 1);
+    for (int l = 0; l <= tp.depth; ++l) tp.row_b[l] = tp.pitch[l] - 1;
+    if (tp.mode != 1 || tp.depth == 0) return;
+    if (const char* e = getenv("VP3D_TABLE_EDGES"))
+        if (atoi(e) == 0) return;
+    const Layer& L0 = h->layers[0];
+    int64_t S = (int64_t)(L0.taps - 1) * L0.dil;
+    for (int l = 1; l <= tp.depth; ++l) {
+        const Layer &Lk = h->layers[2 * l - 1], &Lp = h->layers[2 * l];
+        const int st = tp.step[l - 1], pin = tp.pitch[l - 1], pout = tp.pitch[l];
+        S += (int64_t)(Lk.taps - 1) * Lk.dil * st;
+        const int64_t a64 = (int64_t)gs->lead - tp.main_lo - S;
+        const int64_t b64 = (int64_t)tp.max_len - 1 + gs->lead - tp.main_lo;
+        const int a = (int)std::min<int64_t>(std::max<int64_t>(a64, 0), pout - 1);
+        const int b = (int)std::min<int64_t>(std::max<int64_t>(b64, a), pout - 1);
+        if (a == 0 && b == pout - 1) continue;
+        const int rows = b - a + 1;
+        ConvGemmParams q = x3_probe(Lk, 0, 0, 0);
+        table_layer_geometry(q, Lk, n_seq, pin, st);
+        q.M = n_seq * rows;
+        q.T_out = rows;
+        ConvGemmParams r = x3_probe(Lp, 0, 0, 0);
+        table_layer_geometry(r, Lp, n_seq, rows, st);
+        table_residual_geometry(r, Lp, pin, st);
+        r.Y_T = pout;
+        if (!vp3d::conv_gemm_a4_x3_eligible(q, false) || !vp3d::conv_gemm_a4_x3_eligible(r, false) ||
+            !vp3d::conv_gemm_a4_x3_pitched_ok(r))
+            continue;
+        tp.row_a[l] = a;
+        tp.row_b[l] = b;
+    }
+}
+
 size_t table_slot_bytes(const TablePlan& tp) { return (size_t)tp.b_pad * 4 + tp.table_bytes; }
 
 int ensure_table(vp3d_handle* h, const TablePlan& tp, int n_seq, hipStream_t s) {
@@ -855,10 +891,17 @@
         const char* xe = getenv("VP3D_X3_EXPAND");
         if ((xe && strcmp(xe, "pack") == 0) || !expand_gemm_x3_eligible(tab_p, &tab_gs)) tp = TablePlan{};
     }
+    if (tp.mode) plan_table_edges(h, gs, n_seq, tp);
     if (gs) {
         h->tab_mode = tp.mode;
         h->tab_depth = tp.depth;
         h->tab_layout = tp.mode ? (tp.trimmed ? 2 : 1) : 0;
+        h->tab_rows.clear();
+        for (int l = 0; tp.mode && l <= tp.depth; ++l) {
+            h->tab_rows.push_back(tp.row_a[l]);
+            h->tab_rows.push_back(tp.row_b[l] - tp.row_a[l] + 1);
+            h->tab_rows.push_back(tp.pitch[l]);
+        }
     }
     const int buf_first = tp.mode == 1 ? 2 * tp.depth + 1 : 0;
     int rc = ensure_ws(h, B, T, dtype, buf_first);
@@ -972,9 +1015,14 @@
             p.R_off = L.res_off;
             p.ldr = L.cout;
         }
+        int erows = 0, erow0 = 0;
         if (tlevel) {
             table_layer_geometry(p, L, n_seq, cur_len, tp.step[tlevel - 1]);
             if (L.residual) table_residual_geometry(p, L, block_len, tp.step[tlevel - 1]);
+            if (tp.row_a[tlevel] > 0 || tp.row_b[tlevel] < tp.pitch[tlevel] - 1) {
+                erow0 = tp.row_a[tlevel];
+                erows = tp.row_b[tlevel] - erow0 + 1;
+            }
         } else if (first && tp.mode) {
             p.M = tab_p.M;
         }
@@ -984,7 +1032,7 @@
             pe.layer = li;
             pe.a = get_event(h);
             pe.b = get_event(h);
-            pe.flop = 2.0 * (double)p.M * (double)p.N * (double)p.K;
+            pe.flop = 2.0 * (double)(erows ? n_seq * erows : p.M) * (double)p.N * (double)p.K;
             hipEventRecord(pe.a, s);
         }
         Act a_type = first ? Act::F32 : act;
@@ -1059,7 +1107,24 @@
                     return fail(VP3D_ERR_ASSERT, "frame table layer " + std::to_string(li) + " left the a4 tile forms");
                 if (li == 2 * tp.depth && p.Y != tbuf[dslot])
                     return fail(VP3D_ERR_ASSERT, "the deepest frame table left the slot its window bases are in front of");
-                e = launch_conv_gemm_a4_x3(p, false, s);
+                ConvGemmParams pm = p;
+                if (erows) {
+                    pm.M = n_seq * erows;
+                    pm.T_out = erows;
+                    if (!L.residual) {
+                        pm.A = (const char*)p.A + (size_t)erow0 * p.lda * 2;
+                    } else {
+                        pm.T_in = erows;
+                        pm.R_off = p.R_off + erow0;
+                        pm.Y = (char*)p.Y + (size_t)erow0 * p.ldy * 2;
+                        pm.Y_T = tp.pitch[tlevel];
+                    }
+                    if (!conv_gemm_a4_x3_eligible(pm, false) || (L.residual && !conv_gemm_a4_x3_pitched_ok(pm)))
+                        return fail(VP3D_ERR_ASSERT, "frame table layer " + std::to_string(li) + " (between its edge rows) left the a4 tile forms");
+                }
+                e = launch_conv_gemm_a4_x3(pm, false, s);
+                if (e == hipSuccess && erows && L.residual)
+                    e = launch_replicate_edge_rows(p.Y, n_seq, tp.pitch[tlevel], erow0, erow0 + erows - 1, p.ldy * 2, s);
                 if (e == hipSuccess && tp.trimmed) {
                     ConvGemmParams q = p;
                     table_layer_geometry(q, L, 2 * n_seq, tp.epitch[L.residual ? tlevel : tlevel - 1], tp.step[tlevel - 1]);
@@ -1223,6 +1288,16 @@
     if (edges)
         *edges = h->tab_layout != 0 && h->tab_hint_host && ((volatile unsigned*)h->tab_hint_host)[1] == h->tab_serial;
     return h->tab_layout;
+}
+
+int vp3d_table_rows(const vp3d_handle* h, int level, int* first_row, int* rows, int* pitch) {
+    if (!h) return fail(VP3D_ERR_ARG, "handle is NULL");
+    if (level < 0 || (size_t)3 * level + 2 >= h->tab_rows.size())
+        return fail(VP3D_ERR_ARG, "the last gathered forward had no table level " + std::to_string(level));
+    if (first_row) *first_row = h->tab_rows[3 * level];
+    if (rows) *rows = h->tab_rows[3 * level + 1];
+    if (pitch) *pitch = h->tab_rows[3 * level + 2];
+    return VP3D_OK;
 }
 
 void vp3d_table_depth_rule(int* factor, int* ratio_num, int* ratio_den) {
diff --git a/dynamic-camera-augmented-videopose3d_amd/vp3d_amd/_native.py b/dynamic-camera-augmented-videopose3d_amd/vp3d_amd/_native.py
--- a/dynamic-camera-augmented-videopose3d_amd/vp3d_amd/_native.py
+++ b/dynamic-camera-augmented-videopose3d_amd/vp3d_amd/_native.py
@@ -33,7 +33,7 @@
     "vp3d_weight_count", "vp3d_create", "vp3d_load_weights", "vp3d_destroy",
     "vp3d_receptive_field", "vp3d_total_causal_shift", "vp3d_out_frames",
     "vp3d_reserve", "vp3d_forward", "vp3d_forward_windows", "vp3d_forward_windows_pool",
-    "vp3d_expand_table_mode", "vp3d_frame_table_depth", "vp3d_table_layout", "vp3d_table_depth_rule",
+    "vp3d_expand_table_mode", "vp3d_frame_table_depth", "vp3d_table_layout", "vp3d_table_rows", "vp3d_table_depth_rule",
     "vp3d_sync_status", "vp3d_profile_enable",
     "vp3d_layer_count",
     "vp3d_set_x3_prescale", "vp3d_get_x3_prescale", "vp3d_x3_calibrate", "vp3d_x3_calibrate_windows",
@@ -150,6 +150,7 @@
     "vp3d_expand_table_mode": (_int, [_vp]),
     "vp3d_frame_table_depth": (_int, [_vp]),
     "vp3d_table_layout": (_int, [_vp, ctypes.POINTER(_int)]),
+    "vp3d_table_rows": (_int, [_vp, _int, ctypes.POINTER(_int), ctypes.POINTER(_int), ctypes.POINTER(_int)]),
     "vp3d_table_depth_rule": (None, [ctypes.POINTER(_int), ctypes.POINTER(_int), ctypes.POINTER(_int)]),
     "vp3d_profile_enable": (_int, [_vp, _int]),
     "vp3d_sync_status": (_int, [_vp, _vp]),
diff --git a/dynamic-camera-augmented-videopose3d_amd/vp3d_amd/lifter.py b/dynamic-camera-augmented-videopose3d_amd/vp3d_amd/lifter.py
--- a/dynamic-camera-augmented-videopose3d_amd/vp3d_amd/lifter.py
+++ b/dynamic-camera-augmented-videopose3d_amd/vp3d_amd/lifter.py
@@ -132,6 +132,12 @@
         e = ctypes.c_int(0)
         layout = self._lib.vp3d_table_layout(self._h, ctypes.byref(e))
         return layout, bool(e.value)
+
+    def table_rows(self, level: int):
+        a, r, p = ctypes.c_int(0), ctypes.c_int(0), ctypes.c_int(0)
+        N.check(self._lib.vp3d_table_rows(self._h, int(level), ctypes.byref(a), ctypes.byref(r), ctypes.byref(p)),
+                "vp3d_table_rows")
+        return a.value, r.value, p.value
 
     def table_depth_rule(self):
         f, n, d = ctypes.c_int(0), ctypes.c_int(0), ctypes.c_int(0)
diff --git a/include/vp3d.h b/include/vp3d.h
--- a/include/vp3d.h
+++ b/include/vp3d.h
@@ -71,6 +71,7 @@
 int vp3d_expand_table_mode(const vp3d_handle* h);
 int vp3d_frame_table_depth(const vp3d_handle* h);
 int vp3d_table_layout(const vp3d_handle* h, int* edges);
+int vp3d_table_rows(const vp3d_handle* h, int level, int* first_row, int* rows, int* pitch);
 void vp3d_table_depth_rule(int* factor, int* ratio_num, int* ratio_den);
 
 #define VP3D_X3_PRESCALE_MAX 24
```

New measurement: 7.749 million poses/s, median of 6. 3.6% higher.
